# hkapp/cniic

Measured on AMD Instinct MI355X. Metric: Mpixels/sec encode (cluster-colors K=256), higher is better.
Workload: dtype u8/u64; 1 GPU; configs[1]: cluster-colors(256) encode of one 4096x4096 photo-like synthetic RGB image per GPU (seed 0x636E696963+2+rank), to convergence; image and stream HBM-resident; pixels_per_gpu=16777216, parallelism=1 GPU

## Files before the change

### cniic_amd/csrc/codec.cpp

```cpp
#include "codec.hpp"
#include "cc_small.hpp"
#include "vor_small.hpp"
#include "delta_small.hpp"
#include "delta_small_dec.hpp"
#include "huf_small.hpp"
#include "small_trie.hpp"

#include <algorithm>
#include <cctype>
#include <cmath>
#include <cstring>
#include <functional>
#include <memory>

#include "huff_host.hpp"
#include "pal_bounds.hpp"

namespace cniic {

HostTrace &host_trace() { static thread_local HostTrace t; return t; }

static bool match_fun_u32(const std::string &s, const char *const *names, uint32_t *arg) {
    for (size_t p = 0; p < s.size(); p++)
        for (int i = 0; names[i]; i++) {
            const size_t l = strlen(names[i]);
            if (s.compare(p, l, names[i]) != 0 || p + l >= s.size() || s[p + l] != '(') continue;
            size_t q = p + l + 1;
            if (q >= s.size() || !isdigit((unsigned char)s[q])) continue;
            unsigned long long v = 0;
            bool ok = true;
            while (q < s.size() && isdigit((unsigned char)s[q])) {
                v = v * 10 + (unsigned)(s[q] - '0');
                if (v > 0xffffffffull) { ok = false; break; }
                q++;
            }
            if (!ok || q >= s.size() || s[q] != ')') continue;
            *arg = (uint32_t)v;
            return true;
        }
    return false;
}

static bool parse_rust_f64(const std::string &t, double *out) {
    size_t p = 0;
    if (p < t.size() && (t[p] == '+' || t[p] == '-')) p++;
    std::string rest = t.substr(p);
    std::transform(rest.begin(), rest.end(), rest.begin(), [](unsigned char ch) { return (char)tolower(ch); });
    if (rest != "inf" && rest != "infinity" && rest != "nan") {
        size_t q = p, digits = 0;
        while (q < t.size() && isdigit((unsigned char)t[q])) { q++; digits++; }
        if (q < t.size() && t[q] == '.') {
            q++;
            while (q < t.size() && isdigit((unsigned char)t[q])) { q++; digits++; }
        }
        if (!digits) return false;
        if (q < t.size() && (t[q] == 'e' || t[q] == 'E')) {
            q++;
            if (q < t.size() && (t[q] == '+' || t[q] == '-')) q++;
            size_t ed = 0;
            while (q < t.size() && isdigit((unsigned char)t[q])) { q++; ed++; }
            if (!ed) return false;
        }
        if (q != t.size()) return false;
    }
    *out = strtod(t.c_str(), nullptr);
    return true;
}

static bool match_hilbert_rle(const std::string &s, double *d) {
    *d = 0.0;
    if (s.compare(0, 8, "hilbert(") != 0 && s.compare(0, 8, "Hilbert(") != 0) return false;
    if (s.size() < 10 || s.back() != ')') return false;
    const std::string arg = s.substr(8, s.size() - 9);
    if (arg == "rle") return true;
    if (arg.size() > 5 && arg.compare(0, 4, "rle(") == 0 && arg.back() == ')') {
        const std::string num = arg.substr(4, arg.size() - 5);
        double v = 0.0;
        if (parse_rust_f64(num, &v)) {
            if (v != 0.0) *d = v;
            return true;
        }
        char *end = nullptr;
        v = strtod(num.c_str(), &end);
        return end && *end == 0 && !num.empty() && v == 0.0;
    }
    return false;
}

bool parse_codec(const char *expr, CodecDesc *out) {
    if (!expr) return false;
    const std::string s(expr);
    static const char *const cc[] = {"cluster-colors", "cluster-col", "clustercolors", "clustercol",
                                     "c-colors", "c-col", "ccolors", "ccol", nullptr};
    static const char *const vo[] = {"voronoi", nullptr};
    uint32_t k = 0;
    double dv = 0.0;
    if (match_fun_u32(s, cc, &k)) { *out = {CODEC_CLUSTER_COLORS, k, 0.0}; return true; }
    if (match_fun_u32(s, vo, &k)) { *out = {CODEC_VORONOI, k, 0.0}; return true; }
// ... 227 lines not shown
    StreamOut so(c, out, cap, len);
    CNIIC_TRY(so.begin_sized(header_bytes, (nbits + 7) / 8));
    CNIIC_TRY(st.write_decoder(so, header));
    CNIIC_TRY(st.upload_codes());
    CNIIC_HIP_TRY(c, hipStreamSynchronize(c->stream));
    st.release_tree();
    uint64_t packed_bits = 0;
    ScopedKernelTimer timer(c, "huff_pack");
    uint32_t *const keys_d = st.keys_d.as<uint32_t>();
    const uint8_t *const len_d = st.len_d.as<uint8_t>();
    const uint64_t *const code_d = st.code_d.as<uint64_t>();
    if (hot_route) {
        CNIIC_TRY(huff_pack_code32_hot(c, syms_d, n, table_d, keys_d, len_d, code_d, U, syms_d, so.dev, header_bytes * 8, &packed_bits));
    } else if (direct) {
        CNIIC_TRY(huff_pack_code32(c, syms_d, rgb_d, n, table_d, keys_d, len_d, code_d, U, ranks, so.dev, header_bytes * 8, &packed_bits));
    } else if (inline_codes) {
        DevBuf code32;
        CNIIC_HIP_TRY(c, code32.alloc(U * 4));
        CNIIC_TRY(huff_pack_code32(c, ranks, nullptr, n, code32.as<uint32_t>(), nullptr, len_d, code_d, U, ranks, so.dev, header_bytes * 8, &packed_bits));
    } else {
        CNIIC_TRY(huff_pack_ranks(c, ranks, n, len_d, code_d, so.dev, header_bytes * 8, &packed_bits));
    }
    timer.stop(1);
    host_trace().mark("huf: pack");
    if (packed_bits != nbits)
        return c->fail(CNIIC_ERR_HIP, "huffman: packed %llu bits, histogram predicts %llu", (unsigned long long)packed_bits,
                       (unsigned long long)nbits);
    const int rc_fin = so.finish();
    host_trace().mark("huf: finish");
    host_trace().dump();
    return rc_fin;
}

static int encode_hufman(Ctx *c, const uint8_t *rgb_d, uint32_t w, uint32_t h, uint8_t *out, uint64_t cap, uint64_t *len) {
    const uint64_t n = (uint64_t)w * h;
    std::vector<uint8_t> header;
    put_u32(header, w);
    put_u32(header, h);
    uint32_t *table = nullptr;
    CNIIC_TRY(dense_table(c, 24, &table));
    return huf_encode_all_dev(c, CNIIC_SYM_RGB, rgb_d, nullptr, false, n, table, false, header, out, cap, len);
}

CcSession::~CcSession() { if (km) km_rgbw_destroy(km); }

int cc_prepare(Ctx *c, uint32_t *table_counts_d, uint32_t K, const cniic_kmeans_opts *opts, uint32_t shard, uint32_t nshards,
               void *partials_dev, CcSession **out, const uint32_t *occ_d) {
    if (K == 0) return c->fail(CNIIC_ERR_BAD_ARG, "cluster-colors(0)");
    auto s = std::make_unique<CcSession>();
    s->c = c; s->K = K; s->table = table_counts_d;
    s->counts_local = occ_d != nullptr || nshards == 1;
    CompactPlan plan;
    DevBuf cell_count;
    CNIIC_HIP_TRY(c, cell_count.alloc((uint64_t)kNumCells * 4));
    CNIIC_HIP_TRY(c, hipMemsetAsync(cell_count.p, 0, (uint64_t)kNumCells * 4, c->stream));
    CNIIC_TRY(hist_compact_count(c, table_counts_d, 24, &plan, cell_count.as<uint32_t>()));
    host_trace().mark("compact_count+sync");
    const uint64_t U = plan.n_unique;
    s->U = U;
    uint64_t Ug = 0;
    if (occ_d) {
        CNIIC_TRY(gidx_build(c, occ_d, s->gbits, s->gprefix, &Ug));
        s->local_points = true;
    }
    if ((occ_d ? Ug : U) / K == 0 || U == 0)
        return c->fail(CNIIC_ERR_TOO_FEW_POINTS, "kmeans: %llu distinct colours for %u clusters (src/kmeans.rs:68)",
                       (unsigned long long)(occ_d ? Ug : U), K);
    CNIIC_HIP_TRY(c, s->keys_d.alloc(U * 4));
    CNIIC_HIP_TRY(c, s->weight_d.alloc(U * 4));
    CNIIC_TRY(hist_compact_write(c, table_counts_d, &plan, s->keys_d.as<uint32_t>(), nullptr, s->weight_d.as<uint32_t>()));
    host_trace().mark("compact_write enq");
    CNIIC_TRY(km_rgbw_create(c, s->keys_d.as<uint32_t>(), s->weight_d.as<uint32_t>(), U, shard, nshards, K, opts, partials_dev,
                             table_counts_d, &s->km, cell_count.as<uint32_t>(), occ_d ? s->gbits.p : nullptr,
                             occ_d ? s->gprefix.as<uint32_t>() : nullptr, Ug));
    host_trace().mark("km_create");
    *out = s.release();
    return CNIIC_OK;
}

int cc_prepare_image(Ctx *c, const uint8_t *rgb_d, uint64_t npx, uint32_t K, const cniic_kmeans_opts *opts, CcSession **out) {
    if (K == 0) return c->fail(CNIIC_ERR_BAD_ARG, "cluster-colors(0)");
    auto s = std::make_unique<CcSession>();
    s->c = c; s->K = K; s->sp_mode = true;
    CNIIC_TRY(sp_build(c, rgb_d, npx, &s->sp));
    const uint64_t Umax = std::min<uint64_t>(npx, 1ull << 24);
    const uint64_t *U_dev = s->sp.total.as<uint64_t>();
    CNIIC_TRY(km_rgbw_create(c, nullptr, nullptr, Umax, 0, 1, K, opts, nullptr, nullptr, &s->km, s->sp.cell_count.as<uint32_t>(), s->sp.bits.p,
                             s->sp.wprefix.as<uint32_t>(), Umax, true, U_dev));
    uint32_t *cell_start, *ckeys, *cweight;
    km_rgbw_cell_arrays(s->km, &cell_start, &ckeys, &cweight);
    CNIIC_TRY(sp_emit(c, &s->sp, cell_start, ckeys, cweight, km_rgbw_labels_internal(s->km, nullptr), km_rgbw_is_wide(s->km), K, s->sp.bits.p,
                      s->sp.wprefix.as<uint32_t>(), 0, U_dev));
    CNIIC_TRY(sp_wait_count(c, &s->sp));
    s->U = s->sp.U;
    if (s->U / K == 0)
        return c->fail(CNIIC_ERR_TOO_FEW_POINTS, "kmeans: %llu distinct colours for %u clusters (src/kmeans.rs:68)", (unsigned long long)s->U, K);
    CNIIC_TRY(km_rgbw_set_points(s->km, s->U));
    host_trace().mark("km_create + emit enq");
    *out = s.release();
    return CNIIC_OK;
}

int cc_image_begin(Ctx *c, const uint8_t *rgb_d, uint64_t npx, CcSession **out) {
    auto s = std::make_unique<CcSession>();
    s->c = c; s->sp_mode = true; s->local_points = true;
    CNIIC_TRY(sp_build(c, rgb_d, npx, &s->sp));
    *out = s.release();
    return CNIIC_OK;
}

int cc_image_create(CcSession *s, const uint32_t *occ_d, uint32_t K, const cniic_kmeans_opts *opts, void *partials_dev) {
    Ctx *c = s->c;
    if (!s->sp_mode || s->km) return c->fail(CNIIC_ERR_BAD_ARG, "cc_image_create: needs a session from cc_image_begin, once");
    if (K == 0) return c->fail(CNIIC_ERR_BAD_ARG, "cluster-colors(0)");
    s->K = K;
    CNIIC_HIP_TRY(c, c->pinned_u.reserve(kPinnedUBytes, kPinnedUBytes));
    uint64_t *Ug_h = c->pinned_u.as<uint64_t>() + kPuPointCount.at;
    CNIIC_TRY(gidx_build(c, occ_d, s->gbits, s->gprefix, Ug_h, &s->gtotal));
    const uint64_t Umax = std::min<uint64_t>(s->sp.npx, 1ull << 24);
    const uint64_t *Ug_dev = s->gtotal.as<uint64_t>();
    CNIIC_TRY(km_rgbw_create(c, nullptr, nullptr, Umax, 0, 1, K, opts, partials_dev, nullptr, &s->km, s->sp.cell_count.as<uint32_t>(), s->gbits.p,
                             s->gprefix.as<uint32_t>(), 1ull << 24, true, Ug_dev));
    uint32_t *cell_start, *ckeys, *cweight;
    km_rgbw_cell_arrays(s->km, &cell_start, &ckeys, &cweight);
    CNIIC_TRY(sp_emit(c, &s->sp, cell_start, ckeys, cweight, km_rgbw_labels_internal(s->km, nullptr), km_rgbw_is_wide(s->km), K, s->gbits.p,
                      s->gprefix.as<uint32_t>(), 0, Ug_dev));
    CNIIC_HIP_TRY(c, hipMemcpyAsync(c->pinned_u.as<uint64_t>() + kPuImageCount.at, s->sp.total.p, 8, hipMemcpyDeviceToHost, c->stream));
    CNIIC_HIP_TRY(c, hipStreamSynchronize(c->stream));
    const uint64_t Ug = *Ug_h;
    s->sp.U = c->pinned_u.as<uint64_t>()[kPuImageCount.at];
    s->U = s->sp.U;
    if (Ug / K == 0 || s->U == 0)
        return c->fail(CNIIC_ERR_TOO_FEW_POINTS, "kmeans: %llu distinct colours for %u clusters (src/kmeans.rs:68)", (unsigned long long)Ug, K);
    return km_rgbw_set_points(s->km, s->U, Ug);
}

template <class Count>
static bool palette_code(const uint8_t *cent, const Count *pixels, uint32_t K, uint32_t w, uint32_t h, std::vector<uint8_t> &header,
                         uint8_t *clen, uint64_t *ccode, uint64_t *nbits) {
    auto colour = [&](uint32_t k) { return ((uint32_t)cent[3 * k] << 16) | ((uint32_t)cent[3 * k + 1] << 8) | cent[3 * k + 2]; };
    std::vector<std::pair<uint32_t, uint64_t>> kc;
    kc.reserve(K);
    for (uint32_t k = 0; k < K; k++)
        if (pixels[k]) kc.emplace_back(colour(k), pixels[k]);
    std::sort(kc.begin(), kc.end());
    std::vector<uint32_t> skeys;
    std::vector<uint64_t> scounts;
    for (auto &e : kc) {
        if (!skeys.empty() && skeys.back() == e.first) scounts.back() += e.second;
        else { skeys.push_back(e.first); scounts.push_back(e.second); }
    }
    HuffTree tree;
    std::vector<uint8_t> slen;
    std::vector<uint64_t> scode;
    if (!huff_build_tree(scounts.data(), scounts.size(), tree) || !huff_codes(tree, slen, scode)) return false;
    put_u32(header, w);
    put_u32(header, h);
    huff_serialize_tree(tree, CNIIC_SYM_RGB, skeys.data(), header);
    *nbits = 0;
    for (size_t i = 0; i < scounts.size(); i++) *nbits += scounts[i] * slen[i];
    for (uint32_t k = 0; k < K; k++) {
        const size_t si = std::lower_bound(skeys.begin(), skeys.end(), colour(k)) - skeys.begin();
        clen[k] = pixels[k] ? slen[si] : 0;
        ccode[k] = pixels[k] ? scode[si] : 0;
    }
    return true;
}

int cc_finish(CcSession *s, const uint8_t *rgb_d, uint32_t w, uint32_t h, const uint32_t *local_counts_d, uint8_t *out,
              uint64_t cap, uint64_t *len, cniic_kmeans_stats *stats) {
    Ctx *c = s->c;
    const uint32_t K = s->K;
    const uint64_t U = s->U, n = (uint64_t)w * h;
    KmRgbwState *km = s->km;
    std::vector<uint8_t> cent(3 * (size_t)K);
// ... 1714 lines not shown
```

### cniic_amd/csrc/common.hpp

```cpp
#pragma once
#include <hip/hip_runtime.h>

#include <algorithm>
#include <cstdarg>
#include <cstdint>
#include <cstdio>
#include <cstring>
#include <atomic>
#include <chrono>
#include <map>
#include <memory>
#include <mutex>
#include <string>
#include <thread>
#include <vector>

#include "../../include/cniic_hip.h"

namespace cniic {

constexpr uint64_t kDefaultSeed = 0x636E696963ULL;

struct KernelTime {
    double   ms = 0.0;
// ... 411 lines not shown
                volatile KmDevState *m = &slots[2];
                KmDevState t{};
                t.done = m->done;
                std::atomic_thread_fence(std::memory_order_acquire);
                t.iter = m->iter; t.moved_last = m->moved_last; t.reseeds = m->reseeds; t.active = m->active; t.pair_evals = m->pair_evals;
                *h = t;
            } else {
                *h = slots[slot ^ 1];
            }
        }
        slot ^= 1;
        pending = 1;
        last_prev = last_launch;
        return CNIIC_OK;
    }
    int drain(KmDevState *h) {
        KmDevState *slots = c->pinned.as<KmDevState>();
        CNIIC_HIP_TRY(c, hipEventSynchronize(c->poll_ev[slot ^ 1]));
        *h = slots[slot ^ 1];
        return CNIIC_OK;
    }
};

struct HostTrace {
    bool on;
    std::vector<std::pair<const char *, double>> marks;
    HostTrace() : on(test_env("CNIIC_TRACE_HOST") != nullptr) {}
    static double now() { return std::chrono::duration<double, std::micro>(std::chrono::steady_clock::now().time_since_epoch()).count(); }
    void mark(const char *what) { if (on) marks.emplace_back(what, now()); }
    void dump() {
        if (!on || marks.empty()) return;
        for (size_t i = 1; i < marks.size(); i++) fprintf(stderr, "[host] %-28s %8.1f us\n", marks[i].first, marks[i].second - marks[i - 1].second);
        fprintf(stderr, "[host] %-28s %8.1f us\n", "total", marks.back().second - marks.front().second);
        marks.clear();
    }
};
HostTrace &host_trace();

struct ScopedKernelTimer {
    Ctx        *c;
    const char *name;
    bool        on;
    ScopedKernelTimer(Ctx *ctx, const char *nm) : ScopedKernelTimer(ctx, nm, ctx->timers) {}
    ScopedKernelTimer(Ctx *ctx, const char *nm, bool enable) : c(ctx), name(nm), on(enable) {
        if (on) (void)hipEventRecord(c->ev0, c->stream);
    }
    void stop(uint64_t launches = 1) {
        if (!on) return;
        (void)hipEventRecord(c->ev1, c->stream);
        (void)hipEventSynchronize(c->ev1);
        float ms = 0.f;
        (void)hipEventElapsedTime(&ms, c->ev0, c->ev1);
        KernelTime &kt = c->ktimes[name];
        kt.ms += ms;
        kt.launches += launches;
        on = false;
    }
};


int hist_rgb_dense(Ctx *c, const uint8_t *rgb_d, uint64_t npx, uint32_t *table_d);
int hist_syms_dense(Ctx *c, const uint32_t *syms_d, uint64_t n, uint32_t *table_d, uint32_t bits);
struct CompactPlan {
    DevBuf   blockoff, blockmax;
    uint64_t n_unique = 0;
    uint64_t max_count = 0;
    uint32_t bits = 0;
    const uint8_t *pages = nullptr;
};
int occupancy_pack(Ctx *c, const uint32_t *table_d, uint32_t *occ_d);
int gidx_build(Ctx *c, const uint32_t *occ_d, DevBuf &bits, DevBuf &wprefix, uint64_t *U_h, DevBuf *total_keep = nullptr);
int gidx_finish(Ctx *c, uint32_t *wprefix_d, const uint32_t *blocktot_d, uint64_t *total_d);

struct SpPlan {
    uint64_t npx = 0, U = 0;
    uint32_t nchunks = 0;
    DevBuf cnt, pre, bstart;
    DevBuf part, prank;
    DevBuf cell_count;
    DevBuf sstart, sbin, scnt;
    DevBuf bits, wprefix;
    DevBuf total;
};
int sp_build(Ctx *c, const uint8_t *rgb_d, uint64_t npx, SpPlan *plan);
int sp_wait_count(Ctx *c, SpPlan *plan);
int sp_emit(Ctx *c, const SpPlan *plan, const uint32_t *cell_start_d, uint32_t *ckeys_d, uint32_t *cweight_d, void *labels_d, bool wide,
            uint32_t K, const void *gbits_d, const uint32_t *gprefix_d, uint64_t Ug, const uint64_t *Ug_dev );
int sp_occupancy(Ctx *c, const SpPlan *plan, uint32_t *occ_d);
int sp_pixel_labels(Ctx *c, const SpPlan *plan, const uint8_t *rgb_d, const uint32_t *cell_start_d, const uint32_t *ckeys_d,
                    const void *labels_d, bool wide, void *pixlab_d);
int sp_part_labels(Ctx *c, const SpPlan *plan, const uint32_t *cell_start_d, const uint32_t *ckeys_d, const void *labels_d, bool wide, DevBuf &partlab,
                   DevBuf *look );
int sp_pixlab(Ctx *c, const SpPlan *plan, const uint8_t *rgb_d, const void *partlab_d, bool wide, void *pixlab_d);
int sp_pixpack(Ctx *c, const SpPlan *plan, const void *partlab_d, DevBuf &look, const uint8_t *upl_h, uint32_t hdr_bytes, uint8_t *out_d, uint64_t *done_h);
constexpr uint32_t kCcUpCode = 0, kCcUpLen = 2048, kCcUpHdrBytes = 2304 , kCcUpHdr = 2312 , kCcUpBytes = 8192;
int hist_compact_count(Ctx *c, const uint32_t *table_d, uint32_t bits, CompactPlan *plan, uint32_t *cell_count_d = nullptr,
                       const uint8_t *pages_d = nullptr);
int hist_compact_write(Ctx *c, uint32_t *table_d, const CompactPlan *plan, uint32_t *keys_d, uint64_t *counts_d,
                       uint32_t *weights_d);
int dense_table(Ctx *c, uint32_t bits, uint32_t **table_d);

struct KmRgbwState;
int km_rgbw_create(Ctx *c, const uint32_t *keys_d, const uint32_t *weight_d, uint64_t U, uint32_t shard,
                   uint32_t nshards, uint32_t K, const cniic_kmeans_opts *opts, void *partials_dev,
                   const uint32_t *rank_table_d , KmRgbwState **out,
                   const uint32_t *cell_count_d = nullptr ,
                   const void *gbits_d = nullptr, const uint32_t *gprefix_d = nullptr, uint64_t Ug = 0
                   ,
                   bool points_follow = false ,
                   const uint64_t *points_dev = nullptr );
int km_rgbw_set_points(KmRgbwState *s, uint64_t U, uint64_t Ulist = 0 );
void km_rgbw_cell_arrays(KmRgbwState *s, uint32_t **cell_start_d, uint32_t **ckeys_d, uint32_t **cweight_d);
void km_rgbw_destroy(KmRgbwState *s);
int km_rgbw_set_state(KmRgbwState *s, const uint8_t *centroids_h, const uint32_t *labels_d_u32);
int km_rgbw_set_centroids(KmRgbwState *s, const uint8_t *init_h);
int km_rgbw_assign(KmRgbwState *s);
int km_rgbw_update(KmRgbwState *s);
struct Comm;
int comm_unique_id(uint8_t *id128);
int comm_create(Ctx *c, const uint8_t *id128, uint32_t rank, uint32_t nranks, Comm **out);
int comm_create_host(Ctx *c, uint32_t rank, uint32_t nranks, int32_t (*fn)(void *, void *, uint64_t, int32_t), void *user, Comm **out);
void comm_destroy(Comm *cm);
Ctx *comm_ctx(Comm *cm);
uint32_t comm_size(const Comm *cm);
int comm_all_reduce(Comm *cm, void *buf_d, uint64_t count, int kind);
void comm_abort(Comm *cm);
int comm_async_error(Comm *cm);
uint64_t comm_timeout_ms(const Comm *cm);
void comm_set_timeout_ms(Comm *cm, uint64_t ms);
int comm_create_mailbox(Ctx *c, uint32_t rank, uint32_t nranks, uint64_t max_bytes, uint8_t *handle64, Comm **out);
int comm_connect_mailbox(Comm *cm, const uint8_t *handles);

struct Mailbox;
int mailbox_create(Ctx *c, uint32_t rank, uint32_t nranks, uint64_t cap_bytes, uint8_t *handle64, Mailbox **out);
int mailbox_connect(Mailbox *m, const uint8_t *handles);
int mailbox_all_reduce(Mailbox *m, void *buf_d, uint64_t count, int kind, uint64_t timeout_ms);
int mailbox_status(const Mailbox *m);
void mailbox_abort(Mailbox *m);
void mailbox_destroy(Mailbox *m);

constexpr int kKmRetry = 1000;
int km_rgbw_run(KmRgbwState *s, Comm *cm = nullptr, bool may_defer = false);
int km_rgbw_poll_changed(KmRgbwState *s, uint64_t *changed);
int km_rgbw_poll(KmRgbwState *s, cniic_kmeans_stats *st, uint32_t *done);
bool km_rgbw_run_stats(KmRgbwState *s, cniic_kmeans_stats *st);
int km_rgbw_poll_lagged(KmRgbwState *s, cniic_kmeans_stats *st, uint32_t *done, uint32_t *have);
int km_rgbw_result(KmRgbwState *s, uint8_t *centroids_h, uint32_t *labels_d_u32, uint64_t *members_h,
                   uint64_t *wsum_h, cniic_kmeans_stats *stats);
int km_rgbw_result_begin(KmRgbwState *s);
int km_rgbw_result_end(KmRgbwState *s, uint8_t *centroids_h, uint64_t *members_h, uint64_t *wsum_h, cniic_kmeans_stats *stats);
int km_rgbw_time_assign(KmRgbwState *s, int reps, double *ms_per_launch);
int km_rgbw_partials(KmRgbwState *s, uint64_t *sums_h, uint64_t *wsum_h, uint64_t *members_h, uint64_t *changed_h);
void *km_rgbw_partials_dev(KmRgbwState *s);
const uint32_t *km_rgbw_centroids_dev(KmRgbwState *s);
bool km_rgbw_is_wide(KmRgbwState *s);
int km_rgbw_labels_canonical(KmRgbwState *s, void *dst_d);
void *km_rgbw_labels_internal(KmRgbwState *s, uint64_t *elem_bytes);
int km_rgbw_fold_initial(KmRgbwState *s);
int km_rgbw_export_labels(KmRgbwState *s, void *dst_d);
int km_rgbw_import_labels(KmRgbwState *s, const void *src_d);
uint64_t km_rgbw_points(KmRgbwState *s);

int km_xyrgb_run(Ctx *c, const uint8_t *rgb_d, uint32_t w, uint32_t h, uint32_t K,
                 const cniic_kmeans_opts *opts, cniic_colorpos *centroids_h, uint32_t *labels_d_u32,
                 uint64_t *members_h, cniic_kmeans_stats *stats, const cniic_colorpos *init_h = nullptr);
int km_xyrgb_run_wide(Ctx *c, const uint8_t *rgb_d, uint32_t w, uint32_t h, uint32_t K, const cniic_kmeans_opts *opts, cniic_colorpos *centroids_h,
                      uint32_t *labels_d_u32, uint64_t *members_h, cniic_kmeans_stats *stats, const cniic_colorpos *init_h = nullptr);
// ... 203 lines not shown
```

### cniic_amd/csrc/device_utils.hpp

```cpp
#pragma once
#include <hip/hip_runtime.h>

#include <cstdint>

namespace cniic {

__device__ __forceinline__ uint32_t rgb_key(const uint8_t *p) {
    return ((uint32_t)p[0] << 16) | ((uint32_t)p[1] << 8) | p[2];
}

__device__ __forceinline__ uint32_t key_from_le24(uint32_t v) { return __builtin_bswap32(v) >> 8; }

__device__ __forceinline__ void load16px_keys(const uint4 *p, uint32_t key[16]) {
    uint4 q0 = p[0], q1 = p[1], q2 = p[2];
    uint32_t w[12] = {q0.x, q0.y, q0.z, q0.w, q1.x, q1.y, q1.z, q1.w, q2.x, q2.y, q2.z, q2.w};
#pragma unroll
    for (int g = 0; g < 4; g++) {
        uint32_t a = w[3 * g], b = w[3 * g + 1], c = w[3 * g + 2];
        key[4 * g + 0] = key_from_le24(a);
        key[4 * g + 1] = key_from_le24((a >> 24) | (b << 8));
        key[4 * g + 2] = key_from_le24((b >> 16) | (c << 16));
        key[4 * g + 3] = key_from_le24(c >> 8);
    }
}
// ... 132 lines not shown
    __syncthreads();
    return off + inc - v;
}

template <int THREADS, int PER>
__device__ __forceinline__ void pack_emit(const uint32_t (&lab)[PER], const uint32_t (&l)[PER], uint32_t excl, uint32_t total, uint64_t g0,
                                          const unsigned long long *s_tab, uint32_t *img, uint32_t img_words, uint32_t *__restrict__ out_words) {
    const uint32_t skew = (uint32_t)(g0 & 31);
    uint32_t pos = skew + excl;
    const uint32_t nw_all = (skew + total + 31) >> 5;
    if (nw_all + 2 > img_words) {
        const uint64_t w0 = g0 >> 5;
#pragma unroll 1
        for (int i = 0; i < PER; i++) {
            const uint32_t L = l[i];
            if (L == 0) continue;
            const uint64_t cd = s_tab[lab[i]];
            const uint32_t w = pos >> 5, b = pos & 31, room = 32 - b;
            if (L <= room) {
                atomicOr(&out_words[w0 + w], __builtin_bswap32((uint32_t)(cd << (room - L))));
            } else {
                const uint32_t rem = L - room;
                atomicOr(&out_words[w0 + w], __builtin_bswap32((uint32_t)(cd >> rem)));
                if (rem <= 32) atomicOr(&out_words[w0 + w + 1], __builtin_bswap32((uint32_t)(cd << (32 - rem))));
                else { atomicOr(&out_words[w0 + w + 1], __builtin_bswap32((uint32_t)(cd >> (rem - 32)))); atomicOr(&out_words[w0 + w + 2], __builtin_bswap32((uint32_t)(cd << (64 - rem)))); }
            }
            pos += L;
        }
        return;
    }
    for (uint32_t i = threadIdx.x; i < nw_all + 2; i += THREADS) img[i] = 0;
    __syncthreads();
#pragma unroll
    for (int i = 0; i < PER; i++) {
        const uint32_t L = l[i];
        if (L == 0) continue;
        const uint64_t cd = s_tab[lab[i]];
        const uint32_t w = pos >> 5, b = pos & 31, room = 32 - b;
        if (L <= room) {
            atomicOr(&img[w], (uint32_t)(cd << (room - L)));
        } else {
            const uint32_t rem = L - room;
            atomicOr(&img[w], (uint32_t)(cd >> rem));
            if (rem <= 32) atomicOr(&img[w + 1], (uint32_t)(cd << (32 - rem)));
            else { atomicOr(&img[w + 1], (uint32_t)(cd >> (rem - 32))); atomicOr(&img[w + 2], (uint32_t)(cd << (64 - rem))); }
        }
        pos += L;
    }
    __syncthreads();
    if (total == 0) return;
    const uint64_t w0 = g0 >> 5;
    for (uint32_t i = threadIdx.x; i < nw_all; i += THREADS) {
        const uint32_t v = __builtin_bswap32(img[i]);
        if (v == 0) continue;
        if (i == 0 || i == nw_all - 1) atomicOr(&out_words[w0 + i], v);
        else out_words[w0 + i] = v;
    }
}

constexpr int kSuperShift = 6;
constexpr uint32_t kSupersPerDim = kCellsPerDim / 4;
__device__ __forceinline__ uint32_t cell_of(uint32_t key) {
    const uint32_t rc = ((key >> 16) & 255) >> kCellShift, gc = ((key >> 8) & 255) >> kCellShift, bc = (key & 255) >> kCellShift;
    const uint32_t sup = ((rc >> 2) * kSupersPerDim + (gc >> 2)) * kSupersPerDim + (bc >> 2);
    return (sup << kSuperShift) | ((rc & 3) << 4) | ((gc & 3) << 2) | (bc & 3);
}

struct GIdx {
    const unsigned long long *bits;
    const uint32_t *wprefix;
    uint64_t U;
};
__device__ __forceinline__ uint32_t gidx_rank(const GIdx &g, uint32_t key) {
    const uint32_t w = key >> 6;
    return g.wprefix[w] + (uint32_t)__popcll(g.bits[w] & ((1ull << (key & 63)) - 1ull));
}
__device__ __forceinline__ uint32_t gidx_select(const GIdx &g, uint64_t idx) {
    uint32_t a = 0, b = 1u << 18;
    while (b - a > 1) { const uint32_t mid = (a + b) >> 1; if (g.wprefix[mid] <= idx) a = mid; else b = mid; }
    unsigned long long word = g.bits[a];
    for (uint32_t r = (uint32_t)(idx - g.wprefix[a]); r; r--) word &= word - 1;
    return (a << 6) | (uint32_t)(__ffsll((long long)word) - 1);
}

__host__ __device__ __forceinline__ uint64_t splitmix_mix(uint64_t z) {
    z = (z ^ (z >> 30)) * 0xBF58476D1CE4E5B9ULL;
    z = (z ^ (z >> 27)) * 0x94D049BB133111EBULL;
    return z ^ (z >> 31);
}

__host__ __device__ __forceinline__ uint64_t reseed_index(uint64_t seed, uint64_t iter, uint32_t c, uint64_t n) {
    uint64_t z = seed + 0x9E3779B97F4A7C15ULL * (iter * 65536ULL + (uint64_t)c + 1ULL);
    return splitmix_mix(z) % n;
}

__host__ __device__ __forceinline__ uint32_t init_label(uint64_t i, uint64_t n, uint32_t K) {
    uint64_t ppc = n / K;
    uint64_t c = (n - 1 - i) / ppc;
    return (uint32_t)(c > (uint64_t)K - 1 ? (uint64_t)K - 1 : c);
}

__device__ __forceinline__ uint32_t div_floor_small(unsigned long long a, unsigned long long b) {
    if ((b >> 32) || (a >> 53)) return (uint32_t)(a / b);
    uint32_t q = (uint32_t)((double)a / (double)b);
    const uint32_t b32 = (uint32_t)b;
    if ((unsigned long long)q * b32 > a) q--;
    else if ((unsigned long long)(q + 1) * b32 <= a) q++;
    return q;
}

__device__ __forceinline__ uint32_t init_label24(uint32_t i, uint32_t n, uint32_t K, uint32_t ppc, float rcp) {
    const uint32_t x = n - 1 - i;
    uint32_t q = (uint32_t)((float)x * rcp);
    if (q * ppc > x) q--;
    else if ((q + 1) * ppc <= x) q++;
    return min(q, K - 1);
}

constexpr uint32_t kEscape = 63;

template <typename Emit>
__device__ __forceinline__ void pack_pieces(uint32_t pos, uint32_t L, uint64_t cd, Emit emit) {
    const uint32_t w = pos >> 5, b = pos & 31, room = 32 - b;
    if (L <= room) {
        emit(w, (uint32_t)(cd << (room - L)));
    } else {
        const uint32_t rem = L - room;
        emit(w, (uint32_t)(cd >> rem));
        if (rem <= 32) emit(w + 1, (uint32_t)(cd << (32 - rem)));
        else { emit(w + 1, (uint32_t)(cd >> (rem - 32))); emit(w + 2, (uint32_t)(cd << (64 - rem))); }
    }
}
template <bool DIRECT>
__device__ __forceinline__ void pack_put(uint32_t *words, uint32_t pos, uint32_t L, uint64_t cd) {
    pack_pieces(pos, L, cd, [&](uint32_t i, uint32_t v) { atomicOr(&words[i], DIRECT ? __builtin_bswap32(v) : v); });
}

}
```

### cniic_amd/csrc/k_hist.hip

```cpp
#include <cstdlib>

#include "common.hpp"
#include "device_utils.hpp"

namespace cniic {

__global__ __launch_bounds__(256) void k_hist_rgb(const uint8_t *__restrict__ rgb, uint64_t npx,
                                                  uint32_t *__restrict__ table) {
    const uint64_t ngroups = npx / 16;
    const uint64_t stride = (uint64_t)gridDim.x * blockDim.x;
    const uint4 *v = reinterpret_cast<const uint4 *>(rgb);
    for (uint64_t g = (uint64_t)blockIdx.x * blockDim.x + threadIdx.x; g < ngroups; g += stride) {
        uint32_t key[16];
        load16px_keys(v + 3 * g, key);
#pragma unroll
        for (int i = 0; i < 16; i++) atomic_count(table, key[i]);
    }
    if (blockIdx.x == 0) {
        uint64_t i = ngroups * 16 + threadIdx.x;
        if (i < npx) atomic_count(table, rgb_key(rgb + 3 * i));
    }
}

constexpr int kPartBits = 12;
// ... 259 lines not shown
        }
    }
    if (dirty) {
#pragma unroll
        for (int j = 0; j < kScanPerThread / 4; j++)
            v[j] = make_uint4(val[4 * j], val[4 * j + 1], val[4 * j + 2], val[4 * j + 3]);
    }
}

int hist_compact_count(Ctx *c, const uint32_t *table_d, uint32_t bits, CompactPlan *plan, uint32_t *cell_count_d, const uint8_t *pages_d) {
    static_assert(kScanChunk == (1 << kPageShift), "a page flag per block of the compaction");
    plan->pages = pages_d;
    const uint64_t entries = 1ull << bits;
    const uint32_t nblocks = (uint32_t)(entries / kScanChunk);
    DevBuf tot;
    CNIIC_HIP_TRY(c, plan->blockoff.alloc((uint64_t)nblocks * 4));
    CNIIC_HIP_TRY(c, plan->blockmax.alloc((uint64_t)nblocks * 4));
    CNIIC_HIP_TRY(c, tot.alloc(16));
    hipLaunchKernelGGL(k_compact_count, dim3(nblocks), dim3(kScanThreads), 0, c->stream, table_d, plan->blockoff.as<uint32_t>(), plan->blockmax.as<uint32_t>(),
                       bits == 24 ? cell_count_d : nullptr, pages_d, tot.as<uint64_t>());
    {
        const uint32_t nparts = (nblocks + 1023) / 1024;
        DevBuf parttot;
        CNIIC_HIP_TRY(c, parttot.alloc((uint64_t)nparts * 4));
        hipLaunchKernelGGL(k_compact_scan_local, dim3(nparts), dim3(1024), 0, c->stream, plan->blockoff.as<uint32_t>(), (const uint32_t *)plan->blockmax.as<uint32_t>(), nblocks,
                           parttot.as<uint32_t>(), tot.as<uint64_t>());
        if (nparts > 1)
            hipLaunchKernelGGL(k_compact_scan_add, dim3(nparts), dim3(1024), 0, c->stream, plan->blockoff.as<uint32_t>(), nblocks,
                               (const uint32_t *)parttot.as<uint32_t>(), tot.as<uint64_t>());
    }
    CNIIC_HIP_TRY(c, hipGetLastError());
    uint64_t total[2] = {0, 0};
    CNIIC_HIP_TRY(c, hipMemcpyAsync(total, tot.p, 16, hipMemcpyDeviceToHost, c->stream));
    CNIIC_HIP_TRY(c, pages_d ? ctx_spin_sync(c) : hipStreamSynchronize(c->stream));
    plan->n_unique = total[0];
    plan->max_count = total[1];
    plan->bits = bits;
    return CNIIC_OK;
}

int hist_compact_write(Ctx *c, uint32_t *table_d, const CompactPlan *plan, uint32_t *keys_d, uint64_t *counts_d,
                       uint32_t *weights_d) {
    const uint32_t nblocks = (uint32_t)((1ull << plan->bits) / kScanChunk);
    hipLaunchKernelGGL(k_compact_write, dim3(nblocks), dim3(kScanThreads), 0, c->stream, table_d,
                       plan->blockoff.as<uint32_t>(), keys_d, counts_d, weights_d, plan->pages);
    CNIIC_HIP_TRY(c, hipGetLastError());
    return CNIIC_OK;
}

__global__ __launch_bounds__(256) void k_occ_pack(const uint32_t *__restrict__ table, uint32_t *__restrict__ occ) {
    const uint32_t wd = blockIdx.x * 256 + threadIdx.x;
    const uint4 a = reinterpret_cast<const uint4 *>(table)[2 * (size_t)wd], b = reinterpret_cast<const uint4 *>(table)[2 * (size_t)wd + 1];
    occ[wd] = (a.x != 0) | ((a.y != 0) << 4) | ((a.z != 0) << 8) | ((a.w != 0) << 12) | ((b.x != 0) << 16) | ((b.y != 0) << 20) |
              ((b.z != 0) << 24) | ((uint32_t)(b.w != 0) << 28);
}
__global__ __launch_bounds__(256) void k_gidx_words(const uint32_t *__restrict__ occ, unsigned long long *__restrict__ bits,
                                                    uint32_t *__restrict__ wprefix, uint32_t *__restrict__ blocktot) {
    __shared__ uint32_t wsum[256 / 64];
    const uint32_t w0 = (blockIdx.x * 256 + threadIdx.x) * 4;
    uint32_t cnt[4], mine = 0;
#pragma unroll
    for (int q = 0; q < 4; q++) {
        unsigned long long m = 0;
#pragma unroll
        for (int j = 0; j < 8; j++) {
            const uint32_t v = occ[8 * (size_t)(w0 + q) + j];
#pragma unroll
            for (int i = 0; i < 8; i++)
                if ((v >> (4 * i)) & 15u) m |= 1ull << (8 * j + i);
        }
        bits[w0 + q] = m;
        cnt[q] = (uint32_t)__popcll(m);
        mine += cnt[q];
    }
    uint32_t run = block_exclusive_scan<256>(mine, wsum);
#pragma unroll
    for (int q = 0; q < 4; q++) { wprefix[w0 + q] = run; run += cnt[q]; }
    if (threadIdx.x == 255) blocktot[blockIdx.x] = run;
}
__global__ __launch_bounds__(256) void k_gidx_finish(uint32_t *__restrict__ wprefix, const uint32_t *__restrict__ blocktot,
                                                     uint64_t *__restrict__ total) {
    __shared__ uint32_t wsum[256 / 64];
    __shared__ uint32_t boff[256];
    const uint32_t t = blocktot[threadIdx.x];
    const uint32_t ex = block_exclusive_scan<256>(t, wsum);
    boff[threadIdx.x] = ex;
    if (blockIdx.x == 0 && threadIdx.x == 255) *total = (uint64_t)ex + t;
    __syncthreads();
    const uint32_t add = boff[blockIdx.x];
    for (uint32_t i = threadIdx.x; i < 1024; i += 256) wprefix[blockIdx.x * 1024 + i] += add;
}

int gidx_finish(Ctx *c, uint32_t *wprefix_d, const uint32_t *blocktot_d, uint64_t *total_d) {
    hipLaunchKernelGGL(k_gidx_finish, dim3(256), dim3(256), 0, c->stream, wprefix_d, blocktot_d, total_d);
    CNIIC_HIP_TRY(c, hipGetLastError());
    return CNIIC_OK;
}

int occupancy_pack(Ctx *c, const uint32_t *table_d, uint32_t *occ_d) {
    hipLaunchKernelGGL(k_occ_pack, dim3((1u << 21) / 256), dim3(256), 0, c->stream, table_d, occ_d);
    CNIIC_HIP_TRY(c, hipGetLastError());
    return CNIIC_OK;
}

int gidx_build(Ctx *c, const uint32_t *occ_d, DevBuf &bits, DevBuf &wprefix, uint64_t *U_h, DevBuf *total_keep) {
    DevBuf tot_own;
    DevBuf &tot = total_keep ? *total_keep : tot_own;
    CNIIC_HIP_TRY(c, bits.alloc((1ull << 18) * 8));
    CNIIC_HIP_TRY(c, wprefix.alloc((1ull << 18) * 4));
    CNIIC_HIP_TRY(c, tot.alloc(8));
    DevBuf blocktot;
    CNIIC_HIP_TRY(c, blocktot.alloc(256 * 4));
    hipLaunchKernelGGL(k_gidx_words, dim3(256), dim3(256), 0, c->stream, occ_d, bits.as<unsigned long long>(), wprefix.as<uint32_t>(),
                       blocktot.as<uint32_t>());
    hipLaunchKernelGGL(k_gidx_finish, dim3(256), dim3(256), 0, c->stream, wprefix.as<uint32_t>(), (const uint32_t *)blocktot.as<uint32_t>(),
                       tot.as<uint64_t>());
    CNIIC_HIP_TRY(c, hipGetLastError());
    CNIIC_HIP_TRY(c, hipMemcpyAsync(U_h, tot.p, 8, hipMemcpyDeviceToHost, c->stream));
    if (!total_keep) CNIIC_HIP_TRY(c, hipStreamSynchronize(c->stream));
    return CNIIC_OK;
}

int dense_table(Ctx *c, uint32_t bits, uint32_t **table_d) {
    const uint64_t bytes = (1ull << bits) * 4;
    if (c->dense.bytes < bytes) CNIIC_HIP_TRY(c, c->dense.alloc(bytes));
    CNIIC_HIP_TRY(c, hipMemsetAsync(c->dense.p, 0, bytes, c->stream));
    *table_d = c->dense.as<uint32_t>();
    return CNIIC_OK;
}

}
```

### cniic_amd/csrc/k_kmeans_persist.hip

```cpp
#include <atomic>

#include <hip/hip_ext.h>

#include "kmeans_rgbw.hpp"

namespace cniic {

constexpr int kPsThreads = 1024, kPsWaves = kPsThreads / 64;
constexpr uint32_t kPsAccWords = 5 * 256;
constexpr uint32_t kPsOffTab = kPsAccWords * 8, kPsOffS = kPsOffTab + 256 * 8;
constexpr uint32_t kPsStaticMax = 3072;
static_assert(kPsDynBytes + kPsStaticMax <= 160 * 1024, "static + dynamic LDS of k_rgbw_persist: a CU has 160 KiB");
static_assert(kPsOffCell == kPsOffS + kPsSlotsMax * kPsScap * 4, "ps_cell_bytes / kPsOffCell (kmeans_rgbw.hpp) describe this layout");

__device__ __forceinline__ uint32_t ps_xcc_id() {
    uint32_t v;
    asm volatile("s_getreg_b32 %0, hwreg(HW_REG_XCC_ID)" : "=s"(v));
    return v & 7u;
}
__device__ __forceinline__ unsigned long long ps_aread(unsigned long long *p) {
    return __hip_atomic_fetch_add(p, 0ull, __ATOMIC_RELAXED, __HIP_MEMORY_SCOPE_AGENT);
}
__device__ __forceinline__ uint32_t ps_ld(const uint32_t *p) { return __hip_atomic_load(p, __ATOMIC_RELAXED, __HIP_MEMORY_SCOPE_AGENT); }
__device__ __forceinline__ void ps_st(uint32_t *p, uint32_t v) { __hip_atomic_store(p, v, __ATOMIC_RELAXED, __HIP_MEMORY_SCOPE_AGENT); }

__device__ __forceinline__ bool ps_spin(uint32_t *word, uint32_t old, PsBar *b, unsigned long long ticks) {
    const unsigned long long t0 = wall_clock64();
    uint32_t spins = 0;
    while (ps_ld(word) == old) {
        __builtin_amdgcn_s_sleep(1);
        if ((++spins & 63u) == 0) {
            if (ps_ld(&b->abort_.v)) return false;
            if (wall_clock64() - t0 > ticks) { ps_st(&b->abort_.v, 1u); return false; }
        }
    }
    return true;
}
__device__ __forceinline__ bool ps_barrier_flat(PsBar *b, uint32_t nblocks, unsigned long long ticks) {
    const uint32_t g = ps_ld(&b->gen.v);
    if (__hip_atomic_fetch_add(&b->count.v, 1u, __ATOMIC_RELAXED, __HIP_MEMORY_SCOPE_AGENT) == nblocks - 1) {
        ps_st(&b->count.v, 0u);
        ps_st(&b->gen.v, g + 1);
        return true;
    }
    return ps_spin(&b->gen.v, g, b, ticks);
}
__device__ __forceinline__ bool ps_barrier_xcd(PsBar *b, uint32_t x, uint32_t nx_blocks, uint32_t nxcd, unsigned long long ticks) {
    const uint32_t tg = ps_ld(&b->topgen.v);
    if (__hip_atomic_fetch_add(&b->xcount[x].v, 1u, __ATOMIC_RELAXED, __HIP_MEMORY_SCOPE_AGENT) == nx_blocks - 1) {
        ps_st(&b->xcount[x].v, 0u);
        if (__hip_atomic_fetch_add(&b->top.v, 1u, __ATOMIC_RELAXED, __HIP_MEMORY_SCOPE_AGENT) == nxcd - 1) {
            ps_st(&b->top.v, 0u);
            ps_st(&b->topgen.v, tg + 1);
            return true;
        }
    }
    return ps_spin(&b->topgen.v, tg, b, ticks);
}

__global__ __launch_bounds__(1024) void k_ps_ranges(const uint32_t *__restrict__ ne_cost, const uint32_t *__restrict__ ne_count, uint32_t G, uint32_t dyn_bytes,
                                                    uint32_t *__restrict__ cb, PsDev *__restrict__ dev, PsDevPtrs ptrs) {
    uint32_t *fail = &dev->fail;
    if (threadIdx.x == 0) dev->p = ptrs;
    const uint32_t M = *ne_count, NC = G * kPsChunks;
    const uint64_t total = ne_cost[M];
    for (uint32_t g0 = threadIdx.x; g0 <= NC; g0 += 8 * blockDim.x) {
        uint32_t a[8], b[8];
        uint64_t c_lo[8];
#pragma unroll
        for (int r = 0; r < 8; r++) {
            const uint32_t g = g0 + r * blockDim.x;
            c_lo[r] = total * min(g, NC) / NC;
            a[r] = 0; b[r] = g <= NC ? M : 0u;
        }
        bool more = true;
        while (more) {
            more = false;
            uint32_t mid[8], v[8];
#pragma unroll
            for (int r = 0; r < 8; r++) { mid[r] = (a[r] + b[r]) >> 1; v[r] = a[r] < b[r] ? ne_cost[mid[r]] : 0u; }
#pragma unroll
            for (int r = 0; r < 8; r++)
                if (a[r] < b[r]) { if (v[r] < c_lo[r]) a[r] = mid[r] + 1; else b[r] = mid[r]; more = more || a[r] < b[r]; }
        }
#pragma unroll
        for (int r = 0; r < 8; r++) {
            const uint32_t g = g0 + r * blockDim.x;
            if (g <= NC) cb[g] = g == NC ? M : a[r];
        }
    }
    __syncthreads();
    for (uint32_t g = threadIdx.x; g < G; g += blockDim.x) {
        uint32_t C = 0;
        for (uint32_t r = 0; r < kPsChunks; r++) C += cb[r * G + g + 1] - cb[r * G + g];
        if (C > kPsMaxCells || kPsOffCell + ps_cell_bytes(C) > dyn_bytes) atomicAdd(fail, 1u);
    }
}

template <class Op> __device__ __forceinline__ uint32_t row_allreduce(uint32_t v, Op op) {
    v = op(v, (uint32_t)__builtin_amdgcn_update_dpp(0, (int)v, 0x121, 0xf, 0xf, false));
    v = op(v, (uint32_t)__builtin_amdgcn_update_dpp(0, (int)v, 0x122, 0xf, 0xf, false));
    v = op(v, (uint32_t)__builtin_amdgcn_update_dpp(0, (int)v, 0x124, 0xf, 0xf, false));
    v = op(v, (uint32_t)__builtin_amdgcn_update_dpp(0, (int)v, 0x128, 0xf, 0xf, false));
    return v;
}
__device__ __forceinline__ uint32_t row_min(uint32_t v) { return row_allreduce(v, [](uint32_t a, uint32_t b) { return a < b ? a : b; }); }
__device__ __forceinline__ uint32_t row_max(uint32_t v) { return row_allreduce(v, [](uint32_t a, uint32_t b) { return a > b ? a : b; }); }
__device__ __forceinline__ uint32_t row_sum(uint32_t v) { return row_allreduce(v, [](uint32_t a, uint32_t b) { return a + b; }); }

__device__ __forceinline__ uint32_t ps_centre_dist(uint32_t ck, uint32_t cpk, uint32_t cc) { return dot4u8(ck, ck, cc) - 2u * dot4u8(ck, cpk, 0); }

__device__ __forceinline__ void ps_build_lists(const uint2 *tab, uint32_t K, uint32_t nslots, const uint16_t *ssup, uint32_t *s_nS, uint32_t *s_lpiv, uint32_t *Sent, int wid, int lane) {
    constexpr int32_t ext = (1 << (kCellShift + 2)) - 1;
    for (uint32_t slot = (uint32_t)wid; slot < nslots; slot += kPsWaves) {
        const CellBox bx = super_box((uint32_t)__builtin_amdgcn_readfirstlane((int)ssup[slot]));
        const uint32_t cpk = pack_rgb(bx.r0 + 16, bx.g0 + 16, bx.b0 + 16), cc = dot4u8(cpk, cpk, 0);
        uint32_t ck[4], best = 0xffffffffu;
#pragma unroll
        for (int r = 0; r < 4; r++) {
            const uint32_t k = 64u * r + (uint32_t)lane;
            ck[r] = k < K ? tab[k].x : 0u;
            if (k < K) best = min(best, (ps_centre_dist(ck[r], cpk, cc) << 8) | k);
        }
        const uint32_t piv = wave_reduce_min(best) & 255u;
        Dominance dm;
        dm.set(bx, ext, (uint32_t)__builtin_amdgcn_readfirstlane((int)tab[piv].x));
        uint32_t n = 0;
#pragma unroll
        for (int r = 0; r < 4; r++) {
            const uint32_t k = 64u * r + (uint32_t)lane;
            const bool keep = k < K && dm.worst(ck[r]) >= 0;
            const unsigned long long bm = __ballot(keep);
            const uint32_t pos = n + lanes_below(bm);
            if (keep && pos < kPsScap) Sent[slot * kPsScap + pos] = (k << 24) | ck[r];
            n += (uint32_t)__popcll(bm);
        }
        if (lane == 0) { s_nS[slot] = n; s_lpiv[slot] = piv; }
    }
    __syncthreads();
}

constexpr uint32_t kPsUlMask = 0x1ffu, kPsComplete = 0x200u;

__device__ __forceinline__ bool ps_row_finish(uint32_t *rec, uint32_t l16, uint32_t pid, uint32_t lpid, bool complete) {
    const uint32_t w = l16 < 8 ? rec[2 + l16] : 0u;
    const uint32_t pc = (uint32_t)__popc(w);
    uint32_t inc = pc;
    inc += (uint32_t)__builtin_amdgcn_update_dpp(0, (int)inc, 0x111, 0xf, 0xf, true);
    inc += (uint32_t)__builtin_amdgcn_update_dpp(0, (int)inc, 0x112, 0xf, 0xf, true);
    inc += (uint32_t)__builtin_amdgcn_update_dpp(0, (int)inc, 0x114, 0xf, 0xf, true);
    const uint32_t cnt = row_max(inc);
    uint32_t pos = inc - pc, ww = w;
    uint8_t *c4 = reinterpret_cast<uint8_t *>(rec + 10);
    while (ww && pos < 4) {
        c4[pos] = (uint8_t)(32u * l16 + (uint32_t)__builtin_ctz(ww));
        ww &= ww - 1;
        pos++;
    }
    const uint32_t r1 = rec[1];
    if (l16 == 0) rec[1] = (r1 & kPsUlMask) | (pid << 16) | (lpid << 24) | (complete ? kPsComplete : 0u);
    const uint32_t only = rec[10] & 255u;
    return !(cnt == 1 && (r1 & kPsUlMask) == only);
}

__device__ __forceinline__ uint32_t ps_row_build_list(const uint2 *tab, const uint32_t *ent, uint32_t n, uint32_t c, uint32_t l16, uint32_t *rec) {
    constexpr int32_t ext = (1 << kCellShift) - 1;
    constexpr int PER = kPsScap / 16;
    const CellBox bx = cell_box(c);
    const uint32_t cpk = pack_rgb(bx.r0 + 4, bx.g0 + 4, bx.b0 + 4), cc = dot4u8(cpk, cpk, 0);
    uint32_t en[PER];
#pragma unroll
    for (int t = 0; t < PER; t++) en[t] = l16 + 16u * t < n ? ent[l16 + 16u * t] : 0xffffffffu;
    uint32_t best = 0xffffffffu;
#pragma unroll
    for (int t = 0; t < PER; t++)
        if (l16 + 16u * t < n) best = min(best, (ps_centre_dist(en[t] & 0xffffffu, cpk, cc) << 8) | (en[t] >> 24));
    const uint32_t pid = row_min(best) & 255u;
    Dominance dm;
    dm.set(bx, ext, tab[pid].x);
// ... 655 lines not shown
                const uint32_t r = div_floor_small(run[0], run[3]) & 255, g = div_floor_small(run[1], run[3]) & 255, b = div_floor_small(run[2], run[3]) & 255;
                ck = (r << 16) | (g << 8) | b;
                atomicAdd(&s_active, 1u);
            }
            const uint32_t oldc = tab[k].x;
            tab[k] = make_cconst(ck, k, 8);
            if (ck != oldc) {
                const uint32_t pos = atomicAdd(&s_nmoved, 1u);
                if (pos < kMaxMovedSkip) { s_mlist[pos] = k; s_mcol[pos] = ck; }
                atomicOr(&s_mm[(k >> 6) & 3], 1ull << (k & 63));
            }
        } else if (tid_i == kPsThreads - 1) {
            s_changed = ps_aread(&Pcur[5 * (size_t)K]);
            s_pev = ps_aread(&Pcur[5 * (size_t)K + 1]);
        }
        __syncthreads();
        const unsigned long long changed = s_changed;
        nS = s_nmoved;
        const bool fin = changed == 0 || (a.max_iters && j >= a.max_iters);
        if (blockIdx.x == 0 && tid_i == 0) {
            KmDevState *sw = a.st_rw;
            const unsigned long long reseeds_total = s_rtot + s_reseed, evals_total = s_etot + s_pev;
            s_rtot = reseeds_total; s_etot = evals_total;
            sw->changed_ring[(j - 1) % kHistRing] = changed;
            sw->nmoved_ring[(j - 1) % kHistRing] = nS;
            if (fin) {
                sw->moved_last = changed; sw->reseeds = reseeds_total; sw->active = s_active; sw->pair_evals = evals_total; sw->iter = j; sw->done = 1;
                PsExit *x = &a.cold->exit;
                x->iter = j; x->moved_last = changed; x->reseeds = reseeds_total; x->active = s_active; x->pair_evals = evals_total;
            }
        }
        if (fin) break;
    }
    if (blockIdx.x == 0 && tid < K) {
        const PsCold *cd = a.cold;
        const uint2 cc = tab[tid];
        cd->cent_g[tid] = cc.x;
        cd->cconst_g[tid] = cc;
        cd->members_out[tid] = runs[256 * 4 + tid];
        cd->wsum_out[tid] = runs[256 * 3 + tid];
    }
    uint8_t *labels = dev->p.labels;
    for (uint32_t i = wid; i < C; i += kPsWaves) {
        const uint32_t s = cstart[i], n = cstart[i + 1] - s, gs = gstart[i];
        if (i < Cres) { for (uint32_t t = lane; t < n; t += 64) labels[gs + t] = (uint8_t)(255u - (pts[s + t] >> 24)); }
        else { for (uint32_t t = lane; t < n; t += 64) labels[gs + t] = (uint8_t)(255u - (a.pk[gs + t] >> 24)); }
    }
    if (blockIdx.x == 0) {
        __syncthreads();
        if (tid == 0) { __threadfence_system(); a.cold->exit.status = kPsStatusDone; __threadfence_system(); }
    }
}

static std::atomic<int> g_ps_cus_in_use[16];

static int ps_cu_count(int device) {
    static std::atomic<int> cached[16];
    const int d = device >= 0 && device < 16 ? device : 0;
    int n = cached[d].load();
    if (n) return n;
    hipDeviceProp_t prop;
    if (hipGetDeviceProperties(&prop, device) != hipSuccess) { (void)hipGetLastError(); return 0; }
    cached[d].store(prop.multiProcessorCount);
    return prop.multiProcessorCount;
}

uint32_t ps_grid_for(Ctx *c, uint64_t Umax) {
    uint32_t G = (uint32_t)ps_cu_count(c->device);
    if (!G) return 0;
    G = std::max(1u, G / std::max(1u, c->ps_div));
    if (const uint64_t mb = c->opt(CNIIC_OPT_KM_MAX_BLOCKS, "CNIIC_KM_MAX_BLOCKS", 0)) G = std::max<uint32_t>(1u, (uint32_t)((uint64_t)G * std::min<uint64_t>(mb, 768) / 768));
    if (const char *e = test_env("CNIIC_KM_PS_BLOCKS")) G = std::max(1, atoi(e));
    G = (uint32_t)std::min<uint64_t>(G, std::max<uint64_t>(1, ceil_div(Umax, 512)));
    return std::min<uint32_t>(G, 1024u);
}

static void ps_learn(Ctx *c, uint32_t status, bool injected) {
    if (status == kPsStatusDone) { c->ps_backoff = 0; c->ps_backoff_left = 0; return; }
    if (status != kPsStatusAborted || injected) return;
    c->ps_backoff = std::min<uint32_t>(256u, std::max<uint32_t>(4u, 2u * c->ps_backoff));
    c->ps_backoff_left = c->ps_backoff;
}

int ps_prepare(KmRgbwState *s) {
    Ctx *c = s->c;
    if (c->ps_backoff_left && !test_env("CNIIC_KM_PS_REQUIRE")) { c->ps_backoff_left--; return CNIIC_OK; }
    const uint32_t G = ps_grid_for(c, s->U);
    if (!G) return CNIIC_OK;
    static bool attr_set[16] = {};
    if (c->device >= 0 && c->device < 16 && !attr_set[c->device]) {
        CNIIC_HIP_TRY(c, hipFuncSetAttribute(reinterpret_cast<const void *>(k_rgbw_persist), hipFuncAttributeMaxDynamicSharedMemorySize, (int)kPsDynBytes));
        attr_set[c->device] = true;
    }
    const uint64_t o_part = kPsArenaPart, o_fail = kPsArenaFail, o_rng = kPsArenaRng, total = o_rng + ((uint64_t)G * kPsChunks + 1) * 4;
    CNIIC_HIP_TRY(c, s->ps_arena.alloc(total));
    CNIIC_HIP_TRY(c, hipMemsetAsync(s->ps_arena.p, 0, o_rng, c->stream));
    CNIIC_HIP_TRY(c, s->ps_pk.alloc(std::max<uint64_t>(s->U, 1) * 4));
    s->ps_blocks = G;
    s->ps_o_part = o_part; s->ps_o_fail = o_fail; s->ps_o_rng = o_rng;
    uint8_t *a = s->ps_arena.as<uint8_t>();
    uint32_t budget = kPsBudget;
    if (const char *e = test_env("CNIIC_TEST_PS_LDS_BYTES")) budget = std::min<uint32_t>(kPsBudget, (uint32_t)atoi(e));
    s->ps_budget = budget;
    PsDevPtrs ptrs{};
    ptrs.ckeys = s->ckeys.as<uint32_t>(); ptrs.cweight = s->cweight.as<uint32_t>(); ptrs.labels = s->labels.as<uint8_t>();
    ptrs.ne_cell = s->ne_cell.as<uint32_t>(); ptrs.ne_start = s->ne_start.as<uint32_t>(); ptrs.cconst0 = s->cconst.as<uint2>();
    hipLaunchKernelGGL(k_ps_ranges, dim3(1), dim3(1024), 0, c->stream, (const uint32_t *)s->ne_cost.as<uint32_t>(), (const uint32_t *)s->ne_count.as<uint32_t>(), G, budget,
                       reinterpret_cast<uint32_t *>(a + o_rng), reinterpret_cast<PsDev *>(a + o_fail), ptrs);
    CNIIC_HIP_TRY(c, hipGetLastError());
    s->ps = true;
    return CNIIC_OK;
}

int km_rgbw_run_persistent(KmRgbwState *s, bool *ran, bool may_defer) {
    Ctx *c = s->c;
    *ran = false;
    if (!s->ps || s->ps_tried) return CNIIC_OK;
    s->ps_tried = true;
    const int dev = c->device >= 0 && c->device < 16 ? c->device : 0, G = (int)s->ps_blocks;
    if (g_ps_cus_in_use[dev].fetch_add(G) + G > ps_cu_count(c->device)) { g_ps_cus_in_use[dev].fetch_sub(G); return CNIIC_OK; }
    std::shared_ptr<void> release(nullptr, [dev, G](void *) { g_ps_cus_in_use[dev].fetch_sub(G); });
    CNIIC_HIP_TRY(c, c->pinned_ps.reserve(1024, 1024));
    static_assert(sizeof(PsCold) <= 1024, "the pinned block holds a PsCold");
    PsCold *cold = c->pinned_ps.as<PsCold>();
    memset(cold, 0, sizeof *cold);
    PsExit *xh = &cold->exit;
    uint8_t *ar = s->ps_arena.as<uint8_t>();
    PsArgs a{};
    a.cweight = s->cweight.as<uint32_t>();
    a.lds_budget = s->ps_budget;
    a.pk = s->ps_pk.as<uint32_t>();
    a.bar = reinterpret_cast<PsBar *>(ar);
    cold->cconst_g = s->cconst.as<uint2>(); cold->cent_g = s->cent.as<uint32_t>(); cold->members_out = s->members_last.as<uint64_t>(); cold->wsum_out = s->wsum_last.as<uint64_t>();
    cold->keys = s->keys; cold->gx = s->gidx; cold->seed = s->seed; cold->U = s->gidx.bits ? s->gidx.U : s->U;
    a.st_rw = s->dstate.as<KmDevState>(); a.cold = cold; a.max_iters = s->max_iters;
    a.K = s->K; a.max_skip = s->no_skip ? 0u : s->max_skip; a.agg_iters = kAggLaunches;
    a.test_abort_at = 0;
    if (const char *e = test_env("CNIIC_TEST_PS_ABORT_AT")) a.test_abort_at = (uint32_t)atoi(e);
    a.clean_skip = 1;
    if (const char *e = test_env("CNIIC_KM_PS_CLEANSKIP")) a.clean_skip = atoi(e) ? 1u : 0u;
    uint64_t tmo_ms = 2000;
    if (const char *e = test_env("CNIIC_KM_PS_TIMEOUT_MS")) tmo_ms = (uint64_t)atoll(e);
    a.timeout_ticks = tmo_ms * 100000ull;
    hipEvent_t e0 = nullptr, e1 = nullptr;
    if (s->profile) { CNIIC_HIP_TRY(c, hipEventCreate(&e0)); CNIIC_HIP_TRY(c, hipEventCreate(&e1)); }
    hipExtLaunchKernelGGL(k_rgbw_persist, dim3((uint32_t)G), dim3(kPsThreads), kPsDynBytes, c->stream, e0, e1, 0, a);
    CNIIC_HIP_TRY(c, hipGetLastError());
    if (may_defer && !s->profile) {
        s->ps_pending = true;
        s->ps_hold = release;
        *ran = true;
        return CNIIC_OK;
    }
    CNIIC_HIP_TRY(c, ctx_spin_sync(c));
    const uint32_t status = xh->status;
    ps_learn(c, status, a.test_abort_at != 0);
    if (status != kPsStatusDone) {
        if (e0) { (void)hipEventDestroy(e0); (void)hipEventDestroy(e1); }
        if (test_env("CNIIC_KM_PS_REQUIRE")) return c->fail(CNIIC_ERR_HIP, "kmeans_rgbw: the persistent launch ended with status %u (CNIIC_KM_PS_REQUIRE)", status);
        return CNIIC_OK;
    }
    s->run_stats.iterations = xh->iter; s->run_stats.moved_last = xh->moved_last; s->run_stats.empty_reseeds = xh->reseeds;
    s->run_stats.active = xh->active; s->run_stats.pair_evals = xh->pair_evals;
    s->run_stats_valid = true;
    if (s->profile) {
        float ms = 0.f;
        (void)hipEventElapsedTime(&ms, e0, e1);
        (void)hipEventDestroy(e0); (void)hipEventDestroy(e1);
        KernelTime &kt = c->ktimes["kmeans_rgbw_persist"];
        kt.ms += ms; kt.launches += 1;
        KernelTime &ki = c->ktimes["kmeans_rgbw_persist_iters"];
        ki.ms += ms; ki.launches += xh->iter;
    }
    *ran = true;
    return CNIIC_OK;
}

int km_rgbw_persistent_verdict(KmRgbwState *s, bool *retry) {
    Ctx *c = s->c;
    *retry = false;
    s->ps_pending = false;
    s->ps_hold.reset();
    const PsExit *xh = &c->pinned_ps.as<const PsCold>()->exit;
    ps_learn(c, xh->status, test_env("CNIIC_TEST_PS_ABORT_AT") != nullptr);
    if (xh->status == kPsStatusDone) {
        s->run_stats.iterations = xh->iter; s->run_stats.moved_last = xh->moved_last; s->run_stats.empty_reseeds = xh->reseeds;
        s->run_stats.active = xh->active; s->run_stats.pair_evals = xh->pair_evals;
        s->run_stats_valid = true;
        return CNIIC_OK;
    }
    if (test_env("CNIIC_KM_PS_REQUIRE")) return c->fail(CNIIC_ERR_HIP, "kmeans_rgbw: the persistent launch ended with status %u (CNIIC_KM_PS_REQUIRE)", xh->status);
    CNIIC_TRY(km_rgbw_run(s, nullptr, false));
    *retry = true;
// ... 5 lines not shown
```

### cniic_amd/csrc/k_kmeans_rgbw.hip

```cpp
#include <cstdlib>
#include <memory>
#include <vector>


#include <hip/hip_ext.h>

#include "kmeans_rgbw.hpp"

namespace cniic {


__global__ void k_rgbw_init_cent(const uint32_t *__restrict__ keys, uint64_t U, uint32_t K, uint32_t Kpad, uint32_t idbits,
                                 uint2 *__restrict__ cconst, uint32_t *__restrict__ cent, GIdx gx, uint32_t *__restrict__ cent_copy,
                                 uint32_t *__restrict__ moved_list, const uint64_t *__restrict__ U_dev) {
    uint32_t k = blockIdx.x * blockDim.x + threadIdx.x;
    if (U_dev) U = max(*U_dev, (uint64_t)K);
    if (k == 0 && moved_list) moved_list[0] = K;
    if (k < K) {
        uint64_t ppc = U / K;
        uint64_t first = (k < K - 1) ? U - ((uint64_t)k + 1) * ppc : 0;
        uint32_t ck = gx.bits ? gidx_select(gx, first) : keys[first];
        cent[k] = ck;
        if (cent_copy) cent_copy[k] = ck;
        cconst[k] = make_cconst(ck, k, idbits);
    } else if (k < Kpad) {
        cconst[k] = make_uint2(0u, 0u);
    }
}

__global__ void k_rgbw_given_cent(const uint32_t *__restrict__ given , uint32_t K, uint32_t Kpad, uint32_t idbits, uint2 *__restrict__ cconst,
                                  uint32_t *__restrict__ cent, uint32_t *__restrict__ cent_copy) {
    const uint32_t k = blockIdx.x * blockDim.x + threadIdx.x;
    if (k < K) {
        const uint32_t ck = given[k] & 0xffffffu;
        cent[k] = ck;
        if (cent_copy) cent_copy[k] = ck;
        cconst[k] = make_cconst(ck, k, idbits);
    } else if (k < Kpad) {
        cconst[k] = make_uint2(0u, 0u);
    }
}

template <typename LabelT>
__global__ void k_rgbw_init_labels(const uint32_t *__restrict__ rank, uint64_t U, uint64_t lo, uint64_t hi, uint32_t K,
                                   LabelT *__restrict__ labels) {
    const uint64_t stride = (uint64_t)gridDim.x * blockDim.x;
    for (uint64_t i = lo + (uint64_t)blockIdx.x * blockDim.x + threadIdx.x; i < hi; i += stride)
        labels[i - lo] = (LabelT)init_label(rank ? rank[i] : i, U, K);
}

template <typename LabelT, int IDBITS>
__global__ __launch_bounds__(kAssignThreads) void k_rgbw_assign(
    const uint32_t *__restrict__ keys, const uint32_t *__restrict__ weight, uint64_t lo, uint64_t hi,
    uint32_t K, uint32_t Kpad, const uint2 *__restrict__ cconst, LabelT *__restrict__ labels,
    uint64_t *__restrict__ slabs, const KmDevState *__restrict__ st) {
    extern __shared__ __align__(16) unsigned long long lds[];
    if (st->done) return;
    unsigned long long *acc = lds;
    uint2 *tab = reinterpret_cast<uint2 *>(lds + 5 * (size_t)K);
    for (uint32_t i = threadIdx.x; i < 5 * K; i += kAssignThreads) acc[i] = 0ull;
    for (uint32_t i = threadIdx.x; i < K; i += kAssignThreads) tab[i] = cconst[i];
    __syncthreads();

    constexpr uint32_t IDMASK = (1u << IDBITS) - 1;
    const uint64_t n = hi - lo;
    const uint64_t sweep = (uint64_t)gridDim.x * kAssignThreads * kPPT;
    uint32_t moved = 0;
    for (uint64_t base = (uint64_t)blockIdx.x * kAssignThreads * kPPT; base < n; base += sweep) {
        uint32_t p[kPPT], best[kPPT];
        bool valid[kPPT];
#pragma unroll
        for (int j = 0; j < kPPT; j++) {
            uint64_t i = base + (uint64_t)j * kAssignThreads + threadIdx.x;
            valid[j] = i < n;
            p[j] = valid[j] ? keys[lo + i] : 0u;
            best[j] = 0u;
        }
#pragma unroll 4
        for (uint32_t k = 0; k < Kpad; k++) {
            const uint2 cc = cconst[k];
#pragma unroll
            for (int j = 0; j < kPPT; j++) {
                uint32_t key = (dot4u8(p[j], cc.x, 0) << (IDBITS + 1)) + cc.y;
                best[j] = max(best[j], key);
            }
        }
#pragma unroll
        for (int j = 0; j < kPPT; j++) {
            if (!valid[j]) continue;
            uint64_t i = base + (uint64_t)j * kAssignThreads + threadIdx.x;
            uint32_t cur = labels[i];
            uint2 cc = tab[cur];
            uint32_t kcur = (dot4u8(p[j], cc.x, 0) << (IDBITS + 1)) + cc.y;
            uint32_t nl = cur;
            if ((best[j] >> IDBITS) > (kcur >> IDBITS)) {
                nl = IDMASK - (best[j] & IDMASK);
                labels[i] = (LabelT)nl;
                moved++;
            }
            uint64_t w = weight[lo + i];
            uint32_t r = (p[j] >> 16) & 255, g = (p[j] >> 8) & 255, b = p[j] & 255;
            atomicAdd(&acc[3 * nl + 0], (unsigned long long)(r * w));
            atomicAdd(&acc[3 * nl + 1], (unsigned long long)(g * w));
            atomicAdd(&acc[3 * nl + 2], (unsigned long long)(b * w));
            atomicAdd(&acc[3 * K + nl], (unsigned long long)w);
            atomicAdd(&acc[4 * K + nl], 1ull);
        }
    }
    moved = block_reduce_sum<kAssignThreads>(moved);
    __syncthreads();
    uint64_t *row = slabs + (size_t)blockIdx.x * (5 * (size_t)K + 2);
    for (uint32_t i = threadIdx.x; i < 5 * K; i += kAssignThreads) row[i] = acc[i];
    if (threadIdx.x == 0) {
        row[5 * (size_t)K] = moved;
        uint64_t per_block = 0;
        for (uint64_t base = (uint64_t)blockIdx.x * kAssignThreads * kPPT; base < n; base += sweep)
            per_block += min((uint64_t)kAssignThreads * kPPT, n - base);
        row[5 * (size_t)K + 1] = per_block * K;
    }
}

__global__ __launch_bounds__(256) void k_slab_reduce(const uint64_t *__restrict__ slabs, uint32_t nrows, uint32_t W,
                                                     uint64_t *__restrict__ partials,
                                                     const KmDevState *__restrict__ st) {
    if (st->done) return;
    __shared__ unsigned long long sh[4][64];
    const uint32_t col = blockIdx.x * 64 + (threadIdx.x & 63);
    const uint32_t rl = threadIdx.x >> 6;
    unsigned long long s = 0;
    if (col < W)
        for (uint32_t r = blockIdx.y * 4 + rl; r < nrows; r += gridDim.y * 4) s += slabs[(size_t)r * W + col];
    sh[rl][threadIdx.x & 63] = s;
    __syncthreads();
    if (rl == 0 && col < W) {
        s = sh[0][threadIdx.x] + sh[1][threadIdx.x] + sh[2][threadIdx.x] + sh[3][threadIdx.x];
        if (s) atomicAdd(reinterpret_cast<unsigned long long *>(partials) + col, s);
    }
}

__global__ __launch_bounds__(256) void k_cell_count(const uint32_t *__restrict__ keys, uint64_t U,
                                                    uint32_t *__restrict__ cell_count) {
    const uint64_t stride = (uint64_t)gridDim.x * blockDim.x;
    const int lane = threadIdx.x & 63;
    for (uint64_t base = (uint64_t)blockIdx.x * blockDim.x; base < U; base += stride) {
        const uint64_t i = base + threadIdx.x;
        bool active = i < U;
        const uint32_t cell = active ? cell_of(keys[i]) : 0;
        for (;;) {
            unsigned long long m = __ballot(active);
            if (!m) break;
            const int leader = __ffsll((long long)m) - 1;
            const uint32_t lc = (uint32_t)__builtin_amdgcn_readlane((int)cell, leader);
            const bool same = active && cell == lc;
            const unsigned long long ms = __ballot(same);
            if (lane == leader) atomicAdd(&cell_count[lc], (uint32_t)__popcll(ms));
            active = active && !same;
        }
    }
}

constexpr uint32_t kCellGroups = kNumCells / 64;
__global__ __launch_bounds__(64) void k_cell_totals(const uint32_t *__restrict__ cell_count, uint2 *__restrict__ tot) {
    const uint32_t v = cell_count[blockIdx.x * 64 + threadIdx.x];
    const uint32_t sum = wave_reduce_sum(v), sweeps = wave_reduce_sum((v + 64 * kSweep - 1) / (64 * kSweep));
    const uint32_t ne = (uint32_t)__popcll(__ballot(v != 0));
    if (threadIdx.x == 0) { tot[blockIdx.x] = make_uint2(sum, ne); tot[kCellGroups + blockIdx.x] = make_uint2(sweeps, 0u); }
}
__global__ __launch_bounds__(64) void k_cell_scan(const uint32_t *__restrict__ cell_count, const uint2 *__restrict__ tot,
                                                  uint32_t *__restrict__ cell_start, uint32_t *__restrict__ cursor,
                                                  uint32_t *__restrict__ ne_cell, uint32_t *__restrict__ ne_start,
                                                  uint32_t *__restrict__ ne_cost, uint32_t *__restrict__ ne_count, uint32_t fixed_cost,
                                                  uint32_t sweep_cost) {
    const uint32_t lane = threadIdx.x, grp = blockIdx.x;
    uint32_t ps = 0, pn = 0, pw = 0;
    for (uint32_t g = lane; g < grp; g += 64) { const uint2 t = tot[g]; ps += t.x; pn += t.y; pw += tot[kCellGroups + g].x; }
    const uint32_t base = wave_reduce_sum(ps), nbase = wave_reduce_sum(pn), wbase = wave_reduce_sum(pw);
    const uint32_t cell = grp * 64 + lane, v = cell_count[cell], sw = (v + 64 * kSweep - 1) / (64 * kSweep);
    const uint32_t start = base + wave_inclusive_scan(v) - v, swb = wbase + wave_inclusive_scan(sw) - sw;
    cell_start[cell] = start;
    if (cursor) cursor[cell] = start;
    const unsigned long long nzm = __ballot(v != 0);
    if (v) {
        const uint32_t m = nbase + (uint32_t)__popcll(nzm & ((1ull << lane) - 1ull));
        ne_cell[m] = cell; ne_start[m] = start; ne_cost[m] = (sweep_cost ? swb * sweep_cost : start) + m * fixed_cost;
    }
    if (grp == kCellGroups - 1 && lane == 63) {
        const uint32_t U = start + v, M = nbase + (uint32_t)__popcll(nzm);
        cell_start[kNumCells] = U;
        ne_start[M] = U;
        ne_cost[M] = (sweep_cost ? (swb + sw) * sweep_cost : U) + M * fixed_cost;
        *ne_count = M;
    }
}

constexpr uint32_t kCellColours = 1u << (3 * kCellShift);
__device__ __forceinline__ uint32_t cell_key(uint32_t cell, uint32_t t) {
    constexpr uint32_t lm = (1u << kCellShift) - 1;
    const CellBox bx = cell_box(cell);
    const uint32_t r = (uint32_t)bx.r0 | (t >> (2 * kCellShift));
    const uint32_t g = (uint32_t)bx.g0 | ((t >> kCellShift) & lm);
    const uint32_t b = (uint32_t)bx.b0 | (t & lm);
    return (r << 16) | (g << 8) | b;
}
__global__ __launch_bounds__(512) void k_cells_count_tbl(const uint32_t *__restrict__ table, uint32_t *__restrict__ cell_count) {
    uint32_t mine = 0;
    for (uint32_t t = threadIdx.x; t < kCellColours; t += 512) mine += table[cell_key(blockIdx.x, t)] != 0;
    const uint32_t n = block_reduce_sum<512>(mine);
    if (threadIdx.x == 0) cell_count[blockIdx.x] = n;
}
template <typename LabelT>
__global__ __launch_bounds__(512) void k_cells_write_tbl(const uint32_t *__restrict__ table, const uint32_t *__restrict__ weight,
                                                         const uint32_t *__restrict__ cell_start, uint64_t U, uint32_t K,
                                                         uint32_t *__restrict__ ckeys, uint32_t *__restrict__ cweight,
                                                         uint32_t *__restrict__ crank, LabelT *__restrict__ labels, GIdx gx) {
    __shared__ uint32_t wsum[512 / 64];
    __shared__ uint32_t s_run;
    const uint32_t s = cell_start[blockIdx.x], e = cell_start[blockIdx.x + 1];
    if (s == e) return;
    if (threadIdx.x == 0) s_run = s;
    __syncthreads();
    for (uint32_t t0 = 0; t0 < kCellColours; t0 += 512) {
        const uint32_t key = cell_key(blockIdx.x, t0 + threadIdx.x);
        const uint32_t v = table[key];
        const uint32_t run = s_run;
        const uint32_t pos = run + block_exclusive_scan<512>(v != 0, wsum);
        if (v) {
            const uint32_t rank = v - 1;
            ckeys[pos] = key;
            cweight[pos] = weight[rank];
            crank[pos] = rank;
            labels[pos] = (LabelT)init_label(gx.bits ? gidx_rank(gx, key) : rank, U, K);
        }
        if (threadIdx.x == 511) s_run = pos + (v != 0);
        __syncthreads();
    }
}

__global__ __launch_bounds__(256) void k_cell_scatter(const uint32_t *__restrict__ keys, const uint32_t *__restrict__ weight,
                                                      uint64_t U, uint32_t *__restrict__ cursor,
                                                      uint32_t *__restrict__ ckeys, uint32_t *__restrict__ cweight,
                                                      uint32_t *__restrict__ crank) {
    const uint64_t stride = (uint64_t)gridDim.x * blockDim.x;
    const int lane = threadIdx.x & 63;
    for (uint64_t base = (uint64_t)blockIdx.x * blockDim.x; base < U; base += stride) {
        const uint64_t i = base + threadIdx.x;
        bool active = i < U;
        const uint32_t key = active ? keys[i] : 0;
        const uint32_t cell = cell_of(key);
        uint32_t pos = 0;
        for (;;) {
            unsigned long long m = __ballot(active);
            if (!m) break;
            const int leader = __ffsll((long long)m) - 1;
            const uint32_t lc = (uint32_t)__builtin_amdgcn_readlane((int)cell, leader);
            const bool same = active && cell == lc;
            const unsigned long long ms = __ballot(same);
            uint32_t b = 0;
            if (lane == leader) b = atomicAdd(&cursor[lc], (uint32_t)__popcll(ms));
            b = (uint32_t)__builtin_amdgcn_readlane((int)b, leader);
            if (same) pos = b + (uint32_t)__popcll(ms & ((1ull << lane) - 1));
            active = active && !same;
        }
        if (i < U) {
            ckeys[pos] = key;
            cweight[pos] = weight[i];
            crank[pos] = (uint32_t)i;
        }
    }
}

__global__ __launch_bounds__(256) void k_wave_ranges(const uint32_t *__restrict__ ne_cost, const uint32_t *__restrict__ ne_count,
                                                     uint32_t G, uint32_t *__restrict__ wfirst) {
    const uint32_t g = blockIdx.x * blockDim.x + threadIdx.x;
    if (g > G) return;
    const uint32_t M = *ne_count;
// ... 738 lines not shown
    if (threadIdx.x == 0) { s_reseed = 0; s_active = 0; s_nmoved = 0; }
    __syncthreads();
    if (done) return;
    for (uint32_t k = threadIdx.x; k < K; k += blockDim.x) {
        const size_t at[5] = {3 * (size_t)k, 3 * (size_t)k + 1, 3 * (size_t)k + 2, 3 * (size_t)K + k, 4 * (size_t)K + k};
        uint64_t v[5];
#pragma unroll
        for (int i = 0; i < 5; i++) { v[i] = partials[at[i]]; partials[at[i]] = 0; }
        if (mode == 1) {
#pragma unroll
            for (int i = 0; i < 5; i++) { v[i] += running[at[i]]; running[at[i]] = v[i]; }
        }
        const uint64_t members = v[4], w = v[3];
        members_out[k] = members;
        wsum_out[k] = w;
        uint32_t ck;
        if (members == 0) {
            const uint64_t ri = reseed_index(seed, iter, k, U);
            ck = gx.bits ? gidx_select(gx, ri) : keys[ri];
            atomicAdd(&s_reseed, 1u);
        } else {
            const uint32_t r = div_floor_small(v[0], w) & 255, g = div_floor_small(v[1], w) & 255, b = div_floor_small(v[2], w) & 255;
            ck = (r << 16) | (g << 8) | b;
            atomicAdd(&s_active, 1u);
        }
        if (moved_list && ck != cent[k]) moved_list[1 + atomicAdd(&s_nmoved, 1u)] = k;
        cent[k] = ck;
        cconst[k] = make_cconst(ck, k, idbits);
    }
    __syncthreads();
    if (threadIdx.x == 0 && moved_list) moved_list[0] = s_nmoved;
    if (threadIdx.x == 0) {
        partials[5 * (size_t)K] = 0;
        partials[5 * (size_t)K + 1] = 0;
        st->changed_ring[iter % kHistRing] = changed;
        st->nmoved_ring[iter % kHistRing] = s_nmoved;
        st->moved_last = changed;
        st->reseeds += s_reseed;
        st->active = s_active;
        st->pair_evals += evals;
        st->iter = iter + 1;
        if (changed == 0 || (max_iters && iter + 1 >= max_iters)) st->done = 1;
    }
}

template <typename LabelT>
__global__ void k_widen_labels(const LabelT *__restrict__ in, const uint32_t *__restrict__ rank, uint32_t *__restrict__ out,
                               uint64_t lo, uint64_t hi) {
    const uint64_t stride = (uint64_t)gridDim.x * blockDim.x;
    for (uint64_t i = lo + (uint64_t)blockIdx.x * blockDim.x + threadIdx.x; i < hi; i += stride) {
        if (rank) out[rank[i]] = in[i];
        else out[i - lo] = in[i - lo];
    }
}
template <typename LabelT>
__global__ void k_narrow_labels(const uint32_t *__restrict__ in, LabelT *__restrict__ out, uint64_t n) {
    const uint64_t stride = (uint64_t)gridDim.x * blockDim.x;
    for (uint64_t i = (uint64_t)blockIdx.x * blockDim.x + threadIdx.x; i < n; i += stride) out[i] = (LabelT)in[i];
}
template <typename LabelT>
__global__ void k_labels_to_canonical(const LabelT *__restrict__ in, const uint32_t *__restrict__ rank, LabelT *__restrict__ out,
                                      uint64_t U) {
    const uint64_t stride = (uint64_t)gridDim.x * blockDim.x;
    for (uint64_t i = (uint64_t)blockIdx.x * blockDim.x + threadIdx.x; i < U; i += stride) out[rank[i]] = in[i];
}
__global__ void k_set_cconst(const uint32_t *__restrict__ cent, uint32_t K, uint32_t Kpad, uint32_t idbits,
                             uint2 *__restrict__ cconst) {
    uint32_t k = blockIdx.x * blockDim.x + threadIdx.x;
    if (k < K) cconst[k] = make_cconst(cent[k], k, idbits);
    else if (k < Kpad) cconst[k] = make_uint2(0u, 0u);
}

static inline uint32_t grid_1d(uint64_t n, uint32_t cap = 2048) {
    return (uint32_t)std::min<uint64_t>(std::max<uint64_t>(ceil_div(n, 256), 1), cap);
}

#define KM_ALLOC(buf, bytes)                                                                       \
    do {                                                                                           \
        hipError_t _e = (buf).alloc(bytes);                                                        \
        if (_e != hipSuccess) { delete s; return c->fail(CNIIC_ERR_HIP, "kmeans_rgbw: hipMalloc(%llu) failed: %s", \
                                                        (unsigned long long)(bytes), hipGetErrorString(_e)); } \
    } while (0)

int km_rgbw_create(Ctx *c, const uint32_t *keys_d, const uint32_t *weight_d, uint64_t U, uint32_t shard,
                   uint32_t nshards, uint32_t K, const cniic_kmeans_opts *opts, void *partials_dev,
                   const uint32_t *rank_table_d, KmRgbwState **out, const uint32_t *cell_count_d, const void *gbits_d,
                   const uint32_t *gprefix_d, uint64_t Ug, bool points_follow, const uint64_t *points_dev) {
    if (K == 0 || U == 0 || nshards == 0 || shard >= nshards) return c->fail(CNIIC_ERR_BAD_ARG, "kmeans_rgbw: bad sizes");
    if (points_follow && (!gbits_d || !cell_count_d || nshards != 1 || (opts && (opts->flags & CNIIC_KM_BRUTE_FORCE))))
        return c->fail(CNIIC_ERR_BAD_ARG, "kmeans_rgbw: points written by the caller need the cell counts and the colour index");
    if (!points_follow && gbits_d && (!rank_table_d || nshards != 1 || (opts && (opts->flags & CNIIC_KM_BRUTE_FORCE))))
        return c->fail(CNIIC_ERR_BAD_ARG, "kmeans_rgbw: a share of a larger point list needs the table-driven cells path, unsharded");
    const uint64_t lo = U * shard / nshards, hi = U * (shard + 1) / nshards;
    const uint64_t Ulist = gbits_d ? Ug : U;
    if (points_dev && !points_follow) return c->fail(CNIIC_ERR_BAD_ARG, "kmeans_rgbw: a device-side point count needs points_follow");
    if (!points_dev && Ulist / K == 0) return c->fail(CNIIC_ERR_TOO_FEW_POINTS, "kmeans: %llu points for %u clusters (src/kmeans.rs:68)",
                                       (unsigned long long)Ulist, K);
    if (K > 65535) return c->fail(CNIIC_ERR_UNSUPPORTED, "kmeans_rgbw: K=%u > 65535 not supported", K);
    if (K > 2048 && (nshards != 1 || (opts && (opts->flags & CNIIC_KM_BRUTE_FORCE))))
        return c->fail(CNIIC_ERR_UNSUPPORTED, "kmeans_rgbw: K=%u > 2048 runs unsharded on the cell-major arrays only", K);
    if (U >= (1ull << 32)) return c->fail(CNIIC_ERR_BAD_ARG, "kmeans_rgbw: too many points");
    auto *s = new KmRgbwState();
    s->c = c; s->U = U; s->lo = lo; s->hi = hi; s->K = K; s->shard = shard; s->nshards = nshards;
    s->Kpad = (K + 3) & ~3u;
    s->wide = K > 256;
    s->big = K > 2048;
    s->idbits = s->wide ? 12 : 8;
    s->seed = (opts && opts->seed) ? opts->seed : kDefaultSeed;
    s->max_iters = opts ? opts->max_iters : 0;
    s->cells = !(opts && (opts->flags & CNIIC_KM_BRUTE_FORCE));
    s->profile = opts && (opts->flags & CNIIC_KM_PROFILE);
    s->no_skip = opts && (opts->flags & CNIIC_KM_NO_SKIP);
    if (const char *ms = test_env("CNIIC_KM_MAXSKIP")) s->max_skip = std::min<uint32_t>((uint32_t)atoi(ms), kMaxMovedSkip);
    if (const char *fa = test_env("CNIIC_TEST_FAIL_AT_LAUNCH")) s->fail_at = atol(fa);
    s->keys = keys_d; s->weight = weight_d;
    s->gidx = GIdx{static_cast<const unsigned long long *>(gbits_d), gprefix_d, Ug};
    const uint64_t n = hi - lo;
    const uint64_t W = 5 * (uint64_t)K + 2;
    const uint64_t lab_bytes = s->wide ? 2 : 1;
    KM_ALLOC(s->cconst, (uint64_t)s->Kpad * 8);
    s->res_cent = (sizeof(KmDevState) + 255) & ~255ull;
    s->res_members = s->res_cent + (((uint64_t)K * 4 + 7) & ~7ull);
    s->res_wsum = s->res_members + (uint64_t)K * 8;
    s->res_bytes = s->res_wsum + (uint64_t)K * 8;
    s->fused = s->cells && !s->wide && !(test_env("CNIIC_KM_UNFUSED") && atoi(test_env("CNIIC_KM_UNFUSED")));
    {
        auto up = [](uint64_t x) { return (x + 255) & ~255ull; };
        const uint64_t o_part = up(s->res_bytes), o_run = o_part + up(partials_dev ? 0 : W * 8), o_fp = o_run + up(s->cells ? W * 8 : 0);
        const uint64_t o_fr = o_fp + up(s->fused ? 3 * W * 8 : 0), o_fc = o_fr + up(s->fused ? 2 * W * 8 : 0);
        const uint64_t o_mv = o_fc + up(s->fused ? 2 * (uint64_t)K * 4 : 0), total = o_mv + up(s->cells ? ((uint64_t)K + 1) * 4 : 0);
        KM_ALLOC(s->arena, total);
        (void)hipMemsetAsync(s->arena.p, 0, total, c->stream);
        uint8_t *a = s->arena.as<uint8_t>();
        s->resblk.view(a, s->res_bytes);
        if (partials_dev) {
            s->partials = reinterpret_cast<uint64_t *>(partials_dev);
            (void)hipMemsetAsync(s->partials, 0, W * 8, c->stream);
        } else {
            s->partials_own.view(a + o_part, W * 8);
            s->partials = s->partials_own.as<uint64_t>();
        }
        if (s->cells) {
            s->running.view(a + o_run, W * 8);
            s->moved_list.view(a + o_mv, ((uint64_t)K + 1) * 4);
        }
        if (s->fused) {
            s->fused_partials.view(a + o_fp, 3 * W * 8);
            s->fused_running.view(a + o_fr, 2 * W * 8);
            s->fused_cent.view(a + o_fc, 2 * (uint64_t)K * 4);
        }
    }
    s->dstate.view(s->resblk.p, sizeof(KmDevState));
    s->cent.view(static_cast<uint8_t *>(s->resblk.p) + s->res_cent, (uint64_t)K * 4);
    s->members_last.view(static_cast<uint8_t *>(s->resblk.p) + s->res_members, (uint64_t)K * 8);
    s->wsum_last.view(static_cast<uint8_t *>(s->resblk.p) + s->res_wsum, (uint64_t)K * 8);
    hipLaunchKernelGGL(k_rgbw_init_cent, dim3(ceil_div(s->Kpad, 256)), dim3(256), 0, c->stream, keys_d, Ulist, K, s->Kpad, s->idbits,
                       s->cconst.as<uint2>(), s->cent.as<uint32_t>(), s->gidx, s->fused ? s->fused_cent.as<uint32_t>() : (uint32_t *)nullptr,
                       s->cells ? s->moved_list.as<uint32_t>() : (uint32_t *)nullptr, points_dev);
    if (s->cells) {
        s->nblocks = (uint32_t)std::min<uint64_t>(std::max<uint64_t>(ceil_div(U / nshards, s->wide ? 1024 : 64), 1), s->wide ? 4096u : kCellBlocks);
        if (const uint64_t mb = c->opt(CNIIC_OPT_KM_MAX_BLOCKS, "CNIIC_KM_MAX_BLOCKS", 0)) {
            const uint32_t cap = std::max(3u, (uint32_t)std::min<uint64_t>(mb, kCellBlocks) / 3 * 3);
            if (!s->wide && nshards == 1 && s->nblocks > cap) s->nblocks = cap;
        }
        if (s->wide) s->nblocks = (s->nblocks + 7) & ~7u;
        KM_ALLOC(s->labels, std::max<uint64_t>(U, 1) * lab_bytes);
        KM_ALLOC(s->ckeys, U * 4);
        KM_ALLOC(s->cweight, U * 4);
        if (!points_follow) KM_ALLOC(s->crank, U * 4);
        KM_ALLOC(s->cell_start, ((uint64_t)kNumCells + 1) * 4);
        KM_ALLOC(s->ne_cell, (uint64_t)kNumCells * 4);
        KM_ALLOC(s->ne_start, ((uint64_t)kNumCells + 1) * 4);
        KM_ALLOC(s->ne_cost, ((uint64_t)kNumCells + 1) * 4);
        KM_ALLOC(s->ne_count, 4);
        const uint32_t G = s->nblocks * (s->wide ? 1u : (uint32_t)kCellWaves) * nshards;
        KM_ALLOC(s->wfirst, ((uint64_t)G + 1) * 4);
        if (!s->big) KM_ALLOC(s->cell_rec, (uint64_t)kNumCells * cell_rec_words((K + 63) / 64) * 4);
        DevBuf count, cursor, cell_tot;
        KM_ALLOC(count, (uint64_t)kNumCells * 4);
        KM_ALLOC(cell_tot, (uint64_t)kCellGroups * 8 * 2);
        if (points_follow) {
            hipLaunchKernelGGL(k_cell_totals, dim3(kCellGroups), dim3(64), 0, c->stream, cell_count_d, cell_tot.as<uint2>());
            hipLaunchKernelGGL(k_cell_scan, dim3(kCellGroups), dim3(64), 0, c->stream, cell_count_d, (const uint2 *)cell_tot.as<uint2>(), s->cell_start.as<uint32_t>(),
                               (uint32_t *)nullptr, s->ne_cell.as<uint32_t>(), s->ne_start.as<uint32_t>(), s->ne_cost.as<uint32_t>(),
                               s->ne_count.as<uint32_t>(), kCellFixedCost, kCellSweepCost);
        } else if (rank_table_d) {
            const uint32_t *cnt = cell_count_d;
            if (!cnt) {
                hipLaunchKernelGGL(k_cells_count_tbl, dim3(kNumCells), dim3(512), 0, c->stream, rank_table_d, count.as<uint32_t>());
                cnt = count.as<uint32_t>();
            }
            hipLaunchKernelGGL(k_cell_totals, dim3(kCellGroups), dim3(64), 0, c->stream, cnt, cell_tot.as<uint2>());
            hipLaunchKernelGGL(k_cell_scan, dim3(kCellGroups), dim3(64), 0, c->stream, cnt, (const uint2 *)cell_tot.as<uint2>(), s->cell_start.as<uint32_t>(),
                               (uint32_t *)nullptr, s->ne_cell.as<uint32_t>(), s->ne_start.as<uint32_t>(), s->ne_cost.as<uint32_t>(),
                               s->ne_count.as<uint32_t>(), kCellFixedCost, kCellSweepCost);
            if (s->wide)
                hipLaunchKernelGGL(k_cells_write_tbl<uint16_t>, dim3(kNumCells), dim3(512), 0, c->stream, rank_table_d, weight_d,
                                   s->cell_start.as<uint32_t>(), Ulist, K, s->ckeys.as<uint32_t>(), s->cweight.as<uint32_t>(),
                                   s->crank.as<uint32_t>(), s->labels.as<uint16_t>(), s->gidx);
            else
                hipLaunchKernelGGL(k_cells_write_tbl<uint8_t>, dim3(kNumCells), dim3(512), 0, c->stream, rank_table_d, weight_d,
                                   s->cell_start.as<uint32_t>(), Ulist, K, s->ckeys.as<uint32_t>(), s->cweight.as<uint32_t>(),
                                   s->crank.as<uint32_t>(), s->labels.as<uint8_t>(), s->gidx);
        } else {
            KM_ALLOC(cursor, (uint64_t)kNumCells * 4);
            (void)hipMemsetAsync(count.p, 0, (uint64_t)kNumCells * 4, c->stream);
            const uint32_t g = grid_1d(U);
            hipLaunchKernelGGL(k_cell_count, dim3(g), dim3(256), 0, c->stream, keys_d, U, count.as<uint32_t>());
            hipLaunchKernelGGL(k_cell_totals, dim3(kCellGroups), dim3(64), 0, c->stream, count.as<uint32_t>(), cell_tot.as<uint2>());
            hipLaunchKernelGGL(k_cell_scan, dim3(kCellGroups), dim3(64), 0, c->stream, count.as<uint32_t>(), (const uint2 *)cell_tot.as<uint2>(), s->cell_start.as<uint32_t>(),
                               cursor.as<uint32_t>(), s->ne_cell.as<uint32_t>(), s->ne_start.as<uint32_t>(), s->ne_cost.as<uint32_t>(),
                               s->ne_count.as<uint32_t>(), kCellFixedCost, kCellSweepCost);
            hipLaunchKernelGGL(k_cell_scatter, dim3(g), dim3(256), 0, c->stream, keys_d, weight_d, U, cursor.as<uint32_t>(),
                               s->ckeys.as<uint32_t>(), s->cweight.as<uint32_t>(), s->crank.as<uint32_t>());
            if (s->wide)
                hipLaunchKernelGGL(k_rgbw_init_labels<uint16_t>, dim3(grid_1d(U)), dim3(256), 0, c->stream, s->crank.as<uint32_t>(), U,
                                   (uint64_t)0, U, K, s->labels.as<uint16_t>());
            else
                hipLaunchKernelGGL(k_rgbw_init_labels<uint8_t>, dim3(grid_1d(U)), dim3(256), 0, c->stream, s->crank.as<uint32_t>(), U,
                                   (uint64_t)0, U, K, s->labels.as<uint8_t>());
        }
        s->wfirst_waves = G;
        if (s->fused && nshards == 1 && c->ps_div <= 1 && c->opt(CNIIC_OPT_KM_LOOP, "CNIIC_KM_LOOP", 0) == 0) {
            const int rc_ps = ps_prepare(s);
            if (rc_ps != CNIIC_OK) { delete s; return rc_ps; }
        }
        hipError_t e = hipGetLastError();
        if (e != hipSuccess) { delete s; return c->fail(CNIIC_ERR_HIP, "kmeans_rgbw setup: %s", hipGetErrorString(e)); }
    } else {
        s->nblocks = (uint32_t)std::min<uint64_t>(std::max<uint64_t>(ceil_div(n, (uint64_t)kAssignThreads * kPPT), 1), kMaxBlocks);
        KM_ALLOC(s->labels, std::max<uint64_t>(n, 1) * lab_bytes);
        KM_ALLOC(s->slabs, (uint64_t)s->nblocks * W * 8);
        if (s->wide)
            hipLaunchKernelGGL(k_rgbw_init_labels<uint16_t>, dim3(grid_1d(n)), dim3(256), 0, c->stream, (const uint32_t *)nullptr, U, lo,
                               hi, K, s->labels.as<uint16_t>());
        else
            hipLaunchKernelGGL(k_rgbw_init_labels<uint8_t>, dim3(grid_1d(n)), dim3(256), 0, c->stream, (const uint32_t *)nullptr, U, lo,
                               hi, K, s->labels.as<uint8_t>());
    }
    hipError_t e = hipGetLastError();
    if (e != hipSuccess) { delete s; return c->fail(CNIIC_ERR_HIP, "kmeans_rgbw init launch: %s", hipGetErrorString(e)); }
    *out = s;
    return CNIIC_OK;
}

void km_rgbw_destroy(KmRgbwState *s) { delete s; }

static int launch_update(KmRgbwState *s, int mode) {
    Ctx *c = s->c;
    hipLaunchKernelGGL(k_rgbw_update, dim3(1), dim3(256), 0, c->stream, s->partials, s->running.as<uint64_t>(), mode, s->keys,
                       s->gidx.bits ? s->gidx.U : s->U,
                       s->K, s->idbits, s->seed, s->max_iters, s->cconst.as<uint2>(), s->cent.as<uint32_t>(),
                       s->members_last.as<uint64_t>(), s->wsum_last.as<uint64_t>(), s->cells ? s->moved_list.as<uint32_t>() : nullptr,
                       s->dstate.as<KmDevState>(), s->gidx);
    CNIIC_HIP_TRY(c, hipGetLastError());
    return CNIIC_OK;
}

int km_rgbw_set_centroids(KmRgbwState *s, const uint8_t *init_h) {
    Ctx *c = s->c;
    if (s->started) return c->fail(CNIIC_ERR_BAD_ARG, "kmeans_rgbw: the centroids can only be given before the first assign");
    s->given_h.resize(s->K);
    for (uint32_t k = 0; k < s->K; k++) s->given_h[k] = ((uint32_t)init_h[3 * k] << 16) | ((uint32_t)init_h[3 * k + 1] << 8) | init_h[3 * k + 2];
    if (!s->given.p) CNIIC_HIP_TRY(c, s->given.alloc((uint64_t)s->K * 4));
    CNIIC_HIP_TRY(c, hipMemcpyAsync(s->given.p, s->given_h.data(), (size_t)s->K * 4, hipMemcpyHostToDevice, c->stream));
    hipLaunchKernelGGL(k_rgbw_given_cent, dim3(ceil_div(s->Kpad, 256)), dim3(256), 0, c->stream, (const uint32_t *)s->given.as<uint32_t>(), s->K, s->Kpad, s->idbits,
                       s->cconst.as<uint2>(), s->cent.as<uint32_t>(), s->fused ? s->fused_cent.as<uint32_t>() : (uint32_t *)nullptr);
    CNIIC_HIP_TRY(c, hipGetLastError());
    return CNIIC_OK;
}

int km_rgbw_fold_initial(KmRgbwState *) { return CNIIC_OK; }

int km_rgbw_set_state(KmRgbwState *s, const uint8_t *centroids_h, const uint32_t *labels_d_u32) {
    Ctx *c = s->c;
    if (s->cells) return c->fail(CNIIC_ERR_BAD_ARG, "km_rgbw_set_state needs the brute-force state");
    std::vector<uint32_t> ck(s->K);
    for (uint32_t k = 0; k < s->K; k++)
        ck[k] = ((uint32_t)centroids_h[3 * k] << 16) | ((uint32_t)centroids_h[3 * k + 1] << 8) | centroids_h[3 * k + 2];
    CNIIC_HIP_TRY(c, hipMemcpyAsync(s->cent.p, ck.data(), (size_t)s->K * 4, hipMemcpyHostToDevice, c->stream));
    hipLaunchKernelGGL(k_set_cconst, dim3(ceil_div(s->Kpad, 256)), dim3(256), 0, c->stream, s->cent.as<uint32_t>(), s->K,
                       s->Kpad, s->idbits, s->cconst.as<uint2>());
    const uint64_t n = s->hi - s->lo;
    if (n) {
        if (s->wide)
            hipLaunchKernelGGL(k_narrow_labels<uint16_t>, dim3(grid_1d(n)), dim3(256), 0, c->stream, labels_d_u32, s->labels.as<uint16_t>(), n);
        else
            hipLaunchKernelGGL(k_narrow_labels<uint8_t>, dim3(grid_1d(n)), dim3(256), 0, c->stream, labels_d_u32, s->labels.as<uint8_t>(), n);
    }
    CNIIC_HIP_TRY(c, hipGetLastError());
    CNIIC_HIP_TRY(c, hipStreamSynchronize(c->stream));
    return CNIIC_OK;
}

static void ensure_wave_ranges(KmRgbwState *s) {
    if (!s->wfirst_waves) return;
    hipLaunchKernelGGL(k_wave_ranges, dim3(ceil_div((uint64_t)s->wfirst_waves + 1, 256)), dim3(256), 0, s->c->stream, s->ne_cost.as<uint32_t>(),
                       s->ne_count.as<uint32_t>(), s->wfirst_waves, s->wfirst.as<uint32_t>());
    s->wfirst_waves = 0;
}

static void launch_assign(KmRgbwState *s, hipEvent_t ev_start = nullptr, hipEvent_t ev_stop = nullptr, const FusedUpdate *fused = nullptr,
                          unsigned long long *part_fused = nullptr) {
    Ctx *c = s->c;
    s->started = true;
    if (s->cells) ensure_wave_ranges(s);
    FusedUpdate fz{};
    if (fused) fz = *fused;
    const KmDevState *st = s->dstate.as<KmDevState>();
    if (s->cells) {
        auto *part = fused ? part_fused : reinterpret_cast<unsigned long long *>(s->partials);
        CellState cs{s->cell_rec.as<uint32_t>(), s->moved_list.as<uint32_t>(), s->no_skip ? 0u : s->max_skip};
        if (s->big) {
            launch_rgbw_assign_big(c, s->ckeys.as<uint32_t>(), s->cweight.as<uint32_t>(), s->U, s->K, s->cent.as<uint32_t>(), s->labels.as<uint16_t>(), part, st);
        } else if (s->wide) {
            auto lds_for = [&](uint32_t wv) {
                return (size_t)s->K * (5 * 8 + 8) + (size_t)wv * (km_scap(s->K) + km_ccap(s->K)) * 8 + (size_t)wv * ((s->K + 63) / 64) * 8;
            };
            uint32_t wv = 8;
            while (wv > 1 && (lds_for(wv) > 150 * 1024 || s->nblocks % wv)) wv >>= 1;
            const size_t lds = lds_for(wv);
            auto kern = wv == 8 ? k_rgbw_assign_cells<uint16_t, 12, 8> : wv == 4 ? k_rgbw_assign_cells<uint16_t, 12, 4>
                        : wv == 2 ? k_rgbw_assign_cells<uint16_t, 12, 2> : k_rgbw_assign_cells<uint16_t, 12, 1>;
            hipLaunchKernelGGL(kern, dim3(s->nblocks / wv), dim3(64 * wv), lds, c->stream,
                               (const uint32_t *)s->ckeys.as<uint32_t>(), (const uint32_t *)s->cweight.as<uint32_t>(), (const uint32_t *)s->ne_cell.as<uint32_t>(),
// ... 390 lines not shown
```

### cniic_amd/csrc/k_points.hip

```cpp
#include "common.hpp"
#include "device_utils.hpp"

namespace cniic {

constexpr uint32_t kSpBuckets = 512;
constexpr uint32_t kSpBins = 1u << 15;
constexpr uint32_t kSpChunk = 1u << 16;
constexpr int kSpThreads = 1024;
constexpr uint32_t kSpSliceMin = 1u << 17;
constexpr uint32_t kSpSlices = 8;
constexpr uint32_t kSpWaves = kSpThreads / 64;

__device__ __forceinline__ uint32_t sp_bucket(uint32_t key) {
    return (((key >> 21) & 7u) << 6) | (((key >> 13) & 7u) << 3) | ((key >> 5) & 7u);
}
__device__ __forceinline__ uint32_t sp_bin(uint32_t key) {
    const uint32_t r = (key >> 16) & 31u, g = (key >> 8) & 31u, b = key & 31u;
    return ((r >> 3) << 13) | ((g >> 3) << 11) | ((b >> 3) << 9) | ((r & 7u) << 6) | ((g & 7u) << 3) | (b & 7u);
}
__device__ __forceinline__ uint32_t sp_key(uint32_t bucket, uint32_t bin) {
    const uint32_t r = (((bucket >> 6) & 7u) << 5) | (((bin >> 13) & 3u) << 3) | ((bin >> 6) & 7u);
    const uint32_t g = (((bucket >> 3) & 7u) << 5) | (((bin >> 11) & 3u) << 3) | ((bin >> 3) & 7u);
    const uint32_t b = ((bucket & 7u) << 5) | (((bin >> 9) & 3u) << 3) | (bin & 7u);
    return (r << 16) | (g << 8) | b;
}

__device__ __forceinline__ uint32_t scan512(uint32_t v, uint32_t *wsum) { return block_exclusive_scan<kSpThreads>(v, wsum); }

template <typename F> __device__ __forceinline__ void sp_for_pixels(const uint8_t *__restrict__ rgb, uint64_t npx, F &&f) {
    const uint64_t p0 = (uint64_t)blockIdx.x * kSpChunk, p1 = min(npx, p0 + kSpChunk);
    const uint4 *v = reinterpret_cast<const uint4 *>(rgb);
    for (uint64_t g = p0 / 16 + threadIdx.x; g * 16 < p1; g += kSpThreads) {
        uint32_t key[16];
        if (g * 16 + 16 <= p1) {
            load16px_keys(v + 3 * g, key);
            f(g * 16, key, 16u);
        } else {
            const uint32_t m = (uint32_t)(p1 - g * 16);
            for (uint32_t i = 0; i < 16; i++) key[i] = i < m ? rgb_key(rgb + 3 * (g * 16 + i)) : 0u;
            f(g * 16, key, m);
        }
    }
}

__global__ __launch_bounds__(kSpThreads) void k_sp_count(const uint8_t *__restrict__ rgb, uint64_t npx, uint32_t *__restrict__ cnt) {
    __shared__ uint32_t h[kSpBuckets];
    if (threadIdx.x < kSpBuckets) h[threadIdx.x] = 0;
    __syncthreads();
    sp_for_pixels(rgb, npx, [&](uint64_t, const uint32_t (&key)[16], uint32_t m) {
#pragma unroll
        for (uint32_t i = 0; i < 16; i++)
            if (i < m) atomicAdd(&h[sp_bucket(key[i])], 1u);
    });
    __syncthreads();
    if (threadIdx.x < kSpBuckets) cnt[(size_t)blockIdx.x * kSpBuckets + threadIdx.x] = h[threadIdx.x];
}

__global__ __launch_bounds__(256) void k_sp_colscan(const uint32_t *__restrict__ cnt, uint32_t nchunks, uint32_t *__restrict__ pre,
                                                    uint32_t *__restrict__ total) {
    __shared__ uint32_t wsum[256 / 64];
    const uint32_t b = blockIdx.x, per = (nchunks + 255) / 256;
    const uint32_t c0 = threadIdx.x * per, c1 = min(c0 + per, nchunks);
    uint32_t s = 0;
    for (uint32_t c = c0; c < c1; c++) s += cnt[(size_t)c * kSpBuckets + b];
    uint32_t run = block_exclusive_scan<256>(s, wsum);
    for (uint32_t c = c0; c < c1; c++) {
        pre[(size_t)c * kSpBuckets + b] = run;
        run += cnt[(size_t)c * kSpBuckets + b];
    }
    if (threadIdx.x == 255) total[b] = run;
}

__global__ __launch_bounds__(kSpBuckets) void k_sp_bstart(const uint32_t *__restrict__ total, uint32_t *__restrict__ bstart,
                                                          uint32_t *__restrict__ sstart) {
    __shared__ uint32_t wsum[kSpBuckets / 64];
    const uint32_t t = total[threadIdx.x];
    const uint32_t ex = block_exclusive_scan<kSpBuckets>(t, wsum);
    bstart[threadIdx.x] = ex;
    if (threadIdx.x == kSpBuckets - 1) bstart[kSpBuckets] = ex + t;
    sstart[threadIdx.x] = block_exclusive_scan<kSpBuckets>(min(t, kSpBins), wsum);
}

template <int STEPS, typename F> __device__ __forceinline__ void sp_walk_sorted(const uint32_t *off, uint32_t n, F &&f) {
    const uint32_t lane = threadIdx.x & 63, wv = threadIdx.x >> 6;
    const uint32_t per = (n + kSpThreads - 1) / kSpThreads * 64;
    const uint32_t j0 = wv * per, j1 = min(n, j0 + per);
    if (j0 >= j1) return;
    const uint32_t jj = min(j0 + lane, j1 - 1);
    uint32_t lo = 0, hi = kSpBuckets;
    while (hi - lo > 1) {
        const uint32_t mid = (lo + hi) >> 1;
        if (off[mid] <= jj) lo = mid; else hi = mid;
    }
    uint32_t b = lo, end = off[b + 1];
    for (uint32_t j = j0 + lane; j < j1; j += 64 * STEPS) {
        uint32_t jb[STEPS];
#pragma unroll
        for (int t = 0; t < STEPS; t++) {
            const uint32_t q = j + 64 * t;
            jb[t] = 0xffffffffu;
            if (q < j1) {
                while (q >= end) { b++; end = off[b + 1]; }
                jb[t] = b;
            }
        }
        f(j, jb);
    }
}

__global__ __launch_bounds__(kSpThreads) void k_sp_scatter(const uint8_t *__restrict__ rgb, uint64_t npx, const uint32_t *__restrict__ cnt,
                                                           const uint32_t *__restrict__ pre, const uint32_t *__restrict__ bstart,
                                                           uint16_t *__restrict__ part, uint16_t *__restrict__ prank) {
    extern __shared__ __align__(16) uint8_t sp_lds[];
    uint16_t *stage = reinterpret_cast<uint16_t *>(sp_lds);
    uint32_t *off = reinterpret_cast<uint32_t *>(sp_lds + (size_t)kSpChunk * 2);
    uint32_t *cur = off + kSpBuckets + 1;
    __shared__ uint32_t wsum[kSpWaves];
    const uint32_t *mycnt = cnt + (size_t)blockIdx.x * kSpBuckets;
    const uint32_t n_b = threadIdx.x < kSpBuckets ? mycnt[threadIdx.x] : 0u;
    const uint32_t ex = scan512(n_b, wsum);
    if (threadIdx.x < kSpBuckets) { off[threadIdx.x] = ex; cur[threadIdx.x] = 0; }
    if (threadIdx.x == kSpBuckets - 1) off[kSpBuckets] = ex + n_b;
    __syncthreads();
    sp_for_pixels(rgb, npx, [&](uint64_t first, const uint32_t (&key)[16], uint32_t m) {
        uint32_t rk[16];
#pragma unroll
        for (uint32_t i = 0; i < 16; i++) {
            rk[i] = 0;
            if (i < m) {
                const uint32_t b = sp_bucket(key[i]);
                rk[i] = off[b] + atomicAdd(&cur[b], 1u);
                stage[rk[i]] = (uint16_t)sp_bin(key[i]);
            }
        }
        if (m == 16) {
            uint4 *d = reinterpret_cast<uint4 *>(prank + first);
            d[0] = make_uint4(rk[0] | (rk[1] << 16), rk[2] | (rk[3] << 16), rk[4] | (rk[5] << 16), rk[6] | (rk[7] << 16));
            d[1] = make_uint4(rk[8] | (rk[9] << 16), rk[10] | (rk[11] << 16), rk[12] | (rk[13] << 16), rk[14] | (rk[15] << 16));
        } else {
            for (uint32_t i = 0; i < m; i++) prank[first + i] = (uint16_t)rk[i];
        }
    });
    __syncthreads();
    const uint32_t lane = threadIdx.x & 63, wv = threadIdx.x >> 6;
    const uint32_t *mypre = pre + (size_t)blockIdx.x * kSpBuckets;
    const uint32_t mb = wv + kSpWaves * (lane & 31);
    const uint32_t m_n = mycnt[mb], m_dst = bstart[mb] + mypre[mb], m_off = off[mb];
    for (uint32_t k = 0; k < kSpBuckets / kSpWaves; k++) {
        const uint32_t n = __shfl(m_n, k, 64), d0 = __shfl(m_dst, k, 64), o = __shfl(m_off, k, 64);
        for (uint32_t i = lane; i < n; i += 64) part[(size_t)d0 + i] = stage[o + i];
    }
}

template <typename F> __device__ __forceinline__ void sp_for_entries(const uint16_t *__restrict__ part, uint64_t s, uint64_t e, F &&f) {
    const uint64_t a = min(e, (s + 3) & ~3ull), z = a + ((e - a) & ~3ull);
    for (uint64_t i = s + threadIdx.x; i < a; i += kSpThreads) { const uint32_t v = part[i]; f(i, v, v, v, v, 1u); }
    constexpr uint64_t kStep = 4 * (uint64_t)kSpThreads;
    for (uint64_t i = a + 4 * (uint64_t)threadIdx.x; i < z; i += 4 * kStep) {
        uint2 q[4];
#pragma unroll
        for (int t = 0; t < 4; t++) q[t] = i + t * kStep < z ? *reinterpret_cast<const uint2 *>(part + i + t * kStep) : make_uint2(0u, 0u);
#pragma unroll
        for (int t = 0; t < 4; t++)
            if (i + t * kStep < z) f(i + t * kStep, q[t].x & 0xffffu, q[t].x >> 16, q[t].y & 0xffffu, q[t].y >> 16, 4u);
    }
    for (uint64_t i = z + threadIdx.x; i < e; i += kSpThreads) { const uint32_t v = part[i]; f(i, v, v, v, v, 1u); }
}

__device__ __forceinline__ void sp_bucket_hist(const uint16_t *__restrict__ part, uint64_t s, uint64_t e, uint32_t *hist) {
    for (uint32_t i = threadIdx.x; i < kSpBins; i += kSpThreads) hist[i] = 0;
    __syncthreads();
    sp_for_entries(part, s, e, [&](uint64_t, uint32_t a, uint32_t b, uint32_t c, uint32_t d, uint32_t m) {
        if (m == 1) { atomicAdd(&hist[a], 1u); return; }
        const bool same = a == b && b == c && c == d;
        const uint32_t first = __builtin_amdgcn_readfirstlane(a);
        if (__all(same && a == first) && __popcll(__ballot(1)) == 64) {
            if ((threadIdx.x & 63) == 0) atomicAdd(&hist[a], 256u);
        } else if (same) {
            atomicAdd(&hist[a], 4u);
        } else {
            atomicAdd(&hist[a], 1u); atomicAdd(&hist[b], 1u); atomicAdd(&hist[c], 1u); atomicAdd(&hist[d], 1u);
        }
    });
    __syncthreads();
}


__global__ __launch_bounds__(kSpThreads) void k_sp_hist(const uint16_t *__restrict__ part, const uint32_t *__restrict__ bstart,
                                                        const uint32_t *__restrict__ sstart, uint32_t *__restrict__ cell_count,
                                                        uint32_t *__restrict__ bits32, uint16_t *__restrict__ sbin,
                                                        uint32_t *__restrict__ scnt) {
    extern __shared__ __align__(16) uint8_t sp_lds[];
    uint32_t *hist = reinterpret_cast<uint32_t *>(sp_lds);
    __shared__ uint32_t wsum[kSpWaves];
    const uint32_t bucket = blockIdx.x;
    const uint64_t s = bstart[bucket], e = bstart[bucket + 1];
    const uint32_t r5 = threadIdx.x >> 5, g5 = threadIdx.x & 31;
    const uint32_t word_at = ((((bucket >> 6) & 7u) << 5 | r5) << 11) | ((((bucket >> 3) & 7u) << 5 | g5) << 3) | (bucket & 7u);
    if (s == e) {
        if (threadIdx.x < 64) cell_count[bucket * 64 + threadIdx.x] = 0;
        bits32[word_at] = 0;
        return;
    }
    sp_bucket_hist(part, s, e, hist);
    uint32_t word = 0;
#pragma unroll
    for (uint32_t bq = 0; bq < 4; bq++) {
        const uint32_t base = ((r5 >> 3) << 13) | ((g5 >> 3) << 11) | (bq << 9) | ((r5 & 7u) << 6) | ((g5 & 7u) << 3);
#pragma unroll
        for (uint32_t j = 0; j < 8; j++) word |= (hist[base + j] != 0 ? 1u : 0u) << (bq * 8 + j);
    }
    bits32[word_at] = word;
    const uint32_t lane = threadIdx.x & 63, wv = threadIdx.x >> 6;
    const unsigned long long lt_mask = (1ull << lane) - 1ull;
    uint32_t mine = 0;
    for (uint32_t c4 = 0; c4 < 4; c4++) {
        uint32_t in_cell = 0;
        for (uint32_t st = 0; st < 8; st++) in_cell += (uint32_t)__popcll(__ballot(hist[wv * 2048 + c4 * 512 + st * 64 + lane] != 0));
        if (lane == 0) cell_count[bucket * 64 + wv * 4 + c4] = in_cell;
        mine += in_cell;
    }
    if (lane == 0) wsum[wv] = mine;
    __syncthreads();
    uint32_t pos0 = sstart[bucket];
    for (uint32_t i = 0; i < wv; i++) pos0 += wsum[i];
    for (uint32_t st = 0; st < 32; st++) {
        const uint32_t bin = wv * 2048 + st * 64 + lane, v = hist[bin];
        const unsigned long long bm = __ballot(v != 0);
        if (v) {
            const uint32_t pos = pos0 + (uint32_t)__popcll(bm & lt_mask);
            sbin[pos] = (uint16_t)bin;
            scnt[pos] = v;
        }
        pos0 += (uint32_t)__popcll(bm);
    }
}

struct SpEmit {
    const uint32_t *cell_start;
    uint32_t *ckeys, *cweight;
    void *labels;
    uint32_t K, wide;
    GIdx gx;
    const uint64_t *U_dev;
};

constexpr uint32_t kSpEmitSplit = 4;
__global__ __launch_bounds__(256) void k_sp_emit(const uint32_t *__restrict__ sstart, const uint16_t *__restrict__ sbin,
                                                 const uint32_t *__restrict__ scnt, SpEmit em) {
    const uint32_t bucket = blockIdx.x / kSpEmitSplit, part_no = blockIdx.x % kSpEmitSplit;
    const uint32_t q0 = em.cell_start[bucket * 64], n = em.cell_start[bucket * 64 + 64] - q0, s0 = sstart[bucket];
    const uint32_t U = em.U_dev ? (uint32_t)*em.U_dev : (uint32_t)em.gx.U, ppc = max(U / em.K, 1u);
    const float rcp = 1.0f / (float)ppc;
    constexpr uint32_t kStride = 256 * kSpEmitSplit;
    for (uint32_t i0 = part_no * 256 + threadIdx.x; i0 < n; i0 += 4 * kStride) {
        uint32_t key[4], cnt[4], rank[4];
#pragma unroll
        for (int t = 0; t < 4; t++) {
            const uint32_t i = i0 + t * kStride;
            key[t] = i < n ? sp_key(bucket, sbin[s0 + i]) : 0u;
            cnt[t] = i < n ? scnt[s0 + i] : 0u;
        }
#pragma unroll
        for (int t = 0; t < 4; t++) rank[t] = i0 + t * kStride < n ? gidx_rank(em.gx, key[t]) : 0u;
#pragma unroll
        for (int t = 0; t < 4; t++) {
            const uint32_t i = i0 + t * kStride;
            if (i >= n) continue;
            em.ckeys[q0 + i] = key[t];
            em.cweight[q0 + i] = cnt[t];
            const uint32_t lab = init_label24(rank[t], U, em.K, ppc, rcp);
            if (em.wide) static_cast<uint16_t *>(em.labels)[q0 + i] = (uint16_t)lab;
            else static_cast<uint8_t *>(em.labels)[q0 + i] = (uint8_t)lab;
        }
    }
}

__global__ __launch_bounds__(256) void k_bits_prefix(const unsigned long long *__restrict__ bits, uint32_t *__restrict__ wprefix,
                                                     uint32_t *__restrict__ blocktot) {
    __shared__ uint32_t wsum[256 / 64];
    const uint32_t w0 = (blockIdx.x * 256 + threadIdx.x) * 4;
    uint32_t cnt[4], mine = 0;
#pragma unroll
    for (int q = 0; q < 4; q++) { cnt[q] = (uint32_t)__popcll(bits[w0 + q]); mine += cnt[q]; }
    uint32_t run = block_exclusive_scan<256>(mine, wsum);
#pragma unroll
    for (int q = 0; q < 4; q++) { wprefix[w0 + q] = run; run += cnt[q]; }
    if (threadIdx.x == 255) blocktot[blockIdx.x] = run;
}

template <typename LabelT>
__global__ __launch_bounds__(kSpThreads) void k_sp_partlab(const uint16_t *__restrict__ part, const uint32_t *__restrict__ bstart,
                                                           const uint32_t *__restrict__ cell_start, const uint32_t *__restrict__ ckeys,
                                                           const LabelT *__restrict__ labels, LabelT *__restrict__ partlab,
                                                           unsigned long long *__restrict__ look = nullptr, uint32_t look_words = 0) {
    extern __shared__ __align__(16) uint8_t sp_lds[];
    LabelT *lut = reinterpret_cast<LabelT *>(sp_lds);
    if (look && blockIdx.x == 0 && blockIdx.y == 0)
        for (uint32_t i = threadIdx.x; i < look_words; i += kSpThreads) look[i] = 0ull;
    const uint32_t bucket = blockIdx.x;
    uint64_t s = bstart[bucket], e = bstart[bucket + 1];
    if (s == e) return;
    {
        const uint64_t len = e - s;
        const uint32_t slices = (uint32_t)min<uint64_t>(gridDim.y, max<uint64_t>(1, len / kSpSliceMin));
        if (blockIdx.y >= slices) return;
        const uint64_t per = ((len + slices - 1) / slices + 3) & ~3ull;
        const uint64_t a = s + per * blockIdx.y;
        e = min(e, a + per);
        s = a;
        if (s >= e) return;
    }
    const uint32_t q0 = cell_start[bucket * 64], q1 = cell_start[bucket * 64 + 64];
    for (uint32_t i = q0 + threadIdx.x; i < q1; i += kSpThreads) lut[sp_bin(ckeys[i])] = labels[i];
    __syncthreads();
    sp_for_entries(part, s, e, [&](uint64_t i, uint32_t a, uint32_t b, uint32_t c, uint32_t d, uint32_t m) {
        if (m == 1) { partlab[i] = lut[a]; return; }
        if (sizeof(LabelT) == 1) {
            *reinterpret_cast<uint32_t *>(partlab + i) = (uint32_t)lut[a] | ((uint32_t)lut[b] << 8) | ((uint32_t)lut[c] << 16) | ((uint32_t)lut[d] << 24);
        } else {
            *reinterpret_cast<uint2 *>(partlab + i) = make_uint2((uint32_t)lut[a] | ((uint32_t)lut[b] << 16), (uint32_t)lut[c] | ((uint32_t)lut[d] << 16));
        }
    });
}

template <typename LabelT>
__device__ __forceinline__ void sp_stage_labels(uint32_t chunk, const uint32_t *__restrict__ cnt, const uint32_t *__restrict__ pre,
                                                const uint32_t *__restrict__ bstart, const LabelT *__restrict__ partlab, LabelT *stage,
                                                uint32_t *off, uint32_t *gsrc, uint32_t *wsum) {
    const uint32_t *mycnt = cnt + (size_t)chunk * kSpBuckets, *mypre = pre + (size_t)chunk * kSpBuckets;
    const uint32_t n_b = threadIdx.x < kSpBuckets ? mycnt[threadIdx.x] : 0u;
    const uint32_t ex = scan512(n_b, wsum);
    if (threadIdx.x < kSpBuckets) off[threadIdx.x] = ex;
    if (threadIdx.x == kSpBuckets - 1) off[kSpBuckets] = ex + n_b;
    __syncthreads();
    if (threadIdx.x < kSpBuckets) gsrc[threadIdx.x] = bstart[threadIdx.x] + mypre[threadIdx.x] - off[threadIdx.x];
    __syncthreads();
    sp_walk_sorted<8>(off, off[kSpBuckets], [&](uint32_t j, const uint32_t (&jb)[8]) {
        LabelT got[8];
#pragma unroll
        for (int t = 0; t < 8; t++) got[t] = jb[t] != 0xffffffffu ? partlab[(size_t)(gsrc[jb[t]] + (j + 64 * t))] : (LabelT)0;
#pragma unroll
        for (int t = 0; t < 8; t++)
            if (jb[t] != 0xffffffffu) stage[j + 64 * t] = got[t];
    });
    __syncthreads();
}

template <typename LabelT>
__global__ __launch_bounds__(kSpThreads) void k_sp_pixlab(const uint8_t *__restrict__ rgb, uint64_t npx, const uint32_t *__restrict__ cnt,
                                                          const uint32_t *__restrict__ pre, const uint32_t *__restrict__ bstart,
                                                          const LabelT *__restrict__ partlab, const uint16_t *__restrict__ prank,
                                                          LabelT *__restrict__ pixlab) {
    extern __shared__ __align__(16) uint8_t sp_lds[];
    LabelT *stage = reinterpret_cast<LabelT *>(sp_lds);
    uint32_t *off = reinterpret_cast<uint32_t *>(sp_lds + (size_t)kSpChunk * sizeof(LabelT));
    uint32_t *gsrc = off + kSpBuckets + 1;
    __shared__ uint32_t wsum[kSpWaves];
    sp_stage_labels(blockIdx.x, cnt, pre, bstart, partlab, stage, off, gsrc, wsum);
    const uint64_t p0 = (uint64_t)blockIdx.x * kSpChunk, p1 = min(npx, p0 + kSpChunk);
    for (uint64_t g = p0 / 16 + threadIdx.x; g * 16 < p1; g += kSpThreads) {
        const uint64_t first = g * 16;
        const uint32_t m = (uint32_t)min<uint64_t>(16, p1 - first);
        uint32_t lab[16];
        if (m == 16) {
            const uint4 *rp = reinterpret_cast<const uint4 *>(prank + first);
            const uint4 r0 = rp[0], r1 = rp[1];
            const uint32_t rw[8] = {r0.x, r0.y, r0.z, r0.w, r1.x, r1.y, r1.z, r1.w};
#pragma unroll
            for (uint32_t i = 0; i < 16; i++) lab[i] = stage[(rw[i >> 1] >> (16 * (i & 1))) & 0xffffu];
            if (sizeof(LabelT) == 1) {
// ... 104 lines not shown
        unsigned long long mine = 0;
        if (chunk == 0) {
            if (tid == 0) look_st(&W[0], kLookInc | total);
        } else {
            if (tid == 0) look_st(&W[chunk], kLookAgg | total);
            const unsigned long long t0 = wall_clock64();
            long long hi = (long long)chunk - 1;
            for (bool found = false; !found; hi -= 64 * kLookPer) {
                unsigned long long v[kLookPer];
                for (uint32_t spins = 0;;) {
                    bool ready = true;
#pragma unroll
                    for (uint32_t k = 0; k < kLookPer; k++) {
                        const long long j = hi - (long long)(tid + 64 * k);
                        v[k] = j >= 0 ? look_ld(&W[j]) : kLookInc;
                        ready = ready && (v[k] >> 62) != 0;
                    }
                    if (a.test_giveup) { ok = false; break; }
                    if (__all(ready)) break;
                    __builtin_amdgcn_s_sleep(1);
                    if ((++spins & 63u) == 0 && __any(__hip_atomic_load(giveup, __ATOMIC_RELAXED, __HIP_MEMORY_SCOPE_AGENT) != 0u || wall_clock64() - t0 > a.timeout_ticks)) { ok = false; break; }
                }
                if (!ok) break;
#pragma unroll
                for (uint32_t k = 0; k < kLookPer; k++) {
                    const bool there = hi - (long long)(tid + 64 * k) >= 0;
                    const unsigned long long inc = __ballot(there && (v[k] >> 62) == 2);
                    const uint32_t nearest = inc ? (uint32_t)__builtin_ctzll(inc) : 64u;
                    if (!found && there && tid <= nearest) mine += v[k] & kLookMask;
                    found = found || inc != 0;
                }
            }
        }
        const unsigned long long sum = wave_inclusive_scan64<false>(mine);
        if (tid == 63) {
            if (!ok) {
                __hip_atomic_store(giveup, 1u, __ATOMIC_RELAXED, __HIP_MEMORY_SCOPE_AGENT);
                s_ok = 0u;
            } else {
                s_excl = sum;
                if (chunk) look_st(&W[chunk], kLookInc | (sum + total));
                if (chunk == a.nchunks - 1) look_st(a.look + 2, sum + total);
            }
        }
    }
    __syncthreads();
    if (!s_ok) return;
    const uint64_t g0 = a.bit_base + s_excl;
    uint32_t run = 0;
#pragma unroll
    for (uint32_t r = 0; r < kSpPackRounds; r++) {
        const uint64_t first = p0 + ((uint64_t)tid + kSpThreads * r) * 16;
        const uint32_t m = first < p1 ? (uint32_t)min<uint64_t>(16, p1 - first) : 0u;
        uint32_t lab[16], l[16];
#pragma unroll
        for (uint32_t i = 0; i < 16; i++) {
            lab[i] = (lw[r][i >> 2] >> (8 * (i & 3))) & 255u;
            l[i] = i < m ? (uint32_t)s_len[lab[i]] : 0u;
        }
        uint32_t before = 0, rtot = 0;
#pragma unroll
        for (uint32_t i = 0; i < kSpWaves; i++) { const uint32_t v = s_rsum[r][i]; rtot += v; if (i < wid) before += v; }
        pack_emit<kSpThreads, 16>(lab, l, before + wexcl[r], rtot, g0 + run, s_tab, img, min(kSpPackImgWords, a.img_cap), a.out_words);
        run += rtot;
        __syncthreads();
    }
}

static int sp_set_lds(Ctx *c) {
    static bool done = false;
    if (done) return CNIIC_OK;
    const int big = 140 * 1024;
    CNIIC_HIP_TRY(c, hipFuncSetAttribute(reinterpret_cast<const void *>(k_sp_scatter), hipFuncAttributeMaxDynamicSharedMemorySize, big));
    CNIIC_HIP_TRY(c, hipFuncSetAttribute(reinterpret_cast<const void *>(k_sp_hist), hipFuncAttributeMaxDynamicSharedMemorySize, big));
    CNIIC_HIP_TRY(c, hipFuncSetAttribute(reinterpret_cast<const void *>(k_sp_partlab<uint8_t>), hipFuncAttributeMaxDynamicSharedMemorySize, big));
    CNIIC_HIP_TRY(c, hipFuncSetAttribute(reinterpret_cast<const void *>(k_sp_partlab<uint16_t>), hipFuncAttributeMaxDynamicSharedMemorySize, big));
    CNIIC_HIP_TRY(c, hipFuncSetAttribute(reinterpret_cast<const void *>(k_sp_pixlab<uint8_t>), hipFuncAttributeMaxDynamicSharedMemorySize, big));
    CNIIC_HIP_TRY(c, hipFuncSetAttribute(reinterpret_cast<const void *>(k_sp_pixlab<uint16_t>), hipFuncAttributeMaxDynamicSharedMemorySize, big));
    CNIIC_HIP_TRY(c, hipFuncSetAttribute(reinterpret_cast<const void *>(k_sp_pixpack), hipFuncAttributeMaxDynamicSharedMemorySize, (int)kSpPackDyn));
    done = true;
    return CNIIC_OK;
}

int sp_build(Ctx *c, const uint8_t *rgb_d, uint64_t npx, SpPlan *plan) {
    if (npx == 0 || (reinterpret_cast<uintptr_t>(rgb_d) & 15)) return c->fail(CNIIC_ERR_BAD_ARG, "sp_build: empty or unaligned image");
    CNIIC_TRY(sp_set_lds(c));
    plan->npx = npx;
    plan->nchunks = (uint32_t)ceil_div(npx, kSpChunk);
    const uint64_t nc = plan->nchunks;
    CNIIC_HIP_TRY(c, plan->cnt.alloc(nc * kSpBuckets * 4));
    CNIIC_HIP_TRY(c, plan->pre.alloc(nc * kSpBuckets * 4));
    CNIIC_HIP_TRY(c, plan->bstart.alloc(((uint64_t)kSpBuckets + 1) * 4));
    CNIIC_HIP_TRY(c, plan->part.alloc(npx * 2 + 16));
    CNIIC_HIP_TRY(c, plan->prank.alloc((npx + 16) * 2));
    CNIIC_HIP_TRY(c, plan->cell_count.alloc((uint64_t)kNumCells * 4));
    const uint64_t smax = std::min<uint64_t>(npx, 1ull << 24);
    CNIIC_HIP_TRY(c, plan->sstart.alloc((uint64_t)kSpBuckets * 4));
    CNIIC_HIP_TRY(c, plan->sbin.alloc(smax * 2));
    CNIIC_HIP_TRY(c, plan->scnt.alloc(smax * 4));
    CNIIC_HIP_TRY(c, plan->bits.alloc((1ull << 18) * 8));
    CNIIC_HIP_TRY(c, plan->wprefix.alloc((1ull << 18) * 4));
    DevBuf total, blocktot;
    CNIIC_HIP_TRY(c, total.alloc((uint64_t)kSpBuckets * 4));
    CNIIC_HIP_TRY(c, blocktot.alloc(256 * 4));
    CNIIC_HIP_TRY(c, plan->total.alloc(8));
    CNIIC_HIP_TRY(c, c->pinned_u.reserve(kPinnedUBytes, kPinnedUBytes));
    CNIIC_HIP_TRY(c, c->u_ev.ensure(hipEventDisableTiming));
    hipLaunchKernelGGL(k_sp_count, dim3(plan->nchunks), dim3(kSpThreads), 0, c->stream, rgb_d, npx, plan->cnt.as<uint32_t>());
    hipLaunchKernelGGL(k_sp_colscan, dim3(kSpBuckets), dim3(256), 0, c->stream, plan->cnt.as<uint32_t>(), plan->nchunks,
                       plan->pre.as<uint32_t>(), total.as<uint32_t>());
    hipLaunchKernelGGL(k_sp_bstart, dim3(1), dim3(kSpBuckets), 0, c->stream, total.as<uint32_t>(), plan->bstart.as<uint32_t>(),
                       plan->sstart.as<uint32_t>());
    hipLaunchKernelGGL(k_sp_scatter, dim3(plan->nchunks), dim3(kSpThreads), (size_t)kSpChunk * 2 + kSpBuckets * 8 + 16, c->stream, rgb_d, npx,
                       plan->cnt.as<uint32_t>(), plan->pre.as<uint32_t>(), plan->bstart.as<uint32_t>(), plan->part.as<uint16_t>(),
                       plan->prank.as<uint16_t>());
    hipLaunchKernelGGL(k_sp_hist, dim3(kSpBuckets), dim3(kSpThreads), (size_t)kSpBins * 4, c->stream, plan->part.as<uint16_t>(),
                       plan->bstart.as<uint32_t>(), plan->sstart.as<uint32_t>(), plan->cell_count.as<uint32_t>(), plan->bits.as<uint32_t>(),
                       plan->sbin.as<uint16_t>(), plan->scnt.as<uint32_t>());
    hipLaunchKernelGGL(k_bits_prefix, dim3(256), dim3(256), 0, c->stream, plan->bits.as<unsigned long long>(), plan->wprefix.as<uint32_t>(),
                       blocktot.as<uint32_t>());
    CNIIC_TRY(gidx_finish(c, plan->wprefix.as<uint32_t>(), blocktot.as<uint32_t>(), plan->total.as<uint64_t>()));
    CNIIC_HIP_TRY(c, hipGetLastError());
    CNIIC_HIP_TRY(c, hipMemcpyAsync(c->pinned_u.as<uint64_t>() + kPuSpCount.at, plan->total.p, 8, hipMemcpyDeviceToHost, c->stream));
    CNIIC_HIP_TRY(c, hipEventRecord(c->u_ev, c->stream));
    return CNIIC_OK;
}

int sp_wait_count(Ctx *c, SpPlan *plan) {
    CNIIC_HIP_TRY(c, hipEventSynchronize(c->u_ev));
    plan->U = c->pinned_u.as<uint64_t>()[kPuSpCount.at];
    return CNIIC_OK;
}

int sp_emit(Ctx *c, const SpPlan *plan, const uint32_t *cell_start_d, uint32_t *ckeys_d, uint32_t *cweight_d, void *labels_d, bool wide,
            uint32_t K, const void *gbits_d, const uint32_t *gprefix_d, uint64_t Ug, const uint64_t *Ug_dev) {
    const GIdx gx{static_cast<const unsigned long long *>(gbits_d), gprefix_d, Ug};
    hipLaunchKernelGGL(k_sp_emit, dim3(kSpBuckets * kSpEmitSplit), dim3(256), 0, c->stream, plan->sstart.as<uint32_t>(), plan->sbin.as<uint16_t>(),
                       plan->scnt.as<uint32_t>(), SpEmit{cell_start_d, ckeys_d, cweight_d, labels_d, K, wide ? 1u : 0u, gx, Ug_dev});
    CNIIC_HIP_TRY(c, hipGetLastError());
    return CNIIC_OK;
}

__global__ __launch_bounds__(256) void k_occ_from_bits(const uint32_t *__restrict__ bits32, uint32_t *__restrict__ occ) {
    const uint32_t i = blockIdx.x * 256 + threadIdx.x;
    const uint32_t byte = (bits32[i >> 2] >> (8 * (i & 3))) & 255u;
    uint32_t v = 0;
#pragma unroll
    for (int j = 0; j < 8; j++) v |= ((byte >> j) & 1u) << (4 * j);
    occ[i] = v;
}
int sp_occupancy(Ctx *c, const SpPlan *plan, uint32_t *occ_d) {
    hipLaunchKernelGGL(k_occ_from_bits, dim3((1u << 21) / 256), dim3(256), 0, c->stream, plan->bits.as<uint32_t>(), occ_d);
    CNIIC_HIP_TRY(c, hipGetLastError());
    return CNIIC_OK;
}

int sp_part_labels(Ctx *c, const SpPlan *plan, const uint32_t *cell_start_d, const uint32_t *ckeys_d, const void *labels_d, bool wide, DevBuf &partlab,
                   DevBuf *look) {
    const uint64_t lb = wide ? 2 : 1;
    CNIIC_HIP_TRY(c, partlab.alloc(plan->npx * lb + 16));
    const uint32_t look_words = look ? plan->nchunks + kLookHead : 0;
    if (look) CNIIC_HIP_TRY(c, look->alloc((uint64_t)look_words * 8));
    const dim3 grid(kSpBuckets, plan->npx >= 2 * (uint64_t)kSpSliceMin ? kSpSlices : 1);
    if (wide)
        hipLaunchKernelGGL(k_sp_partlab<uint16_t>, grid, dim3(kSpThreads), (size_t)kSpBins * 2, c->stream, plan->part.as<uint16_t>(),
                           plan->bstart.as<uint32_t>(), cell_start_d, ckeys_d, static_cast<const uint16_t *>(labels_d), partlab.as<uint16_t>(),
                           (unsigned long long *)nullptr, 0u);
    else
        hipLaunchKernelGGL(k_sp_partlab<uint8_t>, grid, dim3(kSpThreads), (size_t)kSpBins, c->stream, plan->part.as<uint16_t>(),
                           plan->bstart.as<uint32_t>(), cell_start_d, ckeys_d, static_cast<const uint8_t *>(labels_d), partlab.as<uint8_t>(),
                           look ? look->as<unsigned long long>() : nullptr, look_words);
    CNIIC_HIP_TRY(c, hipGetLastError());
    return CNIIC_OK;
}

int sp_pixlab(Ctx *c, const SpPlan *plan, const uint8_t *rgb_d, const void *partlab_d, bool wide, void *pixlab_d) {
    if (wide)
        hipLaunchKernelGGL(k_sp_pixlab<uint16_t>, dim3(plan->nchunks), dim3(kSpThreads), (size_t)kSpChunk * 2 + kSpBuckets * 8 + 16, c->stream, rgb_d,
                           plan->npx, plan->cnt.as<uint32_t>(), plan->pre.as<uint32_t>(), plan->bstart.as<uint32_t>(), static_cast<const uint16_t *>(partlab_d),
                           plan->prank.as<uint16_t>(), static_cast<uint16_t *>(pixlab_d));
    else
        hipLaunchKernelGGL(k_sp_pixlab<uint8_t>, dim3(plan->nchunks), dim3(kSpThreads), (size_t)kSpChunk + kSpBuckets * 8 + 16, c->stream, rgb_d,
                           plan->npx, plan->cnt.as<uint32_t>(), plan->pre.as<uint32_t>(), plan->bstart.as<uint32_t>(), static_cast<const uint8_t *>(partlab_d),
                           plan->prank.as<uint16_t>(), static_cast<uint8_t *>(pixlab_d));
    CNIIC_HIP_TRY(c, hipGetLastError());
    return CNIIC_OK;
}

int sp_pixel_labels(Ctx *c, const SpPlan *plan, const uint8_t *rgb_d, const uint32_t *cell_start_d, const uint32_t *ckeys_d,
                    const void *labels_d, bool wide, void *pixlab_d) {
    DevBuf partlab;
    CNIIC_TRY(sp_part_labels(c, plan, cell_start_d, ckeys_d, labels_d, wide, partlab, nullptr));
    return sp_pixlab(c, plan, rgb_d, partlab.p, wide, pixlab_d);
}

int sp_pixpack(Ctx *c, const SpPlan *plan, const void *partlab_d, DevBuf &look, const uint8_t *upl_h, uint32_t hdr_bytes, uint8_t *out_d, uint64_t *done_h) {
    if (reinterpret_cast<uintptr_t>(out_d) & 3) return c->fail(CNIIC_ERR_BAD_ARG, "sp_pixpack: output must be 4-byte aligned");
    CNIIC_TRY(sp_set_lds(c));
    SpPackArgs a{};
    a.cnt = plan->cnt.as<uint32_t>(); a.pre = plan->pre.as<uint32_t>(); a.bstart = plan->bstart.as<uint32_t>();
    a.partlab = static_cast<const uint8_t *>(partlab_d); a.prank = plan->prank.as<uint16_t>();
    a.npx = plan->npx; a.nchunks = plan->nchunks; a.img_cap = pack_img_cap();
    a.upl = upl_h; a.hdr_bytes = hdr_bytes; a.out_words = reinterpret_cast<uint32_t *>(out_d); a.bit_base = (uint64_t)hdr_bytes * 8;
    a.look = look.as<unsigned long long>();
    a.timeout_ticks = 2000ull * 100000ull;
    a.test_giveup = test_env("CNIIC_TEST_CC_TAIL_GIVEUP") ? 1u : 0u;
    hipLaunchKernelGGL(k_sp_pixpack, dim3(plan->nchunks), dim3(kSpThreads), kSpPackDyn, c->stream, a);
    CNIIC_HIP_TRY(c, hipGetLastError());
// ... 6 lines not shown
```

### cniic_amd/csrc/kmeans_rgbw.hpp

```cpp
#pragma once
#include <cstdlib>
#include <memory>
#include <vector>

#include "common.hpp"
#include "device_utils.hpp"

namespace cniic {

constexpr uint32_t kBias = 1u << 18;
constexpr int kPPT = 8;
constexpr int kAssignThreads = 256;
constexpr uint32_t kMaxBlocks = 512;
constexpr int kCellWaves = 8;
__host__ __device__ constexpr uint32_t km_scap(uint32_t K) { return K <= 256 ? (K + 1) / 2 : (K + 1) / 2 < 512u ? (K + 1) / 2 : 512u; }
__host__ __device__ constexpr uint32_t km_ccap(uint32_t K) { return K <= 256 ? K : 256u; }
constexpr uint32_t kCellWavesBig = 12;
constexpr uint32_t kBigBlocksFrom = 10;
constexpr uint32_t kAggLaunches = 3;
constexpr uint32_t kCellBlocks = 256 * 3;
constexpr int kSweep = 4;
constexpr uint32_t kCellFixedCost = 512;
constexpr uint32_t kCellSweepCost = 256;

struct KmRgbwState {
    Ctx *c = nullptr;
    uint64_t U = 0, lo = 0, hi = 0, seed = 0, max_iters = 0;
    uint32_t K = 0, Kpad = 0, idbits = 8, nblocks = 1;
    bool wide = false;
    bool big = false;
    bool cells = true;
    bool profile = false;
    bool no_skip = false;
    const uint32_t *keys = nullptr, *weight = nullptr;
    DevBuf labels;
    DevBuf cconst, slabs, partials_own, dstate, cent, members_last, wsum_last;
    DevBuf arena;
    DevBuf resblk;
    uint64_t res_cent = 0, res_members = 0, res_wsum = 0, res_bytes = 0;
    std::unique_ptr<LaggedPoll> lagged;
    DevBuf ckeys, cweight, crank, cell_start, running, ne_cell, ne_start, ne_cost, ne_count, wfirst;
    DevBuf cell_rec, moved_list;
    uint32_t wfirst_waves = 0;
    GIdx gidx{nullptr, nullptr, 0};
    DevBuf fused_partials, fused_running, fused_cent;
    bool fused = false;
    cniic_kmeans_stats run_stats{};
    bool run_stats_valid = false;
    uint32_t max_skip = 64;
    long fail_at = -1;
    uint32_t shard = 0, nshards = 1;
    uint64_t *partials = nullptr;
    bool ps = false, ps_tried = false;
    bool ps_pending = false;
    std::shared_ptr<void> ps_hold;
    uint32_t ps_blocks = 0;
    DevBuf ps_arena;
    DevBuf ps_pk;
    uint64_t ps_o_part = 0, ps_o_fail = 0, ps_o_rng = 0;
    uint32_t ps_budget = 0;
    bool started = false;
    DevBuf given;
    std::vector<uint32_t> given_h;
};

constexpr uint32_t kPsChunks = 24;
constexpr uint32_t kPsSlotsMax = 32;
constexpr uint32_t kPsScap = 96;
constexpr uint32_t kPsRecWords = 11;
constexpr uint32_t kPsMaxCells = 2048;
constexpr uint32_t kPsOffCell = 5 * 256 * 8 + 256 * 8 + kPsSlotsMax * kPsScap * 4;
constexpr uint32_t kPsDynBytes = 160 * 1024 - 3072;
constexpr uint32_t kPsRunWords = 5 * 256;
constexpr uint32_t kPsBudget = kPsDynBytes - kPsRunWords * 8;
constexpr uint32_t kPsPartWords = 5 * 256 + 8;
__host__ __device__ constexpr uint32_t ps_cell_bytes(uint32_t C) { return 16u + ((C + 3u) & ~3u) * (4u + 4u + kPsRecWords * 4u + 2u + 2u + 1u); }
static_assert(kPsOffCell + ps_cell_bytes(kPsMaxCells) <= kPsBudget, "a full block's descriptors fit the budget");
struct alignas(128) PsLine { uint32_t v; uint32_t pad[31]; };
struct PsBar { PsLine xcount[8], xgen[8], xblocks[8], top, topgen, count, gen, abort_; };
struct PsDevPtrs {
    const uint32_t *ckeys, *cweight;
    uint8_t *labels;
    const uint32_t *ne_cell, *ne_start;
    const uint2 *cconst0;
};
struct PsDev { uint32_t fail, pad; PsDevPtrs p; };
constexpr uint32_t kPsArenaPart = (sizeof(PsBar) + 255u) & ~255u, kPsArenaFail = kPsArenaPart + ((3u * kPsPartWords * 8u + 255u) & ~255u), kPsArenaRng = kPsArenaFail + 256u;
static_assert(sizeof(PsDev) <= 256, "PsDev has 256 bytes of the arena");
constexpr uint32_t kPsStatusDone = 1, kPsStatusAborted = 2, kPsStatusRanges = 3;
struct PsExit { uint32_t status, pad; uint64_t iter, moved_last, reseeds, active, pair_evals; };
void launch_rgbw_assign_big(Ctx *c, const uint32_t *ckeys, const uint32_t *cweight, uint64_t U, uint32_t K, const uint32_t *cent, uint16_t *labels,
                            unsigned long long *partials, const KmDevState *st);
int ps_prepare(KmRgbwState *s);
int km_rgbw_run_persistent(KmRgbwState *s, bool *ran, bool may_defer);
int km_rgbw_persistent_verdict(KmRgbwState *s, bool *retry);
constexpr uint32_t kAggMin = 16;


__device__ __forceinline__ uint32_t dot4u8(uint32_t a, uint32_t b, uint32_t acc) {
    return __builtin_amdgcn_udot4(a, b, acc, false);
}

__device__ __forceinline__ uint2 make_cconst(uint32_t ckey, uint32_t k, uint32_t idbits) {
    uint32_t h = dot4u8(ckey, ckey, 0);
    uint32_t idmask = (1u << idbits) - 1;
    return make_uint2(ckey, ((kBias - h) << idbits) | (idmask - k));
}

struct CellBox { int32_t r0, g0, b0; };
__device__ __forceinline__ CellBox super_box(uint32_t sup) {
    return CellBox{(int32_t)((sup / (kSupersPerDim * kSupersPerDim)) << (kCellShift + 2)),
                   (int32_t)(((sup / kSupersPerDim) % kSupersPerDim) << (kCellShift + 2)),
                   (int32_t)((sup % kSupersPerDim) << (kCellShift + 2))};
}
__device__ __forceinline__ CellBox cell_box(uint32_t c) {
    const CellBox sb = super_box(c >> kSuperShift);
    return CellBox{sb.r0 + (int32_t)(((c >> 4) & 3) << kCellShift), sb.g0 + (int32_t)(((c >> 2) & 3) << kCellShift),
                   sb.b0 + (int32_t)((c & 3) << kCellShift)};
}

constexpr uint32_t kRecComplete = 0x80000000u;
__host__ __device__ constexpr uint32_t cell_rec_words(uint32_t MW) { return (2 + 2 * MW + 15) & ~15u; }
constexpr uint32_t kMaxMovedSkip = 64;

__device__ __forceinline__ uint32_t pack_rgb(int32_t r, int32_t g, int32_t b) { return ((uint32_t)r << 16) | ((uint32_t)g << 8) | (uint32_t)b; }

__device__ __forceinline__ uint32_t centre_dist(uint32_t ck, const CellBox &bx, int32_t ext) {
    const int32_t h = (ext + 1) >> 1;
    const uint32_t c = pack_rgb(bx.r0 + h, bx.g0 + h, bx.b0 + h);
    return dot4u8(ck, ck, dot4u8(c, c, 0)) - 2u * dot4u8(ck, c, 0);
}

struct Dominance {
    uint32_t ppk, lopk, hipk;
    int32_t cp, ext;
    __device__ __forceinline__ void set(const CellBox &bx, int32_t e, uint32_t pivot) {
        ppk = pivot & 0xffffffu;
        ext = e;
        lopk = pack_rgb(bx.r0, bx.g0, bx.b0);
        hipk = pack_rgb(bx.r0 + e, bx.g0 + e, bx.b0 + e);
        cp = (int32_t)dot4u8(ppk, ppk, 0) - 2 * (int32_t)dot4u8(ppk, lopk, 0) - e * (int32_t)dot4u8(ppk, 0x010101u, 0);
    }
    __device__ __forceinline__ int32_t worst(uint32_t ck) const {
        const uint32_t v = ck;
        return cp - (int32_t)dot4u8(v, v, 0) + (int32_t)dot4u8(v, hipk, dot4u8(v, lopk, 0)) + __mul24(ext, (int32_t)__builtin_amdgcn_sad_u8(ppk, v, 0u));
    }
};

__device__ __forceinline__ uint32_t wave_all_min(uint32_t v) { return wave_reduce_min(v); }

__device__ __forceinline__ uint32_t nearest_to_centre(const uint2 *list, uint32_t n, const CellBox &bx, int32_t ext, int lane) {
    uint32_t bd = 0xfffffu, be = 4095u;
    for (uint32_t e = lane; e < n; e += 64) {
        const uint32_t d = centre_dist(list[e].x, bx, ext);
        if (d < bd) { bd = d; be = e; }
    }
    return wave_all_min((bd << 12) | be) & 4095u;
}

__device__ __forceinline__ uint32_t lanes_below(unsigned long long bm) {
    return __builtin_amdgcn_mbcnt_hi((uint32_t)(bm >> 32), __builtin_amdgcn_mbcnt_lo((uint32_t)bm, 0u));
}

__device__ __forceinline__ uint32_t build_super(const uint2 *tab, uint32_t K, uint32_t sup, int lane, unsigned long long lt_mask,
                                                uint2 *S, uint32_t cap) {
    constexpr int32_t ext = (1 << (kCellShift + 2)) - 1;
    const CellBox bx = super_box(sup);
    Dominance dm;
    dm.set(bx, ext, tab[nearest_to_centre(tab, K, bx, ext, lane)].x);
    uint32_t n = 0;
    for (uint32_t k0 = 0; k0 < K; k0 += 64) {
        const uint32_t k = k0 + lane;
        uint2 cc = make_uint2(0u, 0u);
        bool keep = false;
        if (k < K) { cc = tab[k]; keep = dm.worst(cc.x) >= 0; }
        const unsigned long long bm = __ballot(keep);
        const uint32_t pos = n + lanes_below(bm);
        if (keep && pos < cap) S[pos] = cc;
        n += (uint32_t)__popcll(bm);
    }
    __builtin_amdgcn_wave_barrier();
    return n;
}

__device__ __forceinline__ uint32_t pk_make(uint32_t key, uint32_t w, uint32_t label) {
    return (((key >> 16) & 7u) << 6) | (((key >> 8) & 7u) << 3) | (key & 7u) | (min(w, 255u) << 16) | (label << 24);
}
__device__ __forceinline__ uint32_t pk_key(uint32_t pw, uint32_t cell_base) {
    return cell_base | ((pw & 0x1c0u) << 10) | ((pw & 0x38u) << 5) | (pw & 7u);
}
// ... 7 lines not shown
```

Before: 10420 Mpixels/s.

## Fuse cluster-colors set-up launches into three combined front kernels

Moves the device-side bodies of the k-means set-up kernels (centroid init, cell totals/scan, persistent ranges, prefix finish) into shared inline functions. A deferred create path hands them to new fused front kernels, which also take over the arena memsets when the buffers are 16-byte aligned. The aim is to cut the number of kernel launches and memset calls in the encode set-up, reducing launch overhead and serialization. The cost is extra complexity and an alignment-based fallback to the split path.

```diff
diff --git a/cniic_amd/csrc/codec.cpp b/cniic_amd/csrc/codec.cpp
--- a/cniic_amd/csrc/codec.cpp
+++ b/cniic_amd/csrc/codec.cpp
@@ -14,6 +14,7 @@
 #include <memory>
 
 #include "huff_host.hpp"
+#include "kmeans_rgbw.hpp"
 #include "pal_bounds.hpp"
 
 namespace cniic {
@@ -407,15 +408,19 @@
     if (K == 0) return c->fail(CNIIC_ERR_BAD_ARG, "cluster-colors(0)");
     auto s = std::make_unique<CcSession>();
     s->c = c; s->K = K; s->sp_mode = true;
-    CNIIC_TRY(sp_build(c, rgb_d, npx, &s->sp));
+    CNIIC_TRY(sp_build(c, rgb_d, npx, &s->sp, true));
     const uint64_t Umax = std::min<uint64_t>(npx, 1ull << 24);
     const uint64_t *U_dev = s->sp.total.as<uint64_t>();
-    CNIIC_TRY(km_rgbw_create(c, nullptr, nullptr, Umax, 0, 1, K, opts, nullptr, nullptr, &s->km, s->sp.cell_count.as<uint32_t>(), s->sp.bits.p,
-                             s->sp.wprefix.as<uint32_t>(), Umax, true, U_dev));
+    KmFront front;
+    CNIIC_TRY(km_rgbw_create_deferred(c, Umax, K, opts, &s->km, s->sp.cell_count.as<uint32_t>(), s->sp.bits.p, s->sp.wprefix.as<uint32_t>(), Umax, U_dev, &front));
     uint32_t *cell_start, *ckeys, *cweight;
     km_rgbw_cell_arrays(s->km, &cell_start, &ckeys, &cweight);
-    CNIIC_TRY(sp_emit(c, &s->sp, cell_start, ckeys, cweight, km_rgbw_labels_internal(s->km, nullptr), km_rgbw_is_wide(s->km), K, s->sp.bits.p,
-                      s->sp.wprefix.as<uint32_t>(), 0, U_dev));
+    bool fused = sp_front_fits(front);
+    if (const char *e = test_env("CNIIC_TEST_CC_FRONT")) {
+        if (!fused && !strcmp(e, "require")) return c->fail(CNIIC_ERR_HIP, "cluster-colors: the fused set-up launches cannot clear the K-means arenas (CNIIC_TEST_CC_FRONT=require)");
+        fused = fused && strcmp(e, "split") != 0;
+    }
+    CNIIC_TRY(sp_front(c, &s->sp, front, ckeys, cweight, km_rgbw_labels_internal(s->km, nullptr), km_rgbw_is_wide(s->km), fused));
     CNIIC_TRY(sp_wait_count(c, &s->sp));
     s->U = s->sp.U;
     if (s->U / K == 0)
diff --git a/cniic_amd/csrc/common.hpp b/cniic_amd/csrc/common.hpp
--- a/cniic_amd/csrc/common.hpp
+++ b/cniic_amd/csrc/common.hpp
@@ -517,7 +517,10 @@
     DevBuf bits, wprefix;
     DevBuf total;
 };
-int sp_build(Ctx *c, const uint8_t *rgb_d, uint64_t npx, SpPlan *plan);
+int sp_build(Ctx *c, const uint8_t *rgb_d, uint64_t npx, SpPlan *plan, bool hist_only = false);
+struct KmFront;
+int sp_front(Ctx *c, SpPlan *plan, const KmFront &f, uint32_t *ckeys_d, uint32_t *cweight_d, void *labels_d, bool wide, bool fused);
+bool sp_front_fits(const KmFront &f);
 int sp_wait_count(Ctx *c, SpPlan *plan);
 int sp_emit(Ctx *c, const SpPlan *plan, const uint32_t *cell_start_d, uint32_t *ckeys_d, uint32_t *cweight_d, void *labels_d, bool wide,
             uint32_t K, const void *gbits_d, const uint32_t *gprefix_d, uint64_t Ug, const uint64_t *Ug_dev );
diff --git a/cniic_amd/csrc/device_utils.hpp b/cniic_amd/csrc/device_utils.hpp
--- a/cniic_amd/csrc/device_utils.hpp
+++ b/cniic_amd/csrc/device_utils.hpp
@@ -238,6 +238,27 @@
     for (uint32_t r = (uint32_t)(idx - g.wprefix[a]); r; r--) word &= word - 1;
     return (a << 6) | (uint32_t)(__ffsll((long long)word) - 1);
 }
+__device__ __forceinline__ void bits_prefix_body(uint32_t blk, const unsigned long long *__restrict__ bits, uint32_t *__restrict__ wprefix,
+                                                 uint32_t *__restrict__ blocktot, uint32_t *wsum) {
+    const uint32_t w0 = (blk * 256 + threadIdx.x) * 4;
+    uint32_t cnt[4], mine = 0;
+#pragma unroll
+    for (int q = 0; q < 4; q++) { cnt[q] = (uint32_t)__popcll(bits[w0 + q]); mine += cnt[q]; }
+    uint32_t run = block_exclusive_scan<256>(mine, wsum);
+#pragma unroll
+    for (int q = 0; q < 4; q++) { wprefix[w0 + q] = run; run += cnt[q]; }
+    if (threadIdx.x == 255) blocktot[blk] = run;
+}
+__device__ __forceinline__ void gidx_finish_body(uint32_t blk, uint32_t *__restrict__ wprefix, const uint32_t *__restrict__ blocktot,
+                                                 uint64_t *__restrict__ total, uint32_t *wsum, uint32_t *boff) {
+    const uint32_t t = blocktot[threadIdx.x];
+    const uint32_t ex = block_exclusive_scan<256>(t, wsum);
+    boff[threadIdx.x] = ex;
+    if (blk == 0 && threadIdx.x == 255) *total = (uint64_t)ex + t;
+    __syncthreads();
+    const uint32_t add = boff[blk];
+    for (uint32_t i = threadIdx.x; i < 1024; i += 256) wprefix[blk * 1024 + i] += add;
+}
 
 __host__ __device__ __forceinline__ uint64_t splitmix_mix(uint64_t z) {
     z = (z ^ (z >> 30)) * 0xBF58476D1CE4E5B9ULL;
diff --git a/cniic_amd/csrc/k_hist.hip b/cniic_amd/csrc/k_hist.hip
--- a/cniic_amd/csrc/k_hist.hip
+++ b/cniic_amd/csrc/k_hist.hip
@@ -365,13 +365,7 @@
                                                      uint64_t *__restrict__ total) {
     __shared__ uint32_t wsum[256 / 64];
     __shared__ uint32_t boff[256];
-    const uint32_t t = blocktot[threadIdx.x];
-    const uint32_t ex = block_exclusive_scan<256>(t, wsum);
-    boff[threadIdx.x] = ex;
-    if (blockIdx.x == 0 && threadIdx.x == 255) *total = (uint64_t)ex + t;
-    __syncthreads();
-    const uint32_t add = boff[blockIdx.x];
-    for (uint32_t i = threadIdx.x; i < 1024; i += 256) wprefix[blockIdx.x * 1024 + i] += add;
+    gidx_finish_body(blockIdx.x, wprefix, blocktot, total, wsum, boff);
 }
 
 int gidx_finish(Ctx *c, uint32_t *wprefix_d, const uint32_t *blocktot_d, uint64_t *total_d) {
diff --git a/cniic_amd/csrc/k_kmeans_persist.hip b/cniic_amd/csrc/k_kmeans_persist.hip
--- a/cniic_amd/csrc/k_kmeans_persist.hip
+++ b/cniic_amd/csrc/k_kmeans_persist.hip
@@ -60,41 +60,7 @@
 
 __global__ __launch_bounds__(1024) void k_ps_ranges(const uint32_t *__restrict__ ne_cost, const uint32_t *__restrict__ ne_count, uint32_t G, uint32_t dyn_bytes,
                                                     uint32_t *__restrict__ cb, PsDev *__restrict__ dev, PsDevPtrs ptrs) {
-    uint32_t *fail = &dev->fail;
-    if (threadIdx.x == 0) dev->p = ptrs;
-    const uint32_t M = *ne_count, NC = G * kPsChunks;
-    const uint64_t total = ne_cost[M];
-    for (uint32_t g0 = threadIdx.x; g0 <= NC; g0 += 8 * blockDim.x) {
-        uint32_t a[8], b[8];
-        uint64_t c_lo[8];
-#pragma unroll
-        for (int r = 0; r < 8; r++) {
-            const uint32_t g = g0 + r * blockDim.x;
-            c_lo[r] = total * min(g, NC) / NC;
-            a[r] = 0; b[r] = g <= NC ? M : 0u;
-        }
-        bool more = true;
-        while (more) {
-            more = false;
-            uint32_t mid[8], v[8];
-#pragma unroll
-            for (int r = 0; r < 8; r++) { mid[r] = (a[r] + b[r]) >> 1; v[r] = a[r] < b[r] ? ne_cost[mid[r]] : 0u; }
-#pragma unroll
-            for (int r = 0; r < 8; r++)
-                if (a[r] < b[r]) { if (v[r] < c_lo[r]) a[r] = mid[r] + 1; else b[r] = mid[r]; more = more || a[r] < b[r]; }
-        }
-#pragma unroll
-        for (int r = 0; r < 8; r++) {
-            const uint32_t g = g0 + r * blockDim.x;
-            if (g <= NC) cb[g] = g == NC ? M : a[r];
-        }
-    }
-    __syncthreads();
-    for (uint32_t g = threadIdx.x; g < G; g += blockDim.x) {
-        uint32_t C = 0;
-        for (uint32_t r = 0; r < kPsChunks; r++) C += cb[r * G + g + 1] - cb[r * G + g];
-        if (C > kPsMaxCells || kPsOffCell + ps_cell_bytes(C) > dyn_bytes) atomicAdd(fail, 1u);
-    }
+    ps_ranges_body(ne_cost, ne_count, G, dyn_bytes, cb, dev, ptrs);
 }
 
 template <class Op> __device__ __forceinline__ uint32_t row_allreduce(uint32_t v, Op op) {
@@ -916,8 +882,9 @@
     c->ps_backoff_left = c->ps_backoff;
 }
 
-int ps_prepare(KmRgbwState *s) {
+int ps_decide(KmRgbwState *s, PsSetup *out) {
     Ctx *c = s->c;
+    *out = PsSetup{};
     if (c->ps_backoff_left && !test_env("CNIIC_KM_PS_REQUIRE")) { c->ps_backoff_left--; return CNIIC_OK; }
     const uint32_t G = ps_grid_for(c, s->U);
     if (!G) return CNIIC_OK;
@@ -928,7 +895,6 @@
     }
     const uint64_t o_part = kPsArenaPart, o_fail = kPsArenaFail, o_rng = kPsArenaRng, total = o_rng + ((uint64_t)G * kPsChunks + 1) * 4;
     CNIIC_HIP_TRY(c, s->ps_arena.alloc(total));
-    CNIIC_HIP_TRY(c, hipMemsetAsync(s->ps_arena.p, 0, o_rng, c->stream));
     CNIIC_HIP_TRY(c, s->ps_pk.alloc(std::max<uint64_t>(s->U, 1) * 4));
     s->ps_blocks = G;
     s->ps_o_part = o_part; s->ps_o_fail = o_fail; s->ps_o_rng = o_rng;
@@ -939,10 +905,20 @@
     PsDevPtrs ptrs{};
     ptrs.ckeys = s->ckeys.as<uint32_t>(); ptrs.cweight = s->cweight.as<uint32_t>(); ptrs.labels = s->labels.as<uint8_t>();
     ptrs.ne_cell = s->ne_cell.as<uint32_t>(); ptrs.ne_start = s->ne_start.as<uint32_t>(); ptrs.cconst0 = s->cconst.as<uint2>();
-    hipLaunchKernelGGL(k_ps_ranges, dim3(1), dim3(1024), 0, c->stream, (const uint32_t *)s->ne_cost.as<uint32_t>(), (const uint32_t *)s->ne_count.as<uint32_t>(), G, budget,
-                       reinterpret_cast<uint32_t *>(a + o_rng), reinterpret_cast<PsDev *>(a + o_fail), ptrs);
+    out->on = true; out->G = G; out->budget = budget; out->ptrs = ptrs;
+    out->cb = reinterpret_cast<uint32_t *>(a + o_rng); out->dev = reinterpret_cast<PsDev *>(a + o_fail);
+    out->zero_p = a; out->zero_bytes = o_rng;
+    s->ps = true;
+    return CNIIC_OK;
+}
+void ps_launch_ranges(Ctx *c, const uint32_t *ne_cost, const uint32_t *ne_count, uint32_t G, uint32_t budget, uint32_t *cb, PsDev *dev, const PsDevPtrs &ptrs) {
+    hipLaunchKernelGGL(k_ps_ranges, dim3(1), dim3(1024), 0, c->stream, ne_cost, ne_count, G, budget, cb, dev, ptrs);
+}
+int ps_enqueue(KmRgbwState *s, const PsSetup &p) {
+    Ctx *c = s->c;
+    CNIIC_HIP_TRY(c, hipMemsetAsync(p.zero_p, 0, p.zero_bytes, c->stream));
+    ps_launch_ranges(c, s->ne_cost.as<uint32_t>(), s->ne_count.as<uint32_t>(), p.G, p.budget, p.cb, p.dev, p.ptrs);
     CNIIC_HIP_TRY(c, hipGetLastError());
-    s->ps = true;
     return CNIIC_OK;
 }
 
diff --git a/cniic_amd/csrc/k_kmeans_rgbw.hip b/cniic_amd/csrc/k_kmeans_rgbw.hip
--- a/cniic_amd/csrc/k_kmeans_rgbw.hip
+++ b/cniic_amd/csrc/k_kmeans_rgbw.hip
@@ -13,19 +13,7 @@
 __global__ void k_rgbw_init_cent(const uint32_t *__restrict__ keys, uint64_t U, uint32_t K, uint32_t Kpad, uint32_t idbits,
                                  uint2 *__restrict__ cconst, uint32_t *__restrict__ cent, GIdx gx, uint32_t *__restrict__ cent_copy,
                                  uint32_t *__restrict__ moved_list, const uint64_t *__restrict__ U_dev) {
-    uint32_t k = blockIdx.x * blockDim.x + threadIdx.x;
-    if (U_dev) U = max(*U_dev, (uint64_t)K);
-    if (k == 0 && moved_list) moved_list[0] = K;
-    if (k < K) {
-        uint64_t ppc = U / K;
-        uint64_t first = (k < K - 1) ? U - ((uint64_t)k + 1) * ppc : 0;
-        uint32_t ck = gx.bits ? gidx_select(gx, first) : keys[first];
-        cent[k] = ck;
-        if (cent_copy) cent_copy[k] = ck;
-        cconst[k] = make_cconst(ck, k, idbits);
-    } else if (k < Kpad) {
-        cconst[k] = make_uint2(0u, 0u);
-    }
+    rgbw_init_cent_body(blockIdx.x * blockDim.x + threadIdx.x, keys, U, K, Kpad, idbits, cconst, cent, gx, cent_copy, moved_list, U_dev);
 }
 
 __global__ void k_rgbw_given_cent(const uint32_t *__restrict__ given , uint32_t K, uint32_t Kpad, uint32_t idbits, uint2 *__restrict__ cconst,
@@ -159,38 +147,15 @@
     }
 }
 
-constexpr uint32_t kCellGroups = kNumCells / 64;
 __global__ __launch_bounds__(64) void k_cell_totals(const uint32_t *__restrict__ cell_count, uint2 *__restrict__ tot) {
-    const uint32_t v = cell_count[blockIdx.x * 64 + threadIdx.x];
-    const uint32_t sum = wave_reduce_sum(v), sweeps = wave_reduce_sum((v + 64 * kSweep - 1) / (64 * kSweep));
-    const uint32_t ne = (uint32_t)__popcll(__ballot(v != 0));
-    if (threadIdx.x == 0) { tot[blockIdx.x] = make_uint2(sum, ne); tot[kCellGroups + blockIdx.x] = make_uint2(sweeps, 0u); }
+    cell_totals_body(blockIdx.x, threadIdx.x, cell_count, tot);
 }
 __global__ __launch_bounds__(64) void k_cell_scan(const uint32_t *__restrict__ cell_count, const uint2 *__restrict__ tot,
                                                   uint32_t *__restrict__ cell_start, uint32_t *__restrict__ cursor,
                                                   uint32_t *__restrict__ ne_cell, uint32_t *__restrict__ ne_start,
                                                   uint32_t *__restrict__ ne_cost, uint32_t *__restrict__ ne_count, uint32_t fixed_cost,
                                                   uint32_t sweep_cost) {
-    const uint32_t lane = threadIdx.x, grp = blockIdx.x;
-    uint32_t ps = 0, pn = 0, pw = 0;
-    for (uint32_t g = lane; g < grp; g += 64) { const uint2 t = tot[g]; ps += t.x; pn += t.y; pw += tot[kCellGroups + g].x; }
-    const uint32_t base = wave_reduce_sum(ps), nbase = wave_reduce_sum(pn), wbase = wave_reduce_sum(pw);
-    const uint32_t cell = grp * 64 + lane, v = cell_count[cell], sw = (v + 64 * kSweep - 1) / (64 * kSweep);
-    const uint32_t start = base + wave_inclusive_scan(v) - v, swb = wbase + wave_inclusive_scan(sw) - sw;
-    cell_start[cell] = start;
-    if (cursor) cursor[cell] = start;
-    const unsigned long long nzm = __ballot(v != 0);
-    if (v) {
-        const uint32_t m = nbase + (uint32_t)__popcll(nzm & ((1ull << lane) - 1ull));
-        ne_cell[m] = cell; ne_start[m] = start; ne_cost[m] = (sweep_cost ? swb * sweep_cost : start) + m * fixed_cost;
-    }
-    if (grp == kCellGroups - 1 && lane == 63) {
-        const uint32_t U = start + v, M = nbase + (uint32_t)__popcll(nzm);
-        cell_start[kNumCells] = U;
-        ne_start[M] = U;
-        ne_cost[M] = (sweep_cost ? (swb + sw) * sweep_cost : U) + M * fixed_cost;
-        *ne_count = M;
-    }
+    cell_scan_body(blockIdx.x, threadIdx.x, cell_count, tot, CellScanOut{cell_start, cursor, ne_cell, ne_start, ne_cost, ne_count}, fixed_cost, sweep_cost);
 }
 
 constexpr uint32_t kCellColours = 1u << (3 * kCellShift);
@@ -1095,11 +1060,12 @@
                                                         (unsigned long long)(bytes), hipGetErrorString(_e)); } \
     } while (0)
 
-int km_rgbw_create(Ctx *c, const uint32_t *keys_d, const uint32_t *weight_d, uint64_t U, uint32_t shard,
-                   uint32_t nshards, uint32_t K, const cniic_kmeans_opts *opts, void *partials_dev,
-                   const uint32_t *rank_table_d, KmRgbwState **out, const uint32_t *cell_count_d, const void *gbits_d,
-                   const uint32_t *gprefix_d, uint64_t Ug, bool points_follow, const uint64_t *points_dev) {
+static int km_create_impl(Ctx *c, const uint32_t *keys_d, const uint32_t *weight_d, uint64_t U, uint32_t shard,
+                          uint32_t nshards, uint32_t K, const cniic_kmeans_opts *opts, void *partials_dev,
+                          const uint32_t *rank_table_d, KmRgbwState **out, const uint32_t *cell_count_d, const void *gbits_d,
+                          const uint32_t *gprefix_d, uint64_t Ug, bool points_follow, const uint64_t *points_dev, KmFront *front) {
     if (K == 0 || U == 0 || nshards == 0 || shard >= nshards) return c->fail(CNIIC_ERR_BAD_ARG, "kmeans_rgbw: bad sizes");
+    if (front && (!points_follow || partials_dev)) return c->fail(CNIIC_ERR_BAD_ARG, "kmeans_rgbw: only the set-up of points written by the caller can be left to it");
     if (points_follow && (!gbits_d || !cell_count_d || nshards != 1 || (opts && (opts->flags & CNIIC_KM_BRUTE_FORCE))))
         return c->fail(CNIIC_ERR_BAD_ARG, "kmeans_rgbw: points written by the caller need the cell counts and the colour index");
     if (!points_follow && gbits_d && (!rank_table_d || nshards != 1 || (opts && (opts->flags & CNIIC_KM_BRUTE_FORCE))))
@@ -1143,7 +1109,8 @@
         const uint64_t o_fr = o_fp + up(s->fused ? 3 * W * 8 : 0), o_fc = o_fr + up(s->fused ? 2 * W * 8 : 0);
         const uint64_t o_mv = o_fc + up(s->fused ? 2 * (uint64_t)K * 4 : 0), total = o_mv + up(s->cells ? ((uint64_t)K + 1) * 4 : 0);
         KM_ALLOC(s->arena, total);
-        (void)hipMemsetAsync(s->arena.p, 0, total, c->stream);
+        if (front) { front->arena = s->arena.p; front->arena_bytes = total; }
+        else (void)hipMemsetAsync(s->arena.p, 0, total, c->stream);
         uint8_t *a = s->arena.as<uint8_t>();
         s->resblk.view(a, s->res_bytes);
         if (partials_dev) {
@@ -1167,9 +1134,16 @@
     s->cent.view(static_cast<uint8_t *>(s->resblk.p) + s->res_cent, (uint64_t)K * 4);
     s->members_last.view(static_cast<uint8_t *>(s->resblk.p) + s->res_members, (uint64_t)K * 8);
     s->wsum_last.view(static_cast<uint8_t *>(s->resblk.p) + s->res_wsum, (uint64_t)K * 8);
-    hipLaunchKernelGGL(k_rgbw_init_cent, dim3(ceil_div(s->Kpad, 256)), dim3(256), 0, c->stream, keys_d, Ulist, K, s->Kpad, s->idbits,
-                       s->cconst.as<uint2>(), s->cent.as<uint32_t>(), s->gidx, s->fused ? s->fused_cent.as<uint32_t>() : (uint32_t *)nullptr,
-                       s->cells ? s->moved_list.as<uint32_t>() : (uint32_t *)nullptr, points_dev);
+    if (front) {
+        front->Ulist = Ulist; front->K = K; front->Kpad = s->Kpad; front->idbits = s->idbits;
+        front->cconst = s->cconst.as<uint2>(); front->cent = s->cent.as<uint32_t>(); front->gx = s->gidx;
+        front->cent_copy = s->fused ? s->fused_cent.as<uint32_t>() : nullptr;
+        front->moved_list = s->moved_list.as<uint32_t>(); front->U_dev = points_dev;
+    } else {
+        hipLaunchKernelGGL(k_rgbw_init_cent, dim3(ceil_div(s->Kpad, 256)), dim3(256), 0, c->stream, keys_d, Ulist, K, s->Kpad, s->idbits,
+                           s->cconst.as<uint2>(), s->cent.as<uint32_t>(), s->gidx, s->fused ? s->fused_cent.as<uint32_t>() : (uint32_t *)nullptr,
+                           s->cells ? s->moved_list.as<uint32_t>() : (uint32_t *)nullptr, points_dev);
+    }
     if (s->cells) {
         s->nblocks = (uint32_t)std::min<uint64_t>(std::max<uint64_t>(ceil_div(U / nshards, s->wide ? 1024 : 64), 1), s->wide ? 4096u : kCellBlocks);
         if (const uint64_t mb = c->opt(CNIIC_OPT_KM_MAX_BLOCKS, "CNIIC_KM_MAX_BLOCKS", 0)) {
@@ -1192,7 +1166,12 @@
         DevBuf count, cursor, cell_tot;
         KM_ALLOC(count, (uint64_t)kNumCells * 4);
         KM_ALLOC(cell_tot, (uint64_t)kCellGroups * 8 * 2);
-        if (points_follow) {
+        if (front) {
+            front->cell_count = cell_count_d;
+            front->cell_tot = std::move(cell_tot);
+            front->scan = CellScanOut{s->cell_start.as<uint32_t>(), nullptr, s->ne_cell.as<uint32_t>(), s->ne_start.as<uint32_t>(), s->ne_cost.as<uint32_t>(),
+                                      s->ne_count.as<uint32_t>()};
+        } else if (points_follow) {
             hipLaunchKernelGGL(k_cell_totals, dim3(kCellGroups), dim3(64), 0, c->stream, cell_count_d, cell_tot.as<uint2>());
             hipLaunchKernelGGL(k_cell_scan, dim3(kCellGroups), dim3(64), 0, c->stream, cell_count_d, (const uint2 *)cell_tot.as<uint2>(), s->cell_start.as<uint32_t>(),
                                (uint32_t *)nullptr, s->ne_cell.as<uint32_t>(), s->ne_start.as<uint32_t>(), s->ne_cost.as<uint32_t>(),
@@ -1235,7 +1214,16 @@
         }
         s->wfirst_waves = G;
         if (s->fused && nshards == 1 && c->ps_div <= 1 && c->opt(CNIIC_OPT_KM_LOOP, "CNIIC_KM_LOOP", 0) == 0) {
-            const int rc_ps = ps_prepare(s);
+            PsSetup ps;
+            int rc_ps = ps_decide(s, &ps);
+            if (rc_ps == CNIIC_OK && ps.on) {
+                if (front) {
+                    front->ranges = true; front->G = ps.G; front->budget = ps.budget; front->cb = ps.cb; front->dev = ps.dev; front->ptrs = ps.ptrs;
+                    front->ps_arena = ps.zero_p; front->ps_zero_bytes = ps.zero_bytes;
+                } else {
+                    rc_ps = ps_enqueue(s, ps);
+                }
+            }
             if (rc_ps != CNIIC_OK) { delete s; return rc_ps; }
         }
         hipError_t e = hipGetLastError();
@@ -1254,6 +1242,34 @@
     hipError_t e = hipGetLastError();
     if (e != hipSuccess) { delete s; return c->fail(CNIIC_ERR_HIP, "kmeans_rgbw init launch: %s", hipGetErrorString(e)); }
     *out = s;
+    return CNIIC_OK;
+}
+
+int km_rgbw_create(Ctx *c, const uint32_t *keys_d, const uint32_t *weight_d, uint64_t U, uint32_t shard,
+                   uint32_t nshards, uint32_t K, const cniic_kmeans_opts *opts, void *partials_dev,
+                   const uint32_t *rank_table_d, KmRgbwState **out, const uint32_t *cell_count_d, const void *gbits_d,
+                   const uint32_t *gprefix_d, uint64_t Ug, bool points_follow, const uint64_t *points_dev) {
+    return km_create_impl(c, keys_d, weight_d, U, shard, nshards, K, opts, partials_dev, rank_table_d, out, cell_count_d, gbits_d, gprefix_d, Ug,
+                          points_follow, points_dev, nullptr);
+}
+
+int km_rgbw_create_deferred(Ctx *c, uint64_t Umax, uint32_t K, const cniic_kmeans_opts *opts, KmRgbwState **out, const uint32_t *cell_count_d,
+                            const void *gbits_d, const uint32_t *gprefix_d, uint64_t Ug, const uint64_t *points_dev, KmFront *front) {
+    return km_create_impl(c, nullptr, nullptr, Umax, 0, 1, K, opts, nullptr, nullptr, out, cell_count_d, gbits_d, gprefix_d, Ug, true, points_dev, front);
+}
+
+int km_front_enqueue_split(Ctx *c, const KmFront &f) {
+    CNIIC_HIP_TRY(c, hipMemsetAsync(f.arena, 0, f.arena_bytes, c->stream));
+    hipLaunchKernelGGL(k_rgbw_init_cent, dim3(ceil_div(f.Kpad, 256)), dim3(256), 0, c->stream, (const uint32_t *)nullptr, f.Ulist, f.K, f.Kpad, f.idbits,
+                       f.cconst, f.cent, f.gx, f.cent_copy, f.moved_list, f.U_dev);
+    hipLaunchKernelGGL(k_cell_totals, dim3(kCellGroups), dim3(64), 0, c->stream, f.cell_count, f.cell_tot.as<uint2>());
+    hipLaunchKernelGGL(k_cell_scan, dim3(kCellGroups), dim3(64), 0, c->stream, f.cell_count, (const uint2 *)f.cell_tot.as<uint2>(), f.scan.cell_start,
+                       (uint32_t *)nullptr, f.scan.ne_cell, f.scan.ne_start, f.scan.ne_cost, f.scan.ne_count, kCellFixedCost, kCellSweepCost);
+    if (f.ranges) {
+        CNIIC_HIP_TRY(c, hipMemsetAsync(f.ps_arena, 0, f.ps_zero_bytes, c->stream));
+        ps_launch_ranges(c, f.scan.ne_cost, f.scan.ne_count, f.G, f.budget, f.cb, f.dev, f.ptrs);
+    }
+    CNIIC_HIP_TRY(c, hipGetLastError());
     return CNIIC_OK;
 }
 
diff --git a/cniic_amd/csrc/k_points.hip b/cniic_amd/csrc/k_points.hip
--- a/cniic_amd/csrc/k_points.hip
+++ b/cniic_amd/csrc/k_points.hip
@@ -1,5 +1,6 @@
 #include "common.hpp"
 #include "device_utils.hpp"
+#include "kmeans_rgbw.hpp"
 
 namespace cniic {
 
@@ -71,16 +72,6 @@
     if (threadIdx.x == 255) total[b] = run;
 }
 
-__global__ __launch_bounds__(kSpBuckets) void k_sp_bstart(const uint32_t *__restrict__ total, uint32_t *__restrict__ bstart,
-                                                          uint32_t *__restrict__ sstart) {
-    __shared__ uint32_t wsum[kSpBuckets / 64];
-    const uint32_t t = total[threadIdx.x];
-    const uint32_t ex = block_exclusive_scan<kSpBuckets>(t, wsum);
-    bstart[threadIdx.x] = ex;
-    if (threadIdx.x == kSpBuckets - 1) bstart[kSpBuckets] = ex + t;
-    sstart[threadIdx.x] = block_exclusive_scan<kSpBuckets>(min(t, kSpBins), wsum);
-}
-
 template <int STEPS, typename F> __device__ __forceinline__ void sp_walk_sorted(const uint32_t *off, uint32_t n, F &&f) {
     const uint32_t lane = threadIdx.x & 63, wv = threadIdx.x >> 6;
     const uint32_t per = (n + kSpThreads - 1) / kSpThreads * 64;
@@ -109,15 +100,25 @@
 }
 
 __global__ __launch_bounds__(kSpThreads) void k_sp_scatter(const uint8_t *__restrict__ rgb, uint64_t npx, const uint32_t *__restrict__ cnt,
-                                                           const uint32_t *__restrict__ pre, const uint32_t *__restrict__ bstart,
+                                                           const uint32_t *__restrict__ pre, const uint32_t *__restrict__ total,
+                                                           uint32_t *__restrict__ bstart, uint32_t *__restrict__ sstart,
                                                            uint16_t *__restrict__ part, uint16_t *__restrict__ prank) {
     extern __shared__ __align__(16) uint8_t sp_lds[];
     uint16_t *stage = reinterpret_cast<uint16_t *>(sp_lds);
     uint32_t *off = reinterpret_cast<uint32_t *>(sp_lds + (size_t)kSpChunk * 2);
     uint32_t *cur = off + kSpBuckets + 1;
     __shared__ uint32_t wsum[kSpWaves];
+    __shared__ uint32_t bfirst[kSpBuckets];
     const uint32_t *mycnt = cnt + (size_t)blockIdx.x * kSpBuckets;
     const uint32_t n_b = threadIdx.x < kSpBuckets ? mycnt[threadIdx.x] : 0u;
+    const uint32_t tot_b = threadIdx.x < kSpBuckets ? total[threadIdx.x] : 0u;
+    const uint32_t first_b = scan512(tot_b, wsum);
+    if (threadIdx.x < kSpBuckets) bfirst[threadIdx.x] = first_b;
+    if (blockIdx.x == 0) {
+        const uint32_t sfirst = scan512(min(tot_b, kSpBins), wsum);
+        if (threadIdx.x < kSpBuckets) { bstart[threadIdx.x] = first_b; sstart[threadIdx.x] = sfirst; }
+        if (threadIdx.x == kSpBuckets - 1) bstart[kSpBuckets] = first_b + tot_b;
+    }
     const uint32_t ex = scan512(n_b, wsum);
     if (threadIdx.x < kSpBuckets) { off[threadIdx.x] = ex; cur[threadIdx.x] = 0; }
     if (threadIdx.x == kSpBuckets - 1) off[kSpBuckets] = ex + n_b;
@@ -145,7 +146,7 @@
     const uint32_t lane = threadIdx.x & 63, wv = threadIdx.x >> 6;
     const uint32_t *mypre = pre + (size_t)blockIdx.x * kSpBuckets;
     const uint32_t mb = wv + kSpWaves * (lane & 31);
-    const uint32_t m_n = mycnt[mb], m_dst = bstart[mb] + mypre[mb], m_off = off[mb];
+    const uint32_t m_n = mycnt[mb], m_dst = bfirst[mb] + mypre[mb], m_off = off[mb];
     for (uint32_t k = 0; k < kSpBuckets / kSpWaves; k++) {
         const uint32_t n = __shfl(m_n, k, 64), d0 = __shfl(m_dst, k, 64), o = __shfl(m_off, k, 64);
         for (uint32_t i = lane; i < n; i += 64) part[(size_t)d0 + i] = stage[o + i];
@@ -246,14 +247,13 @@
 };
 
 constexpr uint32_t kSpEmitSplit = 4;
-__global__ __launch_bounds__(256) void k_sp_emit(const uint32_t *__restrict__ sstart, const uint16_t *__restrict__ sbin,
-                                                 const uint32_t *__restrict__ scnt, SpEmit em) {
-    const uint32_t bucket = blockIdx.x / kSpEmitSplit, part_no = blockIdx.x % kSpEmitSplit;
+__device__ __forceinline__ void sp_emit_body(uint32_t bucket, uint32_t first, const uint32_t *__restrict__ sstart, const uint16_t *__restrict__ sbin,
+                                             const uint32_t *__restrict__ scnt, const SpEmit &em) {
     const uint32_t q0 = em.cell_start[bucket * 64], n = em.cell_start[bucket * 64 + 64] - q0, s0 = sstart[bucket];
     const uint32_t U = em.U_dev ? (uint32_t)*em.U_dev : (uint32_t)em.gx.U, ppc = max(U / em.K, 1u);
     const float rcp = 1.0f / (float)ppc;
     constexpr uint32_t kStride = 256 * kSpEmitSplit;
-    for (uint32_t i0 = part_no * 256 + threadIdx.x; i0 < n; i0 += 4 * kStride) {
+    for (uint32_t i0 = first; i0 < n; i0 += 4 * kStride) {
         uint32_t key[4], cnt[4], rank[4];
 #pragma unroll
         for (int t = 0; t < 4; t++) {
@@ -275,18 +275,67 @@
         }
     }
 }
+__global__ __launch_bounds__(256) void k_sp_emit(const uint32_t *__restrict__ sstart, const uint16_t *__restrict__ sbin,
+                                                 const uint32_t *__restrict__ scnt, SpEmit em) {
+    sp_emit_body(blockIdx.x / kSpEmitSplit, (blockIdx.x % kSpEmitSplit) * 256 + threadIdx.x, sstart, sbin, scnt, em);
+}
 
 __global__ __launch_bounds__(256) void k_bits_prefix(const unsigned long long *__restrict__ bits, uint32_t *__restrict__ wprefix,
                                                      uint32_t *__restrict__ blocktot) {
     __shared__ uint32_t wsum[256 / 64];
-    const uint32_t w0 = (blockIdx.x * 256 + threadIdx.x) * 4;
-    uint32_t cnt[4], mine = 0;
-#pragma unroll
-    for (int q = 0; q < 4; q++) { cnt[q] = (uint32_t)__popcll(bits[w0 + q]); mine += cnt[q]; }
-    uint32_t run = block_exclusive_scan<256>(mine, wsum);
-#pragma unroll
-    for (int q = 0; q < 4; q++) { wprefix[w0 + q] = run; run += cnt[q]; }
-    if (threadIdx.x == 255) blocktot[blockIdx.x] = run;
+    bits_prefix_body(blockIdx.x, bits, wprefix, blocktot, wsum);
+}
+
+constexpr uint32_t kFrontPrefixBlocks = 256;
+constexpr uint32_t kFrontCellBlocks = kCellGroups / 4;
+constexpr uint32_t kFrontZeroBlocks = 32;
+static_assert(kCellGroups % 4 == 0, "four waves of a block each take a group of cells");
+struct FrontA {
+    const unsigned long long *bits; uint32_t *wprefix, *blocktot;
+    const uint32_t *cell_count; uint2 *cell_tot;
+    uint4 *zero0, *zero1; uint32_t n0, n1;
+};
+__global__ __launch_bounds__(256) void k_cc_front_a(FrontA a) {
+    __shared__ uint32_t wsum[256 / 64];
+    const uint32_t b = blockIdx.x;
+    if (b < kFrontPrefixBlocks) {
+        bits_prefix_body(b, a.bits, a.wprefix, a.blocktot, wsum);
+    } else if (b < kFrontPrefixBlocks + kFrontCellBlocks) {
+        cell_totals_body((b - kFrontPrefixBlocks) * 4 + (threadIdx.x >> 6), threadIdx.x & 63u, a.cell_count, a.cell_tot);
+    } else {
+        const uint32_t t = (b - kFrontPrefixBlocks - kFrontCellBlocks) * 256 + threadIdx.x;
+        for (uint32_t i = t; i < a.n0; i += kFrontZeroBlocks * 256) a.zero0[i] = make_uint4(0u, 0u, 0u, 0u);
+        for (uint32_t i = t; i < a.n1; i += kFrontZeroBlocks * 256) a.zero1[i] = make_uint4(0u, 0u, 0u, 0u);
+    }
+}
+struct FrontB {
+    uint32_t *wprefix; const uint32_t *blocktot; uint64_t *total;
+    const uint32_t *cell_count; const uint2 *cell_tot; CellScanOut scan;
+};
+__global__ __launch_bounds__(256) void k_cc_front_b(FrontB a) {
+    __shared__ uint32_t wsum[256 / 64];
+    __shared__ uint32_t boff[256];
+    const uint32_t b = blockIdx.x;
+    if (b < kFrontPrefixBlocks) gidx_finish_body(b, a.wprefix, a.blocktot, a.total, wsum, boff);
+    else cell_scan_body((b - kFrontPrefixBlocks) * 4 + (threadIdx.x >> 6), threadIdx.x & 63u, a.cell_count, a.cell_tot, a.scan, kCellFixedCost, kCellSweepCost);
+}
+struct FrontC {
+    uint32_t ranges, cent_blocks;
+    const uint32_t *ne_cost, *ne_count; uint32_t G, budget; uint32_t *cb; PsDev *dev; PsDevPtrs ptrs;
+    uint64_t Ulist; uint32_t K, Kpad, idbits; uint2 *cconst; uint32_t *cent, *cent_copy, *moved_list; const uint64_t *U_dev; GIdx cgx;
+    const uint32_t *sstart; const uint16_t *sbin; const uint32_t *scnt; SpEmit em;
+};
+__global__ __launch_bounds__(kSpThreads) void k_cc_front_c(FrontC a) {
+    const uint32_t b = blockIdx.x;
+    if (b < a.ranges) {
+        ps_ranges_body(a.ne_cost, a.ne_count, a.G, a.budget, a.cb, a.dev, a.ptrs);
+    } else if (b < a.ranges + a.cent_blocks) {
+        rgbw_init_cent_body((b - a.ranges) * kSpThreads + threadIdx.x, nullptr, a.Ulist, a.K, a.Kpad, a.idbits, a.cconst, a.cent, a.cgx, a.cent_copy,
+                            a.moved_list, a.U_dev);
+    } else {
+        static_assert(kSpThreads == 256 * kSpEmitSplit, "one block is the emit's 1024 threads of a bucket");
+        sp_emit_body(b - a.ranges - a.cent_blocks, threadIdx.x, a.sstart, a.sbin, a.scnt, a.em);
+    }
 }
 
 template <typename LabelT>
@@ -557,7 +606,7 @@
     return CNIIC_OK;
 }
 
-int sp_build(Ctx *c, const uint8_t *rgb_d, uint64_t npx, SpPlan *plan) {
+int sp_build(Ctx *c, const uint8_t *rgb_d, uint64_t npx, SpPlan *plan, bool hist_only) {
     if (npx == 0 || (reinterpret_cast<uintptr_t>(rgb_d) & 15)) return c->fail(CNIIC_ERR_BAD_ARG, "sp_build: empty or unaligned image");
     CNIIC_TRY(sp_set_lds(c));
     plan->npx = npx;
@@ -577,21 +626,20 @@
     CNIIC_HIP_TRY(c, plan->wprefix.alloc((1ull << 18) * 4));
     DevBuf total, blocktot;
     CNIIC_HIP_TRY(c, total.alloc((uint64_t)kSpBuckets * 4));
-    CNIIC_HIP_TRY(c, blocktot.alloc(256 * 4));
+    if (!hist_only) CNIIC_HIP_TRY(c, blocktot.alloc(256 * 4));
     CNIIC_HIP_TRY(c, plan->total.alloc(8));
     CNIIC_HIP_TRY(c, c->pinned_u.reserve(kPinnedUBytes, kPinnedUBytes));
     CNIIC_HIP_TRY(c, c->u_ev.ensure(hipEventDisableTiming));
     hipLaunchKernelGGL(k_sp_count, dim3(plan->nchunks), dim3(kSpThreads), 0, c->stream, rgb_d, npx, plan->cnt.as<uint32_t>());
     hipLaunchKernelGGL(k_sp_colscan, dim3(kSpBuckets), dim3(256), 0, c->stream, plan->cnt.as<uint32_t>(), plan->nchunks,
                        plan->pre.as<uint32_t>(), total.as<uint32_t>());
-    hipLaunchKernelGGL(k_sp_bstart, dim3(1), dim3(kSpBuckets), 0, c->stream, total.as<uint32_t>(), plan->bstart.as<uint32_t>(),
-                       plan->sstart.as<uint32_t>());
     hipLaunchKernelGGL(k_sp_scatter, dim3(plan->nchunks), dim3(kSpThreads), (size_t)kSpChunk * 2 + kSpBuckets * 8 + 16, c->stream, rgb_d, npx,
-                       plan->cnt.as<uint32_t>(), plan->pre.as<uint32_t>(), plan->bstart.as<uint32_t>(), plan->part.as<uint16_t>(),
-                       plan->prank.as<uint16_t>());
+                       plan->cnt.as<uint32_t>(), plan->pre.as<uint32_t>(), (const uint32_t *)total.as<uint32_t>(), plan->bstart.as<uint32_t>(),
+                       plan->sstart.as<uint32_t>(), plan->part.as<uint16_t>(), plan->prank.as<uint16_t>());
     hipLaunchKernelGGL(k_sp_hist, dim3(kSpBuckets), dim3(kSpThreads), (size_t)kSpBins * 4, c->stream, plan->part.as<uint16_t>(),
                        plan->bstart.as<uint32_t>(), plan->sstart.as<uint32_t>(), plan->cell_count.as<uint32_t>(), plan->bits.as<uint32_t>(),
                        plan->sbin.as<uint16_t>(), plan->scnt.as<uint32_t>());
+    if (hist_only) { CNIIC_HIP_TRY(c, hipGetLastError()); return CNIIC_OK; }
     hipLaunchKernelGGL(k_bits_prefix, dim3(256), dim3(256), 0, c->stream, plan->bits.as<unsigned long long>(), plan->wprefix.as<uint32_t>(),
                        blocktot.as<uint32_t>());
     CNIIC_TRY(gidx_finish(c, plan->wprefix.as<uint32_t>(), blocktot.as<uint32_t>(), plan->total.as<uint64_t>()));
@@ -599,6 +647,52 @@
     CNIIC_HIP_TRY(c, hipMemcpyAsync(c->pinned_u.as<uint64_t>() + kPuSpCount.at, plan->total.p, 8, hipMemcpyDeviceToHost, c->stream));
     CNIIC_HIP_TRY(c, hipEventRecord(c->u_ev, c->stream));
     return CNIIC_OK;
+}
+
+int sp_front(Ctx *c, SpPlan *plan, const KmFront &f, uint32_t *ckeys_d, uint32_t *cweight_d, void *labels_d, bool wide, bool fused) {
+    DevBuf blocktot;
+    CNIIC_HIP_TRY(c, blocktot.alloc(256 * 4));
+    const uint64_t *U_dev = plan->total.as<uint64_t>();
+    const GIdx gx{plan->bits.as<unsigned long long>(), plan->wprefix.as<uint32_t>(), 0};
+    const SpEmit em{f.scan.cell_start, ckeys_d, cweight_d, labels_d, f.K, wide ? 1u : 0u, gx, U_dev};
+    if (!fused) {
+        hipLaunchKernelGGL(k_bits_prefix, dim3(256), dim3(256), 0, c->stream, plan->bits.as<unsigned long long>(), plan->wprefix.as<uint32_t>(),
+                           blocktot.as<uint32_t>());
+        CNIIC_TRY(gidx_finish(c, plan->wprefix.as<uint32_t>(), blocktot.as<uint32_t>(), plan->total.as<uint64_t>()));
+        CNIIC_HIP_TRY(c, hipMemcpyAsync(c->pinned_u.as<uint64_t>() + kPuSpCount.at, plan->total.p, 8, hipMemcpyDeviceToHost, c->stream));
+        CNIIC_HIP_TRY(c, hipEventRecord(c->u_ev, c->stream));
+        CNIIC_TRY(km_front_enqueue_split(c, f));
+        hipLaunchKernelGGL(k_sp_emit, dim3(kSpBuckets * kSpEmitSplit), dim3(256), 0, c->stream, plan->sstart.as<uint32_t>(), plan->sbin.as<uint16_t>(),
+                           plan->scnt.as<uint32_t>(), em);
+        CNIIC_HIP_TRY(c, hipGetLastError());
+        return CNIIC_OK;
+    }
+    FrontA a{};
+    a.bits = plan->bits.as<unsigned long long>(); a.wprefix = plan->wprefix.as<uint32_t>(); a.blocktot = blocktot.as<uint32_t>();
+    a.cell_count = f.cell_count; a.cell_tot = f.cell_tot.as<uint2>();
+    a.zero0 = static_cast<uint4 *>(f.arena); a.n0 = (uint32_t)(f.arena_bytes / 16);
+    a.zero1 = static_cast<uint4 *>(f.ps_arena); a.n1 = f.ranges ? (uint32_t)(f.ps_zero_bytes / 16) : 0u;
+    hipLaunchKernelGGL(k_cc_front_a, dim3(kFrontPrefixBlocks + kFrontCellBlocks + kFrontZeroBlocks), dim3(256), 0, c->stream, a);
+    FrontB b{};
+    b.wprefix = a.wprefix; b.blocktot = a.blocktot; b.total = plan->total.as<uint64_t>();
+    b.cell_count = f.cell_count; b.cell_tot = a.cell_tot; b.scan = f.scan;
+    hipLaunchKernelGGL(k_cc_front_b, dim3(kFrontPrefixBlocks + kFrontCellBlocks), dim3(256), 0, c->stream, b);
+    CNIIC_HIP_TRY(c, hipGetLastError());
+    CNIIC_HIP_TRY(c, hipMemcpyAsync(c->pinned_u.as<uint64_t>() + kPuSpCount.at, plan->total.p, 8, hipMemcpyDeviceToHost, c->stream));
+    CNIIC_HIP_TRY(c, hipEventRecord(c->u_ev, c->stream));
+    FrontC k{};
+    k.ranges = f.ranges ? 1u : 0u; k.cent_blocks = (uint32_t)ceil_div(f.Kpad, kSpThreads);
+    k.ne_cost = f.scan.ne_cost; k.ne_count = f.scan.ne_count; k.G = f.G; k.budget = f.budget; k.cb = f.cb; k.dev = f.dev; k.ptrs = f.ptrs;
+    k.Ulist = f.Ulist; k.K = f.K; k.Kpad = f.Kpad; k.idbits = f.idbits; k.cconst = f.cconst; k.cent = f.cent; k.cent_copy = f.cent_copy;
+    k.moved_list = f.moved_list; k.U_dev = f.U_dev; k.cgx = f.gx;
+    k.sstart = plan->sstart.as<uint32_t>(); k.sbin = plan->sbin.as<uint16_t>(); k.scnt = plan->scnt.as<uint32_t>(); k.em = em;
+    hipLaunchKernelGGL(k_cc_front_c, dim3(k.ranges + k.cent_blocks + kSpBuckets), dim3(kSpThreads), 0, c->stream, k);
+    CNIIC_HIP_TRY(c, hipGetLastError());
+    return CNIIC_OK;
+}
+bool sp_front_fits(const KmFront &f) {
+    auto ok = [](const void *p, uint64_t n) { return (reinterpret_cast<uintptr_t>(p) & 15) == 0 && n % 16 == 0 && n / 16 < (1ull << 32); };
+    return ok(f.arena, f.arena_bytes) && (!f.ranges || ok(f.ps_arena, f.ps_zero_bytes));
 }
 
 int sp_wait_count(Ctx *c, SpPlan *plan) {
diff --git a/cniic_amd/csrc/kmeans_rgbw.hpp b/cniic_amd/csrc/kmeans_rgbw.hpp
--- a/cniic_amd/csrc/kmeans_rgbw.hpp
+++ b/cniic_amd/csrc/kmeans_rgbw.hpp
@@ -91,7 +91,15 @@
 struct PsExit { uint32_t status, pad; uint64_t iter, moved_last, reseeds, active, pair_evals; };
 void launch_rgbw_assign_big(Ctx *c, const uint32_t *ckeys, const uint32_t *cweight, uint64_t U, uint32_t K, const uint32_t *cent, uint16_t *labels,
                             unsigned long long *partials, const KmDevState *st);
-int ps_prepare(KmRgbwState *s);
+struct PsSetup {
+    bool on = false;
+    uint32_t G = 0, budget = 0;
+    uint32_t *cb = nullptr; PsDev *dev = nullptr; PsDevPtrs ptrs{};
+    void *zero_p = nullptr; uint64_t zero_bytes = 0;
+};
+int ps_decide(KmRgbwState *s, PsSetup *out);
+int ps_enqueue(KmRgbwState *s, const PsSetup &p);
+void ps_launch_ranges(Ctx *c, const uint32_t *ne_cost, const uint32_t *ne_count, uint32_t G, uint32_t budget, uint32_t *cb, PsDev *dev, const PsDevPtrs &ptrs);
 int km_rgbw_run_persistent(KmRgbwState *s, bool *ran, bool may_defer);
 int km_rgbw_persistent_verdict(KmRgbwState *s, bool *retry);
 constexpr uint32_t kAggMin = 16;
@@ -106,6 +114,106 @@
     uint32_t idmask = (1u << idbits) - 1;
     return make_uint2(ckey, ((kBias - h) << idbits) | (idmask - k));
 }
+
+__device__ __forceinline__ void rgbw_init_cent_body(uint32_t k, const uint32_t *__restrict__ keys, uint64_t U, uint32_t K, uint32_t Kpad, uint32_t idbits,
+                                                    uint2 *__restrict__ cconst, uint32_t *__restrict__ cent, const GIdx &gx, uint32_t *__restrict__ cent_copy,
+                                                    uint32_t *__restrict__ moved_list, const uint64_t *__restrict__ U_dev) {
+    if (U_dev) U = max(*U_dev, (uint64_t)K);
+    if (k == 0 && moved_list) moved_list[0] = K;
+    if (k < K) {
+        uint64_t ppc = U / K;
+        uint64_t first = (k < K - 1) ? U - ((uint64_t)k + 1) * ppc : 0;
+        uint32_t ck = gx.bits ? gidx_select(gx, first) : keys[first];
+        cent[k] = ck;
+        if (cent_copy) cent_copy[k] = ck;
+        cconst[k] = make_cconst(ck, k, idbits);
+    } else if (k < Kpad) {
+        cconst[k] = make_uint2(0u, 0u);
+    }
+}
+
+constexpr uint32_t kCellGroups = kNumCells / 64;
+__device__ __forceinline__ void cell_totals_body(uint32_t grp, uint32_t lane, const uint32_t *__restrict__ cell_count, uint2 *__restrict__ tot) {
+    const uint32_t v = cell_count[grp * 64 + lane];
+    const uint32_t sum = wave_reduce_sum(v), sweeps = wave_reduce_sum((v + 64 * kSweep - 1) / (64 * kSweep));
+    const uint32_t ne = (uint32_t)__popcll(__ballot(v != 0));
+    if (lane == 0) { tot[grp] = make_uint2(sum, ne); tot[kCellGroups + grp] = make_uint2(sweeps, 0u); }
+}
+struct CellScanOut { uint32_t *cell_start, *cursor, *ne_cell, *ne_start, *ne_cost, *ne_count; };
+__device__ __forceinline__ void cell_scan_body(uint32_t grp, uint32_t lane, const uint32_t *__restrict__ cell_count, const uint2 *__restrict__ tot,
+                                               const CellScanOut &o, uint32_t fixed_cost, uint32_t sweep_cost) {
+    uint32_t ps = 0, pn = 0, pw = 0;
+    for (uint32_t g = lane; g < grp; g += 64) { const uint2 t = tot[g]; ps += t.x; pn += t.y; pw += tot[kCellGroups + g].x; }
+    const uint32_t base = wave_reduce_sum(ps), nbase = wave_reduce_sum(pn), wbase = wave_reduce_sum(pw);
+    const uint32_t cell = grp * 64 + lane, v = cell_count[cell], sw = (v + 64 * kSweep - 1) / (64 * kSweep);
+    const uint32_t start = base + wave_inclusive_scan(v) - v, swb = wbase + wave_inclusive_scan(sw) - sw;
+    o.cell_start[cell] = start;
+    if (o.cursor) o.cursor[cell] = start;
+    const unsigned long long nzm = __ballot(v != 0);
+    if (v) {
+        const uint32_t m = nbase + (uint32_t)__popcll(nzm & ((1ull << lane) - 1ull));
+        o.ne_cell[m] = cell; o.ne_start[m] = start; o.ne_cost[m] = (sweep_cost ? swb * sweep_cost : start) + m * fixed_cost;
+    }
+    if (grp == kCellGroups - 1 && lane == 63) {
+        const uint32_t U = start + v, M = nbase + (uint32_t)__popcll(nzm);
+        o.cell_start[kNumCells] = U;
+        o.ne_start[M] = U;
+        o.ne_cost[M] = (sweep_cost ? (swb + sw) * sweep_cost : U) + M * fixed_cost;
+        *o.ne_count = M;
+    }
+}
+
+__device__ __forceinline__ void ps_ranges_body(const uint32_t *__restrict__ ne_cost, const uint32_t *__restrict__ ne_count, uint32_t G, uint32_t dyn_bytes,
+                                               uint32_t *__restrict__ cb, PsDev *__restrict__ dev, const PsDevPtrs &ptrs) {
+    uint32_t *fail = &dev->fail;
+    if (threadIdx.x == 0) dev->p = ptrs;
+    const uint32_t M = *ne_count, NC = G * kPsChunks;
+    const uint64_t total = ne_cost[M];
+    for (uint32_t g0 = threadIdx.x; g0 <= NC; g0 += 8 * blockDim.x) {
+        uint32_t a[8], b[8];
+        uint64_t c_lo[8];
+#pragma unroll
+        for (int r = 0; r < 8; r++) {
+            const uint32_t g = g0 + r * blockDim.x;
+            c_lo[r] = total * min(g, NC) / NC;
+            a[r] = 0; b[r] = g <= NC ? M : 0u;
+        }
+        bool more = true;
+        while (more) {
+            more = false;
+            uint32_t mid[8], v[8];
+#pragma unroll
+            for (int r = 0; r < 8; r++) { mid[r] = (a[r] + b[r]) >> 1; v[r] = a[r] < b[r] ? ne_cost[mid[r]] : 0u; }
+#pragma unroll
+            for (int r = 0; r < 8; r++)
+                if (a[r] < b[r]) { if (v[r] < c_lo[r]) a[r] = mid[r] + 1; else b[r] = mid[r]; more = more || a[r] < b[r]; }
+        }
+#pragma unroll
+        for (int r = 0; r < 8; r++) {
+            const uint32_t g = g0 + r * blockDim.x;
+            if (g <= NC) cb[g] = g == NC ? M : a[r];
+        }
+    }
+    __syncthreads();
+    for (uint32_t g = threadIdx.x; g < G; g += blockDim.x) {
+        uint32_t C = 0;
+        for (uint32_t r = 0; r < kPsChunks; r++) C += cb[r * G + g + 1] - cb[r * G + g];
+        if (C > kPsMaxCells || kPsOffCell + ps_cell_bytes(C) > dyn_bytes) atomicAdd(fail, 1u);
+    }
+}
+
+struct KmFront {
+    void *arena = nullptr; uint64_t arena_bytes = 0;
+    void *ps_arena = nullptr; uint64_t ps_zero_bytes = 0;
+    uint64_t Ulist = 0; uint32_t K = 0, Kpad = 0, idbits = 0;
+    uint2 *cconst = nullptr; uint32_t *cent = nullptr, *cent_copy = nullptr, *moved_list = nullptr;
+    GIdx gx{nullptr, nullptr, 0}; const uint64_t *U_dev = nullptr;
+    const uint32_t *cell_count = nullptr; DevBuf cell_tot; CellScanOut scan{};
+    bool ranges = false; uint32_t G = 0, budget = 0; uint32_t *cb = nullptr; PsDev *dev = nullptr; PsDevPtrs ptrs{};
+};
+int km_rgbw_create_deferred(Ctx *c, uint64_t Umax, uint32_t K, const cniic_kmeans_opts *opts, KmRgbwState **out, const uint32_t *cell_count_d,
+                            const void *gbits_d, const uint32_t *gprefix_d, uint64_t Ug, const uint64_t *points_dev, KmFront *front);
+int km_front_enqueue_split(Ctx *c, const KmFront &f);
 
 struct CellBox { int32_t r0, g0, b0; };
 __device__ __forceinline__ CellBox super_box(uint32_t sup) {
```

Measured after the change: 10680 Mpixels/s (median of 6 runs). +2.4%, better.
